# Stylish-TTS/stylish-tts

Measured on AMD Instinct MI355X. Metric: audio frames/sec/GPU (24 kHz) forward+backward; DDP scaling 1/2/4/8 MI355X, higher is better.
Workload: dtype bf16 GEMM operands, f32 accumulation/storage; 1 GPU; c3: B=32/GPU T=520 frames (6.5 s) L=100

## Files before the change

### stylish_tts_amd/csrc/api.hip

```cpp
#include <math.h>
#include <stdarg.h>
#include <string.h>
#include <stdlib.h>
#include <cxxabi.h>

#include <map>
#include <string>

#include "model.h"

namespace sty {

static thread_local char g_err[1024] = "";
void set_error(const char* fmt, ...) {
  va_list ap;
  va_start(ap, fmt);
  vsnprintf(g_err, sizeof(g_err), fmt, ap);
  va_end(ap);
}
int hip_fail(hipError_t e, const char* what) {
  set_error("HIP error %d (%s) at %s", (int)e, hipGetErrorString(e), what);
  return STY_EHIP;
}

// ... 44 lines not shown
  auto it = cache.find(fn);
  if (it != cache.end()) return it->second;
  std::string out;
  const char* mangled = hipKernelNameRefByPtr(fn, st);
  if (mangled) {
    int status = 0;
    char* dem = abi::__cxa_demangle(mangled, nullptr, nullptr, &status);
    std::string d = (status == 0 && dem) ? dem : mangled;
    free(dem);
    int depth = 0;
    size_t cut = d.size();
    for (size_t i = 0; i < d.size(); ++i) {
      if (d[i] == '<') ++depth;
      if (d[i] == '>') --depth;
      if (d[i] == '(' && depth == 0 && d.compare(i, 21, "(anonymous namespace)") != 0) {
        cut = i;
        break;
      }
    }
    d = d.substr(0, cut);
    if (d.compare(0, 5, "void ") == 0) d = d.substr(5);
    for (const char* ns : {"sty::(anonymous namespace)::", "sty::"})
      if (d.compare(0, strlen(ns), ns) == 0) d = d.substr(strlen(ns));
    out = d;
  }
  cache[fn] = out;
  return out;
}

struct Builder {
  sty_model* m;
  bool dry;
  bool ok = true;

  const Param* get(const std::string& key, std::initializer_list<int64_t> shape = {}) {
    if (dry) m->requested.push_back(key);
    auto it = m->params.find(key);
    if (it == m->params.end()) {
      if (ok) m->missing = key;
      ok = false;
      return nullptr;
    }
    if (shape.size()) {
      std::vector<int64_t> want(shape);
      if (want != it->second.shape) {
        if (ok) m->missing = key + " (shape mismatch)";
        ok = false;
        return nullptr;
      }
    }
    return &it->second;
  }
  const float* ptr(const std::string& key, std::initializer_list<int64_t> shape = {}) {
    const Param* p = get(key, shape);
    return p ? p->p : nullptr;
  }
  bool has(const std::string& key) const { return m->params.count(key) != 0; }

  PackedConv conv(const std::string& name, bool wn = false, bool bias = true, bool glu = false,
                  const float* bias_override_src = nullptr) {
    PackedConv pc;
    const Param* w = wn ? get(name + ".parametrizations.weight.original1") : get(name + ".weight");
    const Param* g = wn ? get(name + ".parametrizations.weight.original0") : nullptr;
    const float* b = bias ? ptr(name + ".bias") : nullptr;
    if (!w || (wn && !g)) return pc;
    const auto& s = w->shape;
    pc.Cout = (int)s[0];
    pc.Cin = (int)s[1];
    pc.K = s.size() > 2 ? (int)s[2] : 1;
    pc.CinP = (int)align_up(pc.Cin, CI_CHUNK);
    pc.CoutP = glu ? (int)align_up(pc.Cout, 64) : (int)align_up(pc.Cout, 32);
    float* wp = m->ab.take<float>((size_t)pc.K * pc.CinP * pc.CoutP);
    float* bp = m->ab.take<float>(pc.CoutP);
    pc.wp = wp;
    pc.bias = (bias || bias_override_src) ? bp : nullptr;
    if (!dry) {
      PackJob j;
      j.kind = glu ? PK_CONV_GLU : (wn ? PK_CONV_WN : PK_CONV);
      j.w = wn ? nullptr : w->p;
      j.g = g ? g->p : nullptr;
      j.v = wn ? w->p : nullptr;
      j.bias = b;
      j.Cout = pc.Cout;
      j.Cin = pc.Cin;
      j.K = pc.K;
      j.CinP = pc.CinP;
      j.CoutP = pc.CoutP;
      j.wp = wp;
      j.bp = bp;
      m->jobs.push_back(j);
    }
    if (m->train_enabled) {
      if (glu) {
        PackedConv pl = pc;
        pl.CoutP = (int)align_up(pc.Cout, 32);
        float* wp2 = m->ab.take<float>((size_t)pc.K * pc.CinP * pl.CoutP);
        float* bp2 = m->ab.take<float>(pl.CoutP);
        pl.wp = wp2;
        pl.bias = bias ? bp2 : nullptr;
        if (!dry) {
          PackJob j;
          j.kind = PK_CONV;
          j.w = w->p;
          j.bias = b;
          j.Cout = pc.Cout;
          j.Cin = pc.Cin;
          j.K = pc.K;
          j.CinP = pc.CinP;
          j.CoutP = pl.CoutP;
          j.wp = wp2;
          j.bp = bp2;
          m->jobs.push_back(j);
          m->plain_of[wp] = pl;
        }
        add_dgrad(pl);
      } else {
        add_dgrad(pc);
      }
    }
    return pc;
  }

  void add_dgrad(const PackedConv& pc) {
    PackedConv d;
    d.Cin = pc.Cout;
    d.CinP = pc.CoutP;
    d.Cout = pc.Cin;
    d.CoutP = pc.CinP;
    d.K = pc.K;
    float* wd = m->ab.take<float>((size_t)pc.K * pc.CinP * pc.CoutP);
    d.wp = wd;
    d.bias = nullptr;
    if (!dry) {
      PackJob j;
      j.kind = PK_DGRAD;
      j.w = pc.wp;
      j.K = pc.K;
      j.CinP = pc.CinP;
      j.CoutP = pc.CoutP;
      j.wp = wd;
      m->jobs.push_back(j);
      m->dgrad[pc.wp] = d;
    }
  }

  AdaFc fc(const std::string& name, int C) {
    AdaFc a;
    a.C = C;
    const float* W = ptr(name + ".fc.weight", {2 * C, m->style_dim});
    const float* b = ptr(name + ".fc.bias", {2 * C});
    a.off = m->gb_floats_per_batch;
    m->gb_floats_per_batch += 2 * C;
    if (!dry) {
      a.idx = (int)m->fcs.size();
      StyleFcDesc d;
      d.W = W;
      d.b = b;
      d.off = a.off;
      d.n = 2 * C;
      d.pad = 0;
      m->fcs.push_back(d);
    }
    return a;
  }

  ConvNeXt convnext(const std::string& p, int C, bool snake = true) {
    ConvNeXt c;
    c.C = C;
    c.dw_w = ptr(p + ".dwconv.weight", {C, 1, 7});
    c.dw_b = ptr(p + ".dwconv.bias", {C});
    c.norm = fc(p + ".norm", C);
    c.alpha = snake ? ptr(p + ".snake", {1, 1, 4 * C}) : nullptr;
    c.grn_gamma = ptr(p + ".grn.gamma", {1, 1, 4 * C});
    const float* grn_beta = ptr(p + ".grn.beta", {1, 1, 4 * C});
    c.b1 = ptr(p + ".pwconv1.bias", {4 * C});
    const float* w2 = ptr(p + ".pwconv2.weight", {C, 4 * C});
// ... 115 lines not shown
    v.phase_norm_w = ptr(b + "phase_norm.weight", {32});
    v.phase_norm_b = ptr(b + "phase_norm.bias", {32});
    v.amp_fln_w = ptr(b + "amp_final_layer_norm.weight", {32});
    v.amp_fln_b = ptr(b + "amp_final_layer_norm.bias", {32});
    v.phase_fln_w = ptr(b + "phase_final_layer_norm.weight", {32});
    v.phase_fln_b = ptr(b + "phase_final_layer_norm.bias", {32});
    v.phase_convnext.clear();
    for (int i = 0; has(b + "phase_convnext." + std::to_string(i) + ".dwconv.weight"); ++i)
      v.phase_convnext.push_back(convnext(b + "phase_convnext." + std::to_string(i), 32));
    if (ok && (v.amp_convnext.empty() || v.phase_convnext.empty())) {
      m->missing = b + "amp_convnext.0 / phase_convnext.0";
      ok = false;
    }
  }

  void text_encoder(const std::string& p) {
    TextEncPlan& t = m->te;
    const Param* e = get(p + "emb.weight");
    if (!e) return;
    t.emb = e->p;
    t.tokens = (int)e->shape[0];
    t.H = (int)e->shape[1];
    for (int i = 0; i < 3; ++i) {
      const std::string si = std::to_string(i);
      t.pre[i] = conv(p + "prenet.conv_layers." + si);
      t.pre_g[i] = ptr(p + "prenet.norm_layers." + si + ".gamma", {t.H});
      t.pre_b[i] = ptr(p + "prenet.norm_layers." + si + ".beta", {t.H});
    }
    t.proj = conv(p + "prenet.proj");
    t.layers.clear();
    for (int i = 0; has(p + "encoder.attn_layers." + std::to_string(i) + ".conv_q.weight"); ++i) {
      const std::string si = std::to_string(i);
      TextEncLayer l;
      l.q = conv(p + "encoder.attn_layers." + si + ".conv_q");
      l.k = conv(p + "encoder.attn_layers." + si + ".conv_k");
      l.v = conv(p + "encoder.attn_layers." + si + ".conv_v");
      l.o = conv(p + "encoder.attn_layers." + si + ".conv_o");
      l.n1g = ptr(p + "encoder.norm_layers_1." + si + ".gamma", {t.H});
      l.n1b = ptr(p + "encoder.norm_layers_1." + si + ".beta", {t.H});
      l.f1 = conv(p + "encoder.ffn_layers." + si + ".conv_1");
      l.f2 = conv(p + "encoder.ffn_layers." + si + ".conv_2");
      l.n2g = ptr(p + "encoder.norm_layers_2." + si + ".gamma", {t.H});
      l.n2b = ptr(p + "encoder.norm_layers_2." + si + ".beta", {t.H});
      t.layers.push_back(l);
    }
    t.proj_m = conv(p + "proj_m");
    for (int i = 0; i < 4; ++i) t.theta[i] = 1.0f / powf(10000.0f, (float)(2 * i) / 8.0f);
  }

  DecBlock dec_block(const std::string& p) {
    DecBlock d;
    d.c1 = conv(p + ".conv1", true);
    d.c2 = conv(p + ".conv2", true);
    d.Cin = d.c1.Cin;
    d.Cout = d.c1.Cout;
    d.n1 = fc(p + ".norm1", d.Cin);
    d.n2 = fc(p + ".norm2", d.Cout);
    d.has_sc = has(p + ".conv1x1.parametrizations.weight.original0");
    if (d.has_sc) d.sc = conv(p + ".conv1x1", true, false);
    return d;
  }

  void decoder(const std::string& p) {
    DecoderPlan& d = m->dec;
    d.encode = dec_block(p + "encode");
    for (int i = 0; i < 4; ++i) d.decode[i] = dec_block(p + "decode." + std::to_string(i));
    d.asr_res = conv(p + "asr_res.0", true);
    d.f0_g = ptr(p + "F0_conv.parametrizations.weight.original0", {1, 1, 1});
    d.f0_v = ptr(p + "F0_conv.parametrizations.weight.original1", {1, 1, 3});
// ... 1349 lines not shown
  std::vector<MultiJob> jobs[5];
  std::vector<int> blk[5];
  std::vector<int> blk1;
  auto PG = [&](const float* p) -> float* {
    auto it = p ? m->pgrad.find(p) : m->pgrad.end();
    return it == m->pgrad.end() ? nullptr : it->second;
  };
  auto GA = [&](const float* packed) -> float* {
    return (packed && m->garena) ? reinterpret_cast<float*>(m->garena + (reinterpret_cast<const char*>(packed) - m->arena))
                                 : nullptr;
  };
  auto add = [&](int which, MultiJob j, int nblocks) {
    j.blk0 = (int)blk[which].size();
    for (int i = 0; i < nblocks; ++i) blk[which].push_back((int)jobs[which].size());
    jobs[which].push_back(j);
  };
  size_t job_index = 0;
  m->seg_blk_split = 0;
  for (const PackJob& j : m->jobs) {
    if (job_index++ == m->seg_job_split) m->seg_blk_split = (int)blk[2].size();
    if (j.kind == PK_CONV || j.kind == PK_CONV_WN || j.kind == PK_CONV_GLU) {
      MultiJob a;
      a.p0 = j.w;
      a.p1 = j.g;
      a.p2 = j.v;
      a.p3 = j.bias;
      a.q0 = j.wp;
      a.q1 = j.bp;
      a.Cout = j.Cout;
      a.Cin = j.Cin;
      a.K = j.K;
      a.CinP = j.CinP;
      a.CoutP = j.CoutP;
      a.glu = j.kind == PK_CONV_GLU;
      add(0, a, j.Cout);
      if (m->garena && j.kind != PK_CONV_GLU) {
        MultiJob u;
        u.p0 = GA(j.wp);
        u.p1 = j.g;
        u.p2 = j.kind == PK_CONV_WN ? j.v : nullptr;
        u.p3 = (j.bias && j.bp) ? GA(j.bp) : nullptr;
        u.q0 = j.kind == PK_CONV ? PG(j.w) : nullptr;
        u.q1 = j.kind == PK_CONV_WN ? PG(j.g) : nullptr;
        u.q2 = j.kind == PK_CONV_WN ? PG(j.v) : nullptr;
        u.q3 = (j.bias && j.bp) ? PG(j.bias) : nullptr;
        u.Cout = j.Cout;
        u.Cin = j.Cin;
        u.K = j.K;
        u.CinP = j.CinP;
        u.CoutP = j.CoutP;
        if (u.q0 || (u.q1 && u.q2) || u.q3) add(2, u, j.Cout);
      }
    } else if (j.kind == PK_DGRAD) {
      MultiJob a;
      a.p0 = j.w;
      a.q0 = j.wp;
      a.K = j.K;
      a.CinP = j.CinP;
      a.CoutP = j.CoutP;
      add(1, a, (int)(((size_t)j.K * j.CinP * j.CoutP + 255) / 256));
    } else if (j.kind == PK_DGRAD2D) {
      MultiJob a;
      a.p0 = j.w;
      a.q0 = j.wp;
      a.K = j.K;
      a.KH = j.KH;
      a.Cin = j.Cin;
      a.Cout = j.Cout;
      a.CinP = j.CinP;
      a.CoutP = j.CoutP;
      a.glu = 2;
      a.blk1 = (int)align_up(j.KH * j.Cout, CI_CHUNK);
      a.pad = (int)align_up(j.Cin, 32);
      add(1, a, (int)(((size_t)j.K * j.KH * j.Cout * j.Cin + 255) / 256));
    }
    if (j.kind == PK_CONV2D_SN || j.kind == PK_DW2D_SN) {
      MultiJob a;
      a.p0 = j.w;
      a.p1 = j.bias;
      a.p2 = j.kind == PK_CONV2D_SN ? j.bp : nullptr;
      a.q0 = const_cast<float*>(j.g);
      a.q1 = const_cast<float*>(j.v);
      a.q2 = j.scratch;
// ... 1159 lines not shown
```

### stylish_tts_amd/csrc/attn.hip

```cpp
#include "sty_common.h"

namespace sty {


template <int DH, bool DROP>
__global__ __launch_bounds__(256) void attn_kernel(AttnArgs a) {
  constexpr int DP = DH < 32 ? 32 : DH;
  constexpr int LS = 33;
  __shared__ float ks[DH * LS];
  __shared__ float vs[DP * LS];
  const int tid = threadIdx.x, lane = tid & 63, wave = tid >> 6, l31 = lane & 31, hi = lane >> 5;
  const int b = blockIdx.z, h = blockIdx.y, T = a.T;
  const int i0 = blockIdx.x * 128 + wave * 32;
  const int qi = i0 + l31;
  const float* qb = a.q + (size_t)b * a.qbs + (size_t)h * DH * T;
  const float* kb = a.k + (size_t)b * a.kbs + (size_t)h * DH * T;
  const float* vb = a.v + (size_t)b * a.vbs + (size_t)h * DH * T;
  int len = T;
  if (a.lengths) len = (int)a.lengths[b];

  float qreg[DH / 2];
#pragma unroll
  for (int c2 = 0; c2 < DH / 2; ++c2) qreg[c2] = qi < T ? qb[(size_t)(2 * c2 + hi) * T + qi] * a.scale : 0.f;

  f32x16 oacc[DP / 32];
#pragma unroll
  for (int d = 0; d < DP / 32; ++d)
#pragma unroll
    for (int r = 0; r < 16; ++r) oacc[d][r] = 0.f;
  float m_run = -3.0e38f, l_run = 0.f;
  const bool q_pad = a.lengths && qi >= len;

  for (int j0 = 0; j0 < T; j0 += 32) {
    __syncthreads();
    for (int e = tid; e < DH * 32; e += 256) {
      const int d = e >> 5, jj = e & 31;
      const int j = j0 + jj;
      ks[d * LS + jj] = j < T ? kb[(size_t)d * T + j] : 0.f;
      vs[d * LS + jj] = j < T ? vb[(size_t)d * T + j] : 0.f;
    }
    if (DP > DH)
      for (int e = tid; e < (DP - DH) * 32; e += 256) vs[(DH + (e >> 5)) * LS + (e & 31)] = 0.f;
    __syncthreads();

    f32x16 s;
#pragma unroll
    for (int r = 0; r < 16; ++r) s[r] = 0.f;
#pragma unroll
    for (int c2 = 0; c2 < DH / 2; ++c2)
      s = __builtin_amdgcn_mfma_f32_32x32x2f32(ks[(2 * c2 + hi) * LS + l31], qreg[c2], s, 0, 0, 0);

    float mx = -3.0e38f;
#pragma unroll
    for (int r = 0; r < 16; ++r) {
      const int j = j0 + (r & 3) + 8 * (r >> 2) + 4 * hi;
      float x = s[r];
      if (a.lengths && (q_pad || j >= len)) x += -1e4f;
      if (j >= T) x = -INFINITY;
      s[r] = x;
      mx = fmaxf(mx, x);
    }
    mx = fmaxf(mx, __shfl_xor(mx, 32));
    const float m_new = fmaxf(m_run, mx);
    const float alpha = expf(m_run - m_new);
    float rs = 0.f;
#pragma unroll
    for (int r = 0; r < 16; ++r) {
      const float p = expf(s[r] - m_new);
      s[r] = p;
      rs += p;
    }
// ... 5 lines not shown
      const unsigned rowi = ((unsigned)(b * a.H + h) * (unsigned)T + (unsigned)qi) * (unsigned)T;
#pragma unroll
      for (int r = 0; r < 16; ++r) {
        const int j = j0 + (r & 3) + 8 * (r >> 2) + 4 * hi;
        s[r] = sty_hash_u(a.drop_seed, a.drop_site, rowi + (unsigned)j) >= a.drop_p ? s[r] * ks_ : 0.f;
      }
    }
#pragma unroll
    for (int d = 0; d < DP / 32; ++d) {
#pragma unroll
      for (int r = 0; r < 16; ++r) oacc[d][r] *= alpha;
#pragma unroll
      for (int q = 0; q < 16; ++q) {
        const float av = vs[(d * 32 + l31) * LS + (q & 3) + 8 * (q >> 2) + 4 * hi];
        oacc[d] = __builtin_amdgcn_mfma_f32_32x32x2f32(av, s[q], oacc[d], 0, 0, 0);
      }
    }
  }
  if (qi < T) {
    if (a.lse && hi == 0) a.lse[((size_t)b * a.H + h) * T + qi] = m_run + logf(l_run);
    const float inv = 1.0f / l_run;
    float* ob = a.o + (size_t)b * a.obs + (size_t)h * DH * T;
#pragma unroll
    for (int d = 0; d < DP / 32; ++d)
#pragma unroll
      for (int r = 0; r < 16; ++r) {
        const int dd = d * 32 + (r & 3) + 8 * (r >> 2) + 4 * hi;
        if (dd < DH) ob[(size_t)dd * T + qi] = oacc[d][r] * inv;
      }
  }
}

int launch_attention(const AttnArgs& a, int B, int DH, hipStream_t st) {
  if (attention16_eligible(a, DH)) return launch_attention16(a, B, st);
  dim3 grid(cdiv(a.T, 128), a.H, B);
  const bool drop = a.drop_p > 0.f;
  if (DH == 64 && !drop)
    hipLaunchKernelGGL((attn_kernel<64, false>), grid, dim3(256), 0, st, a);
  else if (DH == 16 && !drop)
    hipLaunchKernelGGL((attn_kernel<16, false>), grid, dim3(256), 0, st, a);
  else if (DH == 160 && !drop)
    hipLaunchKernelGGL((attn_kernel<160, false>), grid, dim3(256), 0, st, a);
  else if (DH == 96 && !drop)
    hipLaunchKernelGGL((attn_kernel<96, false>), grid, dim3(256), 0, st, a);
  else if (DH == 16)
    hipLaunchKernelGGL((attn_kernel<16, true>), grid, dim3(256), 0, st, a);
  else if (DH == 160)
    hipLaunchKernelGGL((attn_kernel<160, true>), grid, dim3(256), 0, st, a);
  else {
    set_error("attention: head dim %d%s not built (16, 64, 96, 160; dropout: 16, 160)", DH, drop ? " with dropout" : "");
    return STY_EINVAL;
  }
  STY_LAUNCH_CHECK();
  return STY_OK;
}

__global__ void rope_kernel(const float* qs, const float* ks, float* q, float* k, int H, int DH, int L, int d, float t0, float t1, float t2, float t3,
                            float sgn) {
  const int pos = blockIdx.x * blockDim.x + threadIdx.x;
  const int h = blockIdx.y, b = blockIdx.z;
  if (pos >= L) return;
  const float theta[4] = {t0, t1, t2, t3};
  const int half = d / 2;
  const float* src[2] = {qs, ks};
  float* ptr[2] = {q, k};
  for (int w = 0; w < 2; ++w) {
    const size_t o = ((size_t)b * H + h) * DH * L + pos;
    const float* sb_ = src[w] + o;
    float* base = ptr[w] + o;
    float x[8];
    for (int i = 0; i < d; ++i) x[i] = sb_[(size_t)i * L];
    for (int i = 0; i < d; ++i) {
      const float ang = (float)pos * theta[i % half];
      const float rot = i < half ? -x[i + half] : x[i - half];
      base[(size_t)i * L] = x[i] * cosf(ang) + rot * (sgn * sinf(ang));
    }
    if (sb_ != base)
      for (int i = d; i < DH; ++i) base[(size_t)i * L] = sb_[(size_t)i * L];
  }
}

int launch_rope_signed(float* q, float* k, int B, int H, int DH, int L, int d, const float* theta4, float sgn,
                       hipStream_t st) {
  if (d != 8) {
    set_error("rope: only d == 8 built");
    return STY_EINVAL;
  }
  hipLaunchKernelGGL(rope_kernel, dim3(cdiv(L, 64), H, B), dim3(64), 0, st, q, k, q, k, H, DH, L, d, theta4[0], theta4[1],
                     theta4[2], theta4[3], sgn);
  STY_LAUNCH_CHECK();
  return STY_OK;
}
int launch_rope_copy(const float* qs, const float* ks, float* q, float* k, int B, int H, int DH, int L, int d,
                     const float* theta4, hipStream_t st) {
  if (d != 8) {
    set_error("rope: only d == 8 built");
    return STY_EINVAL;
  }
  hipLaunchKernelGGL(rope_kernel, dim3(cdiv(L, 64), H, B), dim3(64), 0, st, qs, ks, q, k, H, DH, L, d, theta4[0], theta4[1],
                     theta4[2], theta4[3], 1.0f);
  STY_LAUNCH_CHECK();
  return STY_OK;
}
int launch_rope(float* q, float* k, int B, int H, int DH, int L, int d, const float* theta4, hipStream_t st) {
  return launch_rope_signed(q, k, B, H, DH, L, d, theta4, 1.0f, st);
}
}
```

### stylish_tts_amd/csrc/attn_bwd.hip

```cpp
#include <stdlib.h>

#include "sty_common.h"

namespace sty {

template <int DH>
__global__ __launch_bounds__(64) void attn_bwd_a_kernel(AttnArgs a, const float* __restrict__ dO, size_t dobs,
                                                        float* __restrict__ lse, float* __restrict__ delta) {
  const int T = a.T, b = blockIdx.z, h = blockIdx.y, i = blockIdx.x * 64 + threadIdx.x;
  if (i >= T) return;
  const float* qb = a.q + (size_t)b * a.qbs + (size_t)h * DH * T;
  const float* kb = a.k + (size_t)b * a.kbs + (size_t)h * DH * T;
  const float* ob = a.o + (size_t)b * a.obs + (size_t)h * DH * T;
  const float* gb = dO + (size_t)b * dobs + (size_t)h * DH * T;
  const int len = a.lengths ? (int)a.lengths[b] : T;
  float q[DH];
  float dl = 0.f;
#pragma unroll
  for (int d = 0; d < DH; ++d) {
    q[d] = qb[(size_t)d * T + i] * a.scale;
    dl = fmaf(gb[(size_t)d * T + i], ob[(size_t)d * T + i], dl);
  }
  float m = -3.0e38f, l = 0.f;
  const bool qpad = a.lengths && i >= len;
// ... 295 lines not shown
    }
#pragma unroll
    for (int n = 0; n < NB; ++n)
#pragma unroll
      for (int q = 0; q < 16; ++q)
        dq[n] = __builtin_amdgcn_mfma_f32_32x32x2f32(ks[(n * 32 + l31) * LS + frag_row(q, hi)], dp[q], dq[n], 0, 0, 0);
  }
  if (i < T) {
    float* dqb = dQ + (size_t)b * dqbs + (size_t)h * DH * T;
#pragma unroll
    for (int n = 0; n < NB; ++n)
#pragma unroll
      for (int r = 0; r < 16; ++r) dqb[(size_t)(n * 32 + frag_row(r, hi)) * T + i] += dq[n][r] * a.scale;
  }
}


template <int DH, bool DROP>
__global__ __launch_bounds__(256) void attn_bwd_small_kernel(AttnArgs a, const float* __restrict__ dO, size_t dobs,
                                                            float* __restrict__ dQ, size_t dqbs, float* __restrict__ dK,
                                                            size_t dkbs, float* __restrict__ dV, size_t dvbs, int overwrite) {
  constexpr int TP = 129;
  __shared__ float qs[DH * TP], ks[DH * TP], vs[DH * TP], gs[DH * TP];
  __shared__ float lse_s[128], del_s[128], pm_s[128], pl_s[128];
  const int T = a.T, h = blockIdx.x, b = blockIdx.y, tid = threadIdx.x;
  const int r = tid & 127, half = tid >> 7;
  const size_t ho = (size_t)h * DH * T;
  const float* qb = a.q + (size_t)b * a.qbs + ho;
  const float* kb = a.k + (size_t)b * a.kbs + ho;
  const float* vb = a.v + (size_t)b * a.vbs + ho;
  const float* gb = dO + (size_t)b * dobs + ho;
  const float* ob = a.o + (size_t)b * a.obs + ho;
  const int len = a.lengths ? (int)a.lengths[b] : T;
  for (int e = tid; e < DH * T; e += 256) {
    const int d = e / T, t = e - d * T;
    qs[d * TP + t] = qb[e] * a.scale;
    ks[d * TP + t] = kb[e];
    vs[d * TP + t] = vb[e];
    gs[d * TP + t] = gb[e];
  }
  __syncthreads();
  const int per = (T + 1) / 2, lo = half * per, hi = min(T, lo + per);
  const bool live = r < T;
  const bool rpad = a.lengths && r >= len;
  float q[DH], g[DH];
#pragma unroll
  for (int d = 0; d < DH; ++d) {
    q[d] = live ? qs[d * TP + r] : 0.f;
    g[d] = live ? gs[d * TP + r] : 0.f;
  }
  {
    float m = -3.0e38f, l = 0.f;
    if (live)
      for (int j = lo; j < hi; ++j) {
        float sv = 0.f;
#pragma unroll
        for (int d = 0; d < DH; ++d) sv = fmaf(q[d], ks[d * TP + j], sv);
        if (a.lengths && (rpad || j >= len)) sv += -1e4f;
        const float mn = fmaxf(m, sv);
        l = l * expf(m - mn) + expf(sv - mn);
        m = mn;
      }
    if (half == 1) {
      pm_s[r] = m;
      pl_s[r] = l;
    } else if (live) {
      float dl = 0.f;
#pragma unroll
      for (int d = 0; d < DH; ++d) dl = fmaf(g[d], ob[(size_t)d * T + r], dl);
      del_s[r] = dl;
// ... 6 lines not shown
    }
    __syncthreads();
  }
  const float inv_keep = DROP ? 1.0f / (1.0f - a.drop_p) : 1.f;
  const unsigned rowbase = (unsigned)(b * a.H + h) * (unsigned)T;
  {
    float acc[DH];
#pragma unroll
    for (int d = 0; d < DH; ++d) acc[d] = 0.f;
    if (live) {
      const float L = lse_s[r], dl = del_s[r];
      for (int j = lo; j < hi; ++j) {
        float sv = 0.f, dp = 0.f;
#pragma unroll
        for (int d = 0; d < DH; ++d) {
          sv = fmaf(q[d], ks[d * TP + j], sv);
          dp = fmaf(g[d], vs[d * TP + j], dp);
        }
        if (a.lengths && (rpad || j >= len)) sv += -1e4f;
        if constexpr (DROP) {
          const unsigned idx = (rowbase + (unsigned)r) * (unsigned)T + (unsigned)j;
          dp = sty_hash_u(a.drop_seed, a.drop_site, idx) >= a.drop_p ? dp * inv_keep : 0.f;
        }
        const float ds = expf(sv - L) * (dp - dl);
#pragma unroll
        for (int d = 0; d < DH; ++d) acc[d] = fmaf(ds, ks[d * TP + j], acc[d]);
      }
    }
#pragma unroll
    for (int d = 0; d < DH; ++d) {
      __syncthreads();
      if (half == 1) pm_s[r] = acc[d];
      __syncthreads();
      if (half == 0 && live) {
        float* dq = dQ + (size_t)b * dqbs + ho;
        const float val = (acc[d] + pm_s[r]) * a.scale;
        dq[(size_t)d * T + r] = (overwrite & 1) ? val : dq[(size_t)d * T + r] + val;
      }
    }
  }
  {
    float kk[DH], vv[DH], ak[DH], av[DH];
#pragma unroll
    for (int d = 0; d < DH; ++d) {
      kk[d] = live ? ks[d * TP + r] : 0.f;
      vv[d] = live ? vs[d * TP + r] : 0.f;
      ak[d] = av[d] = 0.f;
    }
    if (live)
      for (int i = lo; i < hi; ++i) {
        float sv = 0.f, dp = 0.f;
#pragma unroll
        for (int d = 0; d < DH; ++d) {
          sv = fmaf(qs[d * TP + i], kk[d], sv);
          dp = fmaf(gs[d * TP + i], vv[d], dp);
        }
        if (a.lengths && (i >= len || rpad)) sv += -1e4f;
        const float p = expf(sv - lse_s[i]);
        float pm = p;
        if constexpr (DROP) {
          const unsigned idx = (rowbase + (unsigned)i) * (unsigned)T + (unsigned)r;
          const float mf = sty_hash_u(a.drop_seed, a.drop_site, idx) >= a.drop_p ? inv_keep : 0.f;
          pm = p * mf;
          dp *= mf;
        }
        const float ds = p * (dp - del_s[i]);
#pragma unroll
        for (int d = 0; d < DH; ++d) {
          av[d] = fmaf(pm, gs[d * TP + i], av[d]);
          ak[d] = fmaf(ds, qs[d * TP + i], ak[d]);
        }
      }
    float* dk = dK + (size_t)b * dkbs + ho;
    float* dv = dV + (size_t)b * dvbs + ho;
#pragma unroll
    for (int d = 0; d < DH; ++d) {
      __syncthreads();
      if (half == 1) {
        pm_s[r] = ak[d];
        pl_s[r] = av[d];
      }
      __syncthreads();
      if (half == 0 && live) {
        const float vk = ak[d] + pm_s[r], vv_ = av[d] + pl_s[r];
        dk[(size_t)d * T + r] = (overwrite & 2) ? vk : dk[(size_t)d * T + r] + vk;
        dv[(size_t)d * T + r] = (overwrite & 4) ? vv_ : dv[(size_t)d * T + r] + vv_;
      }
    }
  }
}

size_t attention_bwd_ws_floats(int B, int H, int T) { return (size_t)2 * B * H * T; }

bool attention_bwd_mfma_dh(int DH) { return DH == 64 || DH == 96 || DH == 160; }
static bool attn_bwd_mfma_path(const AttnArgs& a, int DH) { return a.lse && attention_bwd_mfma_dh(DH); }
static bool attn_bwd_small_path(const AttnArgs& a, int DH) {
  if (attention16_eligible(a, DH) && a.lse) return false;
  if (attn_bwd_mfma_path(a, DH)) return false;
  return DH == 16 && a.T <= 128;
}
bool attention_bwd_can_overwrite(const AttnArgs& a, int DH) { return attn_bwd_small_path(a, DH); }

int launch_attention_bwd(const AttnArgs& a, const float* dO, float* dQ, float* dK, float* dV, size_t dqbs, size_t dkbs,
                         size_t dvbs, size_t dobs, int B, int DH, float* ws, hipStream_t st, int overwrite) {
  if (overwrite && !attn_bwd_small_path(a, DH)) {
    set_error("attention_bwd: overwrite requested on a path that accumulates");
    return STY_EINVAL;
  }
  if (attention16_eligible(a, DH) && a.lse)
    return launch_attention16_bwd(a, dO, dQ, dK, dV, dqbs, dkbs, dvbs, dobs, B, ws, st);
  float* lse = ws;
  float* delta = ws + (size_t)B * a.H * a.T;
  if (attn_bwd_mfma_path(a, DH)) {
    hipLaunchKernelGGL(attn_delta_kernel, dim3(cdiv(a.T, 256), a.H, B), dim3(256), 0, st, a.o, a.obs, dO, dobs, a.H, DH,
                       a.T, delta);
    dim3 g2(cdiv(a.T, 128), a.H, B);
#define STY_ABWD_MFMA(DHV, DR)                                                                                                      \
  hipLaunchKernelGGL((attn_bwd_kv_mfma_kernel<DHV, DR>), g2, dim3(256), 0, st, a, dO, dobs, a.lse, delta, dK, dkbs, dV, dvbs);       \
  hipLaunchKernelGGL((attn_bwd_q_mfma_kernel<DHV, DR>), g2, dim3(256), 0, st, a, dO, dobs, a.lse, delta, dQ, dqbs)
    const bool dr = a.drop_p > 0.f;
    if (DH == 64 && !dr) {
      STY_ABWD_MFMA(64, false);
    } else if (DH == 64) {
      STY_ABWD_MFMA(64, true);
    } else if (DH == 96 && !dr) {
      STY_ABWD_MFMA(96, false);
    } else if (DH == 96) {
      STY_ABWD_MFMA(96, true);
    } else if (!dr) {
      STY_ABWD_MFMA(160, false);
    } else {
      STY_ABWD_MFMA(160, true);
    }
#undef STY_ABWD_MFMA
    STY_LAUNCH_CHECK();
    return STY_OK;
  }
  const bool drop = a.drop_p > 0.f;
  if (attn_bwd_small_path(a, DH)) {
    if (drop)
      hipLaunchKernelGGL((attn_bwd_small_kernel<16, true>), dim3(a.H, B), dim3(256), 0, st, a, dO, dobs, dQ, dqbs, dK, dkbs, dV,
                         dvbs, overwrite);
    else
      hipLaunchKernelGGL((attn_bwd_small_kernel<16, false>), dim3(a.H, B), dim3(256), 0, st, a, dO, dobs, dQ, dqbs, dK, dkbs,
                         dV, dvbs, overwrite);
    STY_LAUNCH_CHECK();
    return STY_OK;
  }
  if (DH != 16) {
    set_error("attention_bwd: head dim %d%s not built", DH, drop ? " with dropout" : "");
    return STY_EINVAL;
  }
  dim3 grid(cdiv(a.T, 64), a.H, B);
#define STY_ABWD(DR)                                                                                                         \
  hipLaunchKernelGGL(attn_bwd_a_kernel<16>, grid, dim3(64), 0, st, a, dO, dobs, lse, delta);                                 \
  hipLaunchKernelGGL((attn_bwd_b_kernel<16, DR>), grid, dim3(256), 2 * 16 * 65 * sizeof(float), st, a, dO, dobs, lse, delta, \
                     dK, dkbs, dV, dvbs);                                                                                    \
  hipLaunchKernelGGL((attn_bwd_c_kernel<16, DR>), grid, dim3(64), 0, st, a, dO, dobs, lse, delta, dQ, dqbs)
  if (drop) {
    STY_ABWD(true);
  } else {
    STY_ABWD(false);
  }
#undef STY_ABWD
  STY_LAUNCH_CHECK();
  return STY_OK;
}

}
```

### stylish_tts_amd/csrc/bwd.hip

```cpp
#include "sty_common.h"

namespace sty {

__device__ __forceinline__ double wave_sum(double v) {
  for (int o = 32; o > 0; o >>= 1) v += __shfl_xor(v, o);
  return v;
}

template <int N>
__device__ __forceinline__ void block_sum(double (&v)[N], double (*red)[4]) {
  const int lane = threadIdx.x & 63, wave = threadIdx.x >> 6;
#pragma unroll
  for (int i = 0; i < N; ++i) {
    v[i] = wave_sum(v[i]);
    if (lane == 0) red[i][wave] = v[i];
  }
  __syncthreads();
  if (threadIdx.x == 0) {
#pragma unroll
    for (int i = 0; i < N; ++i) v[i] = red[i][0] + red[i][1] + red[i][2] + red[i][3];
  }
}

__global__ __launch_bounds__(256) void pro_bwd_kernel(int mode_, const float* __restrict__ u, int Cu, int cu0,
// ... 305 lines not shown
                                                          float eps, float* __restrict__ mean, float* __restrict__ rstd) {
  const int i = blockIdx.x * 4 + (threadIdx.x >> 6), lane = threadIdx.x & 63;
  if (i >= rows) return;
  double sum = 0.0, sq = 0.0;
  for (int k = lane; k < nseg; k += 64) {
    sum += part[((size_t)i * nseg + k) * 2];
    sq += part[((size_t)i * nseg + k) * 2 + 1];
  }
  for (int o = 32; o > 0; o >>= 1) {
    sum += __shfl_xor(sum, o);
    sq += __shfl_xor(sq, o);
  }
  if (lane) return;
  const double m = sum / T;
  double var = sq / T - m * m;
  if (var < 0.0) var = 0.0;
  mean[i] = (float)m;
  rstd[i] = (float)(1.0 / sqrt(var + (double)eps));
}
int launch_adain_stats(const double* part, int nseg, int rows, int T, float eps, float* mean, float* rstd,
                       hipStream_t st) {
  hipLaunchKernelGGL(adain_stats_kernel, dim3(cdiv(rows, 4)), dim3(256), 0, st, part, nseg, rows, T, eps, mean, rstd);
  STY_LAUNCH_CHECK();
  return STY_OK;
}

template <int TC, int NR>
__global__ __launch_bounds__(256) void chan_ln_bwd_dx_reg_kernel(const float* __restrict__ x, const float* __restrict__ dy,
                                                                 const float* __restrict__ y, int C, int T, float eps,
                                                                 int ada, const float* __restrict__ w,
                                                                 const float* __restrict__ gb, int relu,
                                                                 const float* __restrict__ out_mask,
                                                                 float* __restrict__ dx, int accumulate,
                                                                 float* __restrict__ mu_out, float* __restrict__ r_out) {
  constexpr int CG = 256 / TC;
  __shared__ float red[2][CG][TC];
  const int col = threadIdx.x % TC, cg = threadIdx.x / TC;
  const int t = blockIdx.x * TC + col, b = blockIdx.y;
  const bool in = t < T;
  const size_t base = (size_t)b * C * T + (in ? t : 0);
  auto combine = [&](float a, float bb, float& ra, float& rb) {
    red[0][cg][col] = a;
    red[1][cg][col] = bb;
    __syncthreads();
    float s0 = 0.f, s1 = 0.f;
#pragma unroll
    for (int k = 0; k < CG; ++k) {
      s0 += red[0][k][col];
      s1 += red[1][k][col];
    }
    __syncthreads();
    ra = s0;
    rb = s1;
  };
  const float om = (in && out_mask) ? out_mask[(size_t)b * T + t] : 1.f;
  float xr[NR], gr[NR];
#pragma unroll
  for (int i = 0; i < NR; ++i) {
    const int c = cg + i * CG;
    xr[i] = gr[i] = 0.f;
    if (in && c < C) {
      const size_t o = base + (size_t)c * T;
      xr[i] = x[o];
      float g = dy[o] * om;
      if (relu && !(y[o] > 0.f)) g = 0.f;
      const float A = ada ? 1.f + gb[(size_t)b * 2 * C + c] : w[c];
      gr[i] = g * A;
// ... 5 lines not shown
    if (in && cg + i * CG < C) p0 += xr[i];
  combine(p0, 0.f, mean, dummy);
  mean /= (float)C;
  p0 = 0.f;
#pragma unroll
  for (int i = 0; i < NR; ++i)
    if (in && cg + i * CG < C) {
      const float d = xr[i] - mean;
      p0 += d * d;
    }
  float var;
  combine(p0, 0.f, var, dummy);
  const float r = 1.0f / sqrtf(var / (float)C + eps);
  p0 = p1 = 0.f;
#pragma unroll
  for (int i = 0; i < NR; ++i)
    if (in && cg + i * CG < C) {
      const float dxh = gr[i], xh = (xr[i] - mean) * r;
      p0 += dxh;
      p1 += dxh * xh;
    }
  float s1, s2;
  combine(p0, p1, s1, s2);
  s1 /= (float)C;
  s2 /= (float)C;
  if (!in) return;
#pragma unroll
  for (int i = 0; i < NR; ++i) {
    const int c = cg + i * CG;
    if (c < C) {
      const size_t o = base + (size_t)c * T;
      const float xh = (xr[i] - mean) * r;
      const float d = r * (gr[i] - s1 - xh * s2);
      dx[o] = accumulate ? dx[o] + d : d;
    }
  }
  if (cg == 0) {
    mu_out[(size_t)b * T + t] = mean;
    r_out[(size_t)b * T + t] = r;
  }
}
template <int TC>
__global__ __launch_bounds__(256) void chan_ln_bwd_dx_kernel(const float* __restrict__ x, const float* __restrict__ dy,
                                                             const float* __restrict__ y, int C, int T, float eps,
                                                             int ada, const float* __restrict__ w,
                                                             const float* __restrict__ gb, int relu,
                                                             const float* __restrict__ out_mask,
                                                             float* __restrict__ dx, int accumulate,
                                                             float* __restrict__ mu_out, float* __restrict__ r_out) {
  constexpr int CG = 256 / TC;
  __shared__ float red[2][CG][TC];
  const int col = threadIdx.x % TC, cg = threadIdx.x / TC;
  const int t = blockIdx.x * TC + col, b = blockIdx.y;
  const bool in = t < T;
  const size_t base = (size_t)b * C * T + (in ? t : 0);
  auto combine = [&](float a, float bb, float& ra, float& rb) {
    red[0][cg][col] = a;
    red[1][cg][col] = bb;
    __syncthreads();
    float s0 = 0.f, s1 = 0.f;
#pragma unroll
    for (int k = 0; k < CG; ++k) {
      s0 += red[0][k][col];
      s1 += red[1][k][col];
    }
    __syncthreads();
    ra = s0;
    rb = s1;
  };
  float p0 = 0.f, p1 = 0.f, mean, dummy;
  if (in)
    for (int c = cg; c < C; c += CG) p0 += x[base + (size_t)c * T];
  combine(p0, 0.f, mean, dummy);
  mean /= (float)C;
  p0 = 0.f;
  if (in)
    for (int c = cg; c < C; c += CG) {
      const float d = x[base + (size_t)c * T] - mean;
      p0 += d * d;
    }
  float var;
  combine(p0, 0.f, var, dummy);
  const float r = 1.0f / sqrtf(var / (float)C + eps);
  const float om = (in && out_mask) ? out_mask[(size_t)b * T + t] : 1.f;
  p0 = p1 = 0.f;
  if (in)
    for (int c = cg; c < C; c += CG) {
      const size_t o = base + (size_t)c * T;
      float g = dy[o] * om;
      if (relu && !(y[o] > 0.f)) g = 0.f;
      const float A = ada ? 1.f + gb[(size_t)b * 2 * C + c] : w[c];
      const float dxh = g * A, xh = (x[o] - mean) * r;
      p0 += dxh;
      p1 += dxh * xh;
    }
  float s1, s2;
  combine(p0, p1, s1, s2);
  s1 /= (float)C;
  s2 /= (float)C;
  if (!in) return;
  for (int c = cg; c < C; c += CG) {
    const size_t o = base + (size_t)c * T;
    float g = dy[o] * om;
    if (relu && !(y[o] > 0.f)) g = 0.f;
    const float A = ada ? 1.f + gb[(size_t)b * 2 * C + c] : w[c];
    const float xh = (x[o] - mean) * r;
    const float d = r * (g * A - s1 - xh * s2);
    dx[o] = accumulate ? dx[o] + d : d;
  }
  if (cg == 0) {
    mu_out[(size_t)b * T + t] = mean;
    r_out[(size_t)b * T + t] = r;
  }
}
__global__ __launch_bounds__(256) void chan_ln_bwd_param_kernel(const float* __restrict__ x,
                                                                const float* __restrict__ dy,
                                                                const float* __restrict__ y,
                                                                const float* __restrict__ mu,
                                                                const float* __restrict__ r, int C, int T, int ada,
                                                                int relu, const float* __restrict__ out_mask,
                                                                float* __restrict__ dgb, float* __restrict__ dw,
                                                                float* __restrict__ db) {
  __shared__ double red[2][4];
  const int c = blockIdx.x, b = blockIdx.y;
  const size_t row = ((size_t)b * C + c) * T;
  double acc[2] = {0.0, 0.0};
  for (int t = threadIdx.x; t < T; t += 256) {
    float g = dy[row + t];
    if (out_mask) g *= out_mask[(size_t)b * T + t];
    if (relu && !(y[row + t] > 0.f)) g = 0.f;
    const float xh = (x[row + t] - mu[(size_t)b * T + t]) * r[(size_t)b * T + t];
    acc[0] += (double)g * xh;
    acc[1] += (double)g;
  }
  block_sum<2>(acc, red);
  if (threadIdx.x == 0) {
    if (ada) {
      dgb[(size_t)b * 2 * C + c] += (float)acc[0];
      dgb[(size_t)b * 2 * C + C + c] += (float)acc[1];
    } else {
      atomicAdd(&dw[c], (float)acc[0]);
// ... 76 lines not shown
  double s = 0.0;
  for (int b = b0; b < b0 + nb; ++b)
    for (int k = lane; k < nblk; k += 64) s += (double)part[((size_t)b * nblk + k) * 64 + slot];
  s = wave_sum(s);
  if (lane == 0) {
    if (ada)
      dgb[(size_t)b0 * 64 + slot] += (float)s;
    else if (slot < 32)
      dw[slot] += (float)s;
    else
      db[slot - 32] += (float)s;
  }
}

__global__ void cast_any_kernel(const void* __restrict__ x, size_t n, void* __restrict__ y, int to16) {
  const size_t i = (size_t)blockIdx.x * 256 + threadIdx.x;
  if (i < n) sty_st_any(y, i, sty_ld_any(x, i, !to16), to16);
}
int launch_cast_f32_to_16(const float* x, size_t n, void* y16, hipStream_t st) {
  hipLaunchKernelGGL(cast_any_kernel, dim3((unsigned)((n + 255) / 256)), dim3(256), 0, st, x, n, y16, 1);
  STY_LAUNCH_CHECK();
  return STY_OK;
}
int launch_cast_16_to_f32(const void* x16, size_t n, float* y, hipStream_t st) {
  hipLaunchKernelGGL(cast_any_kernel, dim3((unsigned)((n + 255) / 256)), dim3(256), 0, st, x16, n, y, 0);
  STY_LAUNCH_CHECK();
  return STY_OK;
}
bool chan_ln32_eligible(int B, int C, int T, int relu) {
  return C == 32 && !relu && (size_t)B * T >= 65536 && getenv("STY_NO_LN32_BWD") == nullptr;
}
int launch_chan_ln_bwd(const float* x, const float* dy, const float* y, int B, int C, int T, float eps, int ada,
                       const float* w, const float* gb, int relu, const float* out_mask, float* dx, int accumulate,
                       float* mu_tmp, float* r_tmp, float* dgb, float* dw, float* db, hipStream_t st, int h16) {
  const bool no32 = getenv("STY_NO_LN32_BWD") != nullptr;
  if (C == 32 && !relu && (size_t)B * T >= 65536 && !no32) {
    const int nblk = cdiv(T, 256);
    if ((h16 & 4) && accumulate) {
      set_error("chan_ln_bwd: a two-byte dx cannot be accumulated into");
      return STY_EINVAL;
    }
    hipLaunchKernelGGL(chan_ln32_bwd_kernel, dim3(nblk, B), dim3(256), 0, st, x, dy, T, eps, ada, w, gb, out_mask, dx, accumulate,
                       mu_tmp, h16);
    hipLaunchKernelGGL(chan_ln32_param_sum_kernel, dim3(ada ? B * 64 : 64), dim3(64), 0, st, mu_tmp, B, nblk, ada, dgb, dw, db);
    STY_LAUNCH_CHECK();
    return STY_OK;
  }
  if (h16) {
    set_error("chan_ln_bwd: two-byte tensors only on the C = 32 long-row kernel (chan_ln32_eligible)");
    return STY_EINVAL;
  }
  if ((size_t)B * T < 65536 && C <= 256)
    hipLaunchKernelGGL((chan_ln_bwd_dx_reg_kernel<16, 16>), dim3(cdiv(T, 16), B), dim3(256), 0, st, x, dy, y, C, T, eps, ada, w,
                       gb, relu, out_mask, dx, accumulate, mu_tmp, r_tmp);
  else if ((size_t)B * T >= 65536)
    hipLaunchKernelGGL(chan_ln_bwd_dx_kernel<64>, dim3(cdiv(T, 64), B), dim3(256), 0, st, x, dy, y, C, T, eps, ada, w, gb,
                       relu, out_mask, dx, accumulate, mu_tmp, r_tmp);
  else
    hipLaunchKernelGGL(chan_ln_bwd_dx_kernel<16>, dim3(cdiv(T, 16), B), dim3(256), 0, st, x, dy, y, C, T, eps, ada, w, gb,
                       relu, out_mask, dx, accumulate, mu_tmp, r_tmp);
  hipLaunchKernelGGL(chan_ln_bwd_param_kernel, dim3(C, B), dim3(256), 0, st, x, dy, y, mu_tmp, r_tmp, C, T, ada, relu,
                     out_mask, dgb, dw, db);
  STY_LAUNCH_CHECK();
  return STY_OK;
}

__global__ __launch_bounds__(256) void grn_bwd_kernel(const double* __restrict__ part, int nseg,
                                                      const float* __restrict__ gamma,
                                                      const float* __restrict__ ds, int C4,
                                                      float* __restrict__ coef, float* __restrict__ dgamma) {
  __shared__ float gxs[1024];
  __shared__ double red[2][4];
  const int b = blockIdx.x;
  if (nseg < 32) {
    for (int c = threadIdx.x; c < C4; c += 256) {
      double sq = 0.0;
      for (int k = 0; k < nseg; ++k) sq += part[(((size_t)b * C4 + c) * nseg + k) * 2 + 1];
      gxs[c] = (float)sqrt(sq);
    }
  } else {
    const int lane = threadIdx.x & 63, wave = threadIdx.x >> 6;
    for (int c = wave; c < C4; c += 4) {
      const double* pp = part + ((size_t)b * C4 + c) * nseg * 2 + 1;
      double sq = 0.0;
      for (int k = lane; k < nseg; k += 64) sq += pp[(size_t)k * 2];
      for (int o = 32; o > 0; o >>= 1) sq += __shfl_xor(sq, o);
      if (lane == 0) gxs[c] = (float)sqrt(sq);
    }
  }
  __syncthreads();
  double acc[1] = {0.0};
  for (int c = threadIdx.x; c < C4; c += 256) acc[0] += gxs[c];
  __shared__ float mean_s, dot_s;
// ... 44 lines not shown
  else if (kind == ACT_SWISH) r = v / (1.f + expf(-v));
  else if (kind == ACT_SNAKE) r = sty_snake(v, alpha[c], 1.f / alpha[c]);
  else if (kind == 100) r = tanhf(v);
  else if (kind == ACT_GELU) r = 0.5f * v * (1.0f + erff(v * 0.70710678118654752f));
  y[o] = r;
}
__device__ __forceinline__ float act_apply1(int kind, float v, float al, float ral) {
  float r = v;
  if (kind == ACT_RELU) r = fmaxf(v, 0.f);
  else if (kind == ACT_SWISH) r = v / (1.f + expf(-v));
  else if (kind == ACT_SNAKE) r = sty_snake(v, al, ral);
  else if (kind == 100) r = tanhf(v);
  else if (kind == ACT_GELU) r = 0.5f * v * (1.0f + erff(v * 0.70710678118654752f));
  return r;
}
__global__ __launch_bounds__(256) void act_fwd4_kernel(int kind, const float* __restrict__ x, const float* __restrict__ alpha,
                                                       unsigned C, unsigned T4, unsigned n4, float* __restrict__ y) {
  const unsigned idx = blockIdx.x * 256u + threadIdx.x;
  if (idx >= n4) return;
  float al = 1.f, ral = 1.f;
  if (kind == ACT_SNAKE) {
    al = alpha[(idx / T4) % C];
    ral = 1.f / al;
  }
  const float4 v = reinterpret_cast<const float4*>(x)[idx];
  float4 r;
  r.x = act_apply1(kind, v.x, al, ral);
  r.y = act_apply1(kind, v.y, al, ral);
  r.z = act_apply1(kind, v.z, al, ral);
  r.w = act_apply1(kind, v.w, al, ral);
  reinterpret_cast<float4*>(y)[idx] = r;
}
int launch_act_fwd(int kind, const float* x, const float* alpha, int B, int C, int T, float* y, hipStream_t st) {
  const size_t n4 = (size_t)B * C * (T / 4);
  if (kind != ACT_GLU && T % 4 == 0 && n4 < ((size_t)1 << 31) && ((((size_t)x | (size_t)y) & 15) == 0)) {
    hipLaunchKernelGGL(act_fwd4_kernel, dim3((unsigned)((n4 + 255) / 256)), dim3(256), 0, st, kind, x, alpha, (unsigned)C,
                       (unsigned)(T / 4), (unsigned)n4, y);
    STY_LAUNCH_CHECK();
    return STY_OK;
  }
  hipLaunchKernelGGL(act_fwd_kernel, dim3(cdiv(T, 256), C, B), dim3(256), 0, st, kind, x, alpha, C, T, y);
  STY_LAUNCH_CHECK();
  return STY_OK;
}
__global__ __launch_bounds__(256) void act_bwd_kernel(int kind, const float* __restrict__ x,
                                                      const float* __restrict__ dy, const float* __restrict__ alpha,
                                                      int C, int T, float* __restrict__ dx, int accumulate,
                                                      float* __restrict__ dalpha) {
  __shared__ double red[1][4];
  const int c = blockIdx.x, b = blockIdx.y;
  double acc[1] = {0.0};
  if (kind == ACT_GLU) {
    const size_t ra = ((size_t)b * 2 * C + c) * T, rg = ((size_t)b * 2 * C + C + c) * T, ro = ((size_t)b * C + c) * T;
    for (int t = threadIdx.x; t < T; t += 256) {
      const float a = x[ra + t], g = x[rg + t], d = dy[ro + t];
      const float sg = 1.f / (1.f + expf(-g));
      const float da = d * sg, dg = d * a * sg * (1.f - sg);
      dx[ra + t] = accumulate ? dx[ra + t] + da : da;
      dx[rg + t] = accumulate ? dx[rg + t] + dg : dg;
    }
    return;
  }
  const size_t row = ((size_t)b * C + c) * T;
  const float al = kind == ACT_SNAKE ? alpha[c] : 1.f;
  auto one = [&](float v, float d) -> float {
    float g = d;
// ... 31 lines not shown
        g = make_float4(o.x + g.x, o.y + g.y, o.z + g.z, o.w + g.w);
      }
      o4[t] = g;
    }
  } else
  for (int t = threadIdx.x; t < T; t += 256) {
    const float v = x[row + t], d = dy[row + t];
    float g = d;
    if (kind == ACT_RELU) g = v > 0.f ? d : 0.f;
    else if (kind == ACT_SWISH) {
      const float sg = 1.f / (1.f + expf(-v));
      g = d * (sg + v * sg * (1.f - sg));
    } else if (kind == ACT_SNAKE) {
      float sn, cs;
      sty_sincos(al * v, sn, cs);
      const float s2 = sn * sn, s2a = 2.f * sn * cs;
      g = d * (1.f + s2a);
      acc[0] += (double)(d * (v * s2a - s2 / al) / al);
    } else if (kind == 100) {
      const float th = tanhf(v);
      g = d * (1.f - th * th);
    } else if (kind == ACT_GELU) {
      g = d * (0.5f * (1.0f + erff(v * 0.70710678118654752f)) + v * 0.3989422804014327f * expf(-0.5f * v * v));
    }
    dx[row + t] = accumulate ? dx[row + t] + g : g;
  }
  if (kind == ACT_SNAKE && dalpha) {
    block_sum<1>(acc, red);
    if (threadIdx.x == 0) atomicAdd(&dalpha[c], (float)acc[0]);
  }
}
int launch_act_bwd(int kind, const float* x, const float* dy, const float* alpha, int B, int C, int T, float* dx,
                   int accumulate, float* dalpha, hipStream_t st) {
  hipLaunchKernelGGL(act_bwd_kernel, dim3(C, B), dim3(256), 0, st, kind, x, dy, alpha, C, T, dx, accumulate, dalpha);
  STY_LAUNCH_CHECK();
  return STY_OK;
}

__global__ void row_scale_add_kernel(const float* __restrict__ src, const float* __restrict__ coef, float k, int T,
                                     float* __restrict__ dst) {
  const int t = blockIdx.x * 256 + threadIdx.x, row = blockIdx.y;
  if (t >= T) return;
  const size_t o = (size_t)row * T + t;
  dst[o] += src[o] * (coef ? coef[row] : k);
}
__global__ __launch_bounds__(256) void row_scale_add4_kernel(const float* __restrict__ src, const float* __restrict__ coef,
                                                             float k, unsigned T4, unsigned n4, float* __restrict__ dst) {
  const unsigned idx = blockIdx.x * 256u + threadIdx.x;
  if (idx >= n4) return;
  const float f = coef ? coef[idx / T4] : k;
  const float4 sv = reinterpret_cast<const float4*>(src)[idx];
  float4 d = reinterpret_cast<float4*>(dst)[idx];
  d.x += sv.x * f;
  d.y += sv.y * f;
  d.z += sv.z * f;
  d.w += sv.w * f;
  reinterpret_cast<float4*>(dst)[idx] = d;
}
int launch_row_scale_add(const float* src, const float* coef, float k, int rows, int T, float* dst, hipStream_t st) {
  const size_t n4 = (size_t)rows * (T / 4);
  if (vec4_ok(n4, T, src, dst)) {
    hipLaunchKernelGGL(row_scale_add4_kernel, dim3((unsigned)((n4 + 255) / 256)), dim3(256), 0, st, src, coef, k,
                       (unsigned)(T / 4), (unsigned)n4, dst);
    STY_LAUNCH_CHECK();
    return STY_OK;
  }
  hipLaunchKernelGGL(row_scale_add_kernel, dim3(cdiv(T, 256), rows), dim3(256), 0, st, src, coef, k, T, dst);
  STY_LAUNCH_CHECK();
  return STY_OK;
}

__global__ void dwconv_fwd_kernel(const float* __restrict__ x, const float* __restrict__ w,
                                  const float* __restrict__ bias, int C, int T, int K, int pad,
                                  float* __restrict__ y) {
  const int t = blockIdx.x * 256 + threadIdx.x, c = blockIdx.y, b = blockIdx.z;
  if (t >= T) return;
  const float* p = x + ((size_t)b * C + c) * T;
  float acc = bias ? bias[c] : 0.f;
  for (int k = 0; k < K; ++k) {
    const int tt = t - pad + k;
    if (tt >= 0 && tt < T) acc = fmaf(w[c * K + k], p[tt], acc);
  }
  y[((size_t)b * C + c) * T + t] = acc;
}
template <int MAXK>
__global__ __launch_bounds__(256) void dwconv_fwd4_kernel(const float* __restrict__ x, const float* __restrict__ w,
                                                          const float* __restrict__ bias, int C, int T, int K, int pad,
                                                          float* __restrict__ y) {
  const int t0 = (blockIdx.x * 256 + threadIdx.x) * 4, c = blockIdx.y, b = blockIdx.z;
  if (t0 >= T) return;
  const float* p = x + ((size_t)b * C + c) * T;
  float wk[MAXK];
// ... 274 lines not shown
  double acc[2] = {0.0, 0.0};
  for (int b = 0; b < B; ++b) {
    const size_t row = ((size_t)b * C + c) * T;
    for (int t = threadIdx.x; t < T; t += 256) {
      const float g = dy[row + t];
      dx[row + t] = g * w[c] * inv;
      acc[0] += (double)g * ((x[row + t] - rm[c]) * inv);
      acc[1] += g;
    }
  }
  block_sum<2>(acc, red);
  if (threadIdx.x == 0) {
    dw[c] += (float)acc[0];
    db[c] += (float)acc[1];
  }
}
int launch_bn_eval_bwd(const float* x, const float* dy, const float* w, const float* rm, const float* rv, float eps,
                       int B, int C, int T, float* dx, float* dw, float* db, hipStream_t st) {
  hipLaunchKernelGGL(bn_eval_bwd_kernel, dim3(C), dim3(256), 0, st, x, dy, w, rm, rv, eps, B, C, T, dx, dw, db);
  STY_LAUNCH_CHECK();
  return STY_OK;
}

__global__ void dropout_kernel(const float* __restrict__ x, const float* __restrict__ res, size_t n, float p,
                               unsigned seed, unsigned site, float* __restrict__ y, int accumulate, size_t group) {
  const size_t i = (size_t)blockIdx.x * 256 + threadIdx.x;
  if (i >= n) return;
  float v = sty_hash_u(seed, site, (unsigned)(i / group)) >= p ? x[i] / (1.0f - p) : 0.f;
  if (res) v += res[i];
  y[i] = accumulate ? y[i] + v : v;
}
int launch_dropout(const float* x, const float* res, size_t n, float p, unsigned seed, unsigned site, float* y,
                   int accumulate, hipStream_t st, size_t group) {
  hipLaunchKernelGGL(dropout_kernel, dim3((unsigned)((n + 255) / 256)), dim3(256), 0, st, x, res, n, p, seed, site, y,
                     accumulate, group ? group : 1);
  STY_LAUNCH_CHECK();
  return STY_OK;
}

__global__ void bn_train_finalize_kernel(const double* __restrict__ part, int nseg, int B, int C, int T, float eps,
                                         float momentum, float* __restrict__ rm, float* __restrict__ rv,
                                         float* __restrict__ mean, float* __restrict__ rstd) {
  const int c = blockIdx.x * blockDim.x + threadIdx.x;
  if (c >= C) return;
  double s = 0.0, q = 0.0;
  for (int b = 0; b < B; ++b)
    for (int k = 0; k < nseg; ++k) {
      s += part[(((size_t)b * C + c) * nseg + k) * 2];
      q += part[(((size_t)b * C + c) * nseg + k) * 2 + 1];
    }
  const double n = (double)B * T;
  const double mu = s / n;
  double var = q / n - mu * mu;
  if (var < 0.0) var = 0.0;
  mean[c] = (float)mu;
  rstd[c] = (float)(1.0 / sqrt(var + (double)eps));
  rm[c] = (1.f - momentum) * rm[c] + momentum * (float)mu;
  rv[c] = (1.f - momentum) * rv[c] + momentum * (float)(var * n / (n - 1.0));
}
__global__ void bn_apply_kernel(const float* __restrict__ x, const float* __restrict__ w, const float* __restrict__ bvec,
                                const float* __restrict__ mean, const float* __restrict__ rstd, int C, int T,
                                float* __restrict__ y) {
  const int t = blockIdx.x * 256 + threadIdx.x, c = blockIdx.y, b = blockIdx.z;
  if (t >= T) return;
  const size_t o = ((size_t)b * C + c) * T + t;
  y[o] = (x[o] - mean[c]) * rstd[c] * w[c] + bvec[c];
// ... 266 lines not shown
```

### stylish_tts_amd/csrc/conv1d.hip

```cpp
#include <stdlib.h>

#include "sty_common.h"

namespace sty {

__device__ __forceinline__ float sigmoidf_(float v) { return 1.0f / (1.0f + expf(-v)); }

}

#include "conv_stage.h"

namespace sty {

template <int ACT>
__device__ __forceinline__ float act_apply(float x, float alpha) {
  if constexpr (ACT == ACT_RELU) return fmaxf(x, 0.f);
  if constexpr (ACT == ACT_SWISH) return x * sigmoidf_(x);
  if constexpr (ACT == ACT_SNAKE) return sty_snake(x, alpha, 1.0f / alpha);
  if constexpr (ACT == ACT_GELU) return 0.5f * x * (1.0f + erff(x * 0.70710678118654752f));
  return x;
}

constexpr int STY_MINW = 2;
template <int WM, int WN, int MT, int NT, int KS = 1, bool BF = false>
// ... 332 lines not shown
  hipLaunchKernelGGL((conv1d_mfma_kernel<WM, WN, MT, NT, KS, BF>), grid, dim3(64 * WM * WN * KS), lds, st, a);
  STY_LAUNCH_CHECK();
  return STY_OK;
}

static int launch_conv1d_dispatch(const ConvArgs& a, hipStream_t st);
int launch_conv1d(const ConvArgs& a, hipStream_t st) {
  if (a.up_g && !conv1d_has_up_stage(a)) {
    set_error("conv1d: up-sample + gate output stage asked of a conv that does not run on convq_kernel");
    return STY_EINVAL;
  }
  const bool native16 = a.y16 && (stem2d_eligible(a) || (!conv32p_eligible(a) && !convk1_eligible(a) && convp16_eligible(a)));
  int rc = launch_conv1d_dispatch(a, st);
  if (rc == STY_OK && a.y16 && !native16) {
    if (a.shuffle > 1) {
      set_error("conv1d: no output twin for a pixel-shuffled store");
      return STY_EINVAL;
    }
    rc = launch_twin_cast(a.y, nullptr, a.y16_act, a.B, a.w.Cout, a.T, a.y16, st);
  }
  return rc;
}
bool conv1d_reads_twin_only(const ConvArgs& a) {
  if (!a.x16 || a.nsrc != 1 || a.act == ACT_LRELU01) return false;
  if (stem2d_eligible(a) || conv32p_eligible(a) || a.xh || a.yh || a.rh || a.stat_part || convk1_eligible(a)) return false;
  return convp16_eligible(a);
}
bool conv1d_has_up_stage(const ConvArgs& a) {
  if (!conv1d_reads_twin_only(a) || !convq_eligible(a)) return false;
  if (!a.flatW || a.act != ACT_NONE || a.out_mask || a.residual) return false;
  if (a.up_g && (!a.up_gate16 || !a.up_mask || a.up_H <= 0 || a.up_H * a.flatW != a.T)) return false;
  return (long)a.w.Cout * a.T < (1l << 26);
}
static int launch_conv1d_dispatch(const ConvArgs& a, hipStream_t st) {
  int cin = 0;
  for (int i = 0; i < a.nsrc; ++i) cin += a.xc[i];
  if (a.flatW) cin = a.w.Cin;
  if (cin != a.w.Cin) {
    set_error("conv1d: input channels %d != weight Cin %d", cin, a.w.Cin);
    return STY_ESHAPE;
  }
  if (a.pro == PRO_LN_AFFINE && a.w.CinP != CI_CHUNK) {
    set_error("conv1d: LN prologue needs Cin <= %d", CI_CHUNK);
    return STY_EINVAL;
  }
  if (a.ln_out && a.w.Cout != 32) {
    set_error("conv1d: LN epilogue needs Cout == 32");
    return STY_EINVAL;
  }
  if (stem2d_eligible(a)) return launch_stem2d(a, st);
  if (conv32p_eligible(a)) return launch_conv32p(a, st);
  if (a.xh || a.yh || a.rh) {
    set_error("conv1d: bf16-stored operand (xh %d yh %d rh %d) on a conv the persistent 32-channel kernel does not take", a.xh,
              a.yh, a.rh);
    return STY_EINVAL;
  }
  if (a.stat_part) {
    set_error("conv1d: output statistics requested for a conv the persistent 32-channel kernel does not take");
    return STY_EINVAL;
  }
  if (convk1_eligible(a)) return launch_convk1(a, st);
  if (convp16_eligible(a)) return launch_convp16(a, st);
  const long tiles128 = (long)cdiv(a.T, 128) * (a.w.CoutP / 128) * a.B;
  const long t128_min = a.bf16 ? 256 : 512;
  const long t64_min = a.bf16 ? 256 : 512;
  constexpr long t32_min = 512;
  if (a.act == ACT_GLU) {
    if (a.w.CoutP % 128 == 0 && tiles128 >= t128_min) return launch_cfg<2, 2, 2, 2>(a, st);
    return launch_cfg<1, 4, 2, 1>(a, st);
  }
  if (a.w.CoutP % 128 == 0 && tiles128 >= t128_min) return launch_cfg<2, 2, 2, 2>(a, st);
  if (a.w.CoutP % 64 == 0) {
    const long tiles64 = (long)cdiv(a.T, 256) * (a.w.CoutP / 64) * a.B;
    if (tiles64 >= t64_min) return launch_cfg<1, 4, 2, 2>(a, st);
    const long wgs = (long)cdiv(a.T, 64) * (a.w.CoutP / 64) * a.B;
    constexpr int ks4_wgs = 64;
    if (wgs <= ks4_wgs && a.ksplit_max >= 4 && a.w.CinP >= 8 * CI_CHUNK && a.pro != PRO_LN_AFFINE)
      return launch_cfg<2, 2, 1, 1, 4>(a, st);
    constexpr int ks2_wgs = 256;
    if (wgs <= ks2_wgs && a.w.CinP >= 4 * CI_CHUNK && a.pro != PRO_LN_AFFINE) return launch_cfg<2, 2, 1, 1, 2>(a, st);
// ... 60 lines not shown
```

### stylish_tts_amd/csrc/convk1.hip

```cpp
#include <stdlib.h>

#include "sty_common.h"
#include "conv_stage.h"

namespace sty {

constexpr int G_KC = 64;
constexpr int G_PITCH = 160;

typedef short g_s4 __attribute__((ext_vector_type(4)));

__device__ __forceinline__ unsigned g_pk(float a, float b) {
  typedef __bf16 b2 __attribute__((ext_vector_type(2)));
  b2 r;
  r[0] = (__bf16)a;
  r[1] = (__bf16)b;
  return __builtin_bit_cast(unsigned, r);
}

template <int PRO, int RELU>
__global__ __launch_bounds__(256, 2) void convk1_kernel(ConvArgs a, int tiles_per_row, int ncot, int ntiles, int per_xcd) {
  extern __shared__ __attribute__((aligned(16))) __bf16 g_lds[];
  const int tid = threadIdx.x, lane = tid & 63, wave = __builtin_amdgcn_readfirstlane(tid >> 6), l31 = lane & 31, hi = lane >> 5;
  const int wm = wave >> 1, wn = wave & 1;
// ... 89 lines not shown
    for (int ks = 0; ks < 4; ++ks) {
      bf16x8 bfrag[2];
#pragma unroll
      for (int n = 0; n < 2; ++n) {
        const __bf16* p = xb + (ks * 16 + trow) * G_PITCH + tcol + n * 32;
        const g_s4 lo = __builtin_amdgcn_ds_read_tr16_b64_v4i16((__attribute__((address_space(3))) g_s4*)(p));
        const g_s4 hi4 = __builtin_amdgcn_ds_read_tr16_b64_v4i16((__attribute__((address_space(3))) g_s4*)(p + 4 * G_PITCH));
        typedef short s8 __attribute__((ext_vector_type(8)));
        s8 q;
        q[0] = lo[0];
        q[1] = lo[1];
        q[2] = lo[2];
        q[3] = lo[3];
        q[4] = hi4[0];
        q[5] = hi4[1];
        q[6] = hi4[2];
        q[7] = hi4[3];
        bfrag[n] = __builtin_bit_cast(bf16x8, q);
      }
#pragma unroll
      for (int m = 0; m < 2; ++m)
#pragma unroll
        for (int n = 0; n < 2; ++n)
          acc[m][n] = __builtin_amdgcn_mfma_f32_32x32x16_bf16(ac[ks >> 1][ks & 1][m], bfrag[n], acc[m][n], 0, 0, 0);
    }
  }

  __syncthreads();
  float* stg = reinterpret_cast<float*>(g_lds) + wave * 32 * 68;
  const unsigned ybytes = (unsigned)((size_t)a.B * Cout * T * 4);
  const __amdgpu_buffer_rsrc_t ry = __builtin_amdgcn_make_buffer_rsrc(a.y, 0, ybytes, 0x00020000);
  const __amdgpu_buffer_rsrc_t rres = __builtin_amdgcn_make_buffer_rsrc(
      const_cast<float*>(a.residual ? a.residual : a.y), 0, a.residual ? ybytes : 0, 0x00020000);
  const bool post = a.out_mask && a.out_mask_post;
  const int c4 = lane & 15, rq = lane >> 4;
  const int nq = n0 + wn * 64 + 4 * c4;
  const bool qin = nq < NT;
  const int bq = qin ? nq / T : 0, tq = nq - bq * T;
  float om[4] = {1.f, 1.f, 1.f, 1.f};
  if (a.out_mask && qin) {
#pragma unroll
    for (int e = 0; e < 4; ++e) om[e] = a.out_mask[(size_t)nq + e];
  }
#pragma unroll
  for (int m = 0; m < 2; ++m) {
#pragma unroll
    for (int n = 0; n < 2; ++n)
#pragma unroll
      for (int r = 0; r < 16; ++r) stg[((r & 3) + 8 * (r >> 2) + 4 * hi) * 68 + n * 32 + l31] = acc[m][n][r];
    __syncthreads();
    const int cobase = cot * 128 + (wm * 2 + m) * 32;
#pragma unroll
    for (int i = 0; i < 8; ++i) {
      const int row = rq + 4 * i, co = cobase + row;
      if (co < Cout && qin) {
        const int yo = ((bq * Cout + co) * T + tq) * 4;
        const float4 sv = *reinterpret_cast<const float4*>(stg + row * 68 + 4 * c4);
        const float bi = a.w.bias ? a.w.bias[co] : 0.f;
        float v[4] = {sv.x + bi, sv.y + bi, sv.z + bi, sv.w + bi};
        float al = 1.f, ral = 1.f;
        if (RELU == 2) {
          al = a.act_alpha[co];
          ral = 1.0f / al;
        }
        float4 res = make_float4(0.f, 0.f, 0.f, 0.f);
        if (a.residual) res = __builtin_bit_cast(float4, __builtin_amdgcn_raw_buffer_load_b128(rres, yo, 0, 0));
        const float rr[4] = {res.x, res.y, res.z, res.w};
#pragma unroll
        for (int e = 0; e < 4; ++e) {
          if (RELU == 1) v[e] = fmaxf(v[e], 0.f);
          if (RELU == 2) v[e] = sty_snake(v[e], al, ral);
          if (RELU == 3) v[e] = 0.5f * v[e] * (1.0f + erff(v[e] * 0.70710678118654752f));
          v[e] *= a.out_scale;
          if (a.out_mask && !post) v[e] *= om[e];
          v[e] += rr[e];
          if (post) v[e] *= om[e];
        }
        const float4 o4 = make_float4(v[0], v[1], v[2], v[3]);
        __builtin_amdgcn_raw_buffer_store_b128(
            __builtin_bit_cast(__attribute__((__vector_size__(4 * sizeof(unsigned)))) unsigned, o4), ry, yo, 0, 0);
      }
    }
    __syncthreads();
  }
}

int convp16_frags(const ConvArgs& a, hipStream_t st, const void** out);

bool convk1_eligible(const ConvArgs& a) {
  if (!a.bf16 || getenv("STY_NO_CONVK1")) return false;
  if (a.w.K != 1 || a.flatW || a.nsrc != 1 || a.in_shuffle > 1 || a.shuffle != 1 || a.ln_out || a.Tin || a.y_split) return false;
  if (!(a.act == ACT_NONE || a.act == ACT_RELU || (a.act == ACT_SNAKE && a.act_alpha) || a.act == ACT_GELU)) return false;
  if (!(a.pro == PRO_NONE || a.pro == PRO_MASK || a.pro == PRO_SCALE)) return false;
  if (a.T % 4 || a.w.CinP % G_KC || a.w.CinP < 64 || a.w.CoutP < 64) return false;
  if ((size_t)a.B * a.w.CinP * a.T * 4 >= (size_t)1 << 31 || (size_t)a.B * a.w.CoutP * a.T * 4 >= (size_t)1 << 31) return false;
  const char* mt = getenv("STY_CONVK1_MIN_TILES");
  return (long)cdiv(a.B * a.T, 128) * cdiv(a.w.CoutP, 128) >= (mt ? atoi(mt) : 24);
}

template <int PRO>
static void g_launch(const ConvArgs& a, dim3 grid, size_t lds, int tpr, int ncot, int ntiles, int per, hipStream_t st) {
  if (a.act == ACT_RELU)
    hipLaunchKernelGGL((convk1_kernel<PRO, 1>), grid, dim3(256), lds, st, a, tpr, ncot, ntiles, per);
  else if (a.act == ACT_SNAKE)
    hipLaunchKernelGGL((convk1_kernel<PRO, 2>), grid, dim3(256), lds, st, a, tpr, ncot, ntiles, per);
  else if (a.act == ACT_GELU)
    hipLaunchKernelGGL((convk1_kernel<PRO, 3>), grid, dim3(256), lds, st, a, tpr, ncot, ntiles, per);
// ... 28 lines not shown
```

### stylish_tts_amd/csrc/convp16.hip

```cpp
#include <stdlib.h>

#include <mutex>
#include <unordered_map>

#include <algorithm>
#include <vector>

#include "sty_common.h"
#include "conv_stage.h"

namespace sty {

constexpr int Q_TT = 128;
constexpr int Q_PITCH = 40;
constexpr int Q_MAXQ = 3;
constexpr int Q_MAXK = 5;
constexpr int Q_NP = 12;
constexpr int Q_THREADS = 64 * (4 + Q_NP);

struct QTile {
  int b, t0, cot;
};
__device__ __forceinline__ QTile q_tile(int tile, int tiles_per_row, int ncot) {
  QTile t;
// ... 162 lines not shown
  if (t >= T) return;
  const bool wide = t + 3 < T;
  const __amdgpu_buffer_rsrc_t yrs =
      __builtin_amdgcn_make_buffer_rsrc(a.y + (size_t)tl.b * Cout * T, 0, Cout * T * 4, 0x00020000);
  const __amdgpu_buffer_rsrc_t rrs = __builtin_amdgcn_make_buffer_rsrc(
      const_cast<float*>(a.residual ? a.residual + (size_t)tl.b * Cout * T : a.y), 0, a.residual ? Cout * T * 4 : 0, 0x00020000);
  float om[4] = {1.f, 1.f, 1.f, 1.f};
  if (a.out_mask) {
#pragma unroll
    for (int e = 0; e < 4; ++e) om[e] = t + e < T ? a.out_mask[(size_t)tl.b * T + t + e] : 0.f;
  }
  const bool post = a.out_mask && a.out_mask_post;
  const float pre_scale = a.out_scale;
  const int rl0 = 2 * pw + half + 2 * Q_NP * part;
#pragma unroll 1
  for (int rl = rl0; rl < ROWS; rl += 2 * Q_NP * nparts) {
    const int co = tl.cot * ROWS + rl;
    if (co >= Cout) continue;
    float4 res = make_float4(0.f, 0.f, 0.f, 0.f);
    if (a.residual) res = __builtin_bit_cast(float4, __builtin_amdgcn_raw_buffer_load_b128(rrs, t * 4, co * T * 4, 0));
    const float4 sv = *reinterpret_cast<const float4*>(ost + rl * Q_TT + 4 * l);
    const float bi = bias_lds[co];
    float v[4] = {sv.x + bi, sv.y + bi, sv.z + bi, sv.w + bi};
    float rr[4] = {res.x, res.y, res.z, res.w};
    if (!wide && a.residual) {
#pragma unroll 1
      for (int e = 1; e < 4; ++e) {
        const float x = t + e < T ? __builtin_bit_cast(float, __builtin_amdgcn_raw_buffer_load_b32(rrs, (t + e) * 4, co * T * 4, 0)) : 0.f;
        rr[1] = e == 1 ? x : rr[1];
        rr[2] = e == 2 ? x : rr[2];
        rr[3] = e == 3 ? x : rr[3];
      }
    }
#pragma unroll
    for (int e = 0; e < 4; ++e) {
      if (RELU == 1) v[e] = fmaxf(v[e], 0.f);
      if (RELU == 2) v[e] = v[e] > 0.f ? v[e] : 0.1f * v[e];
      v[e] *= pre_scale;
      if (a.out_mask && !post) v[e] *= om[e];
      v[e] += rr[e];
      if (post) v[e] *= om[e];
    }
    if (RELU == 2 && a.y_split) {
      float* sp = a.y_split + (size_t)tl.b * 2 * Cout * (T >> 1) + (size_t)co * (T >> 1) + (t >> 1);
      *reinterpret_cast<float2*>(sp) = make_float2(v[0], v[2]);
      *reinterpret_cast<float2*>(sp + (size_t)Cout * (T >> 1)) = make_float2(v[1], v[3]);
    }
    if (a.y16) {
      float u[4];
#pragma unroll
      for (int e = 0; e < 4; ++e) u[e] = (a.y16_act == PRO_LRELU && v[e] < 0.f) ? 0.2f * v[e] : v[e];
      const __amdgpu_buffer_rsrc_t trs =
          __builtin_amdgcn_make_buffer_rsrc(a.y16 + (size_t)tl.b * Cout * T, 0, Cout * T * 2, 0x00020000);
      typedef __bf16 bf16x2 __attribute__((ext_vector_type(2)));
      bf16x2 p0, p1;
      p0[0] = (__bf16)u[0];
      p0[1] = (__bf16)u[1];
      p1[0] = (__bf16)u[2];
      p1[1] = (__bf16)u[3];
      const unsigned d0 = __builtin_bit_cast(unsigned, p0), d1 = __builtin_bit_cast(unsigned, p1);
      if (wide) {
        typedef unsigned u32x2 __attribute__((ext_vector_type(2)));
        u32x2 dd;
        dd[0] = d0;
        dd[1] = d1;
        __builtin_amdgcn_raw_buffer_store_b64(dd, trs, t * 2, co * T * 2, 0);
      } else {
#pragma unroll 1
        for (int e = 0; e < 4; ++e) {
          const unsigned h = e == 0 ? d0 : e == 1 ? d0 >> 16 : e == 2 ? d1 : d1 >> 16;
          if (t + e < T) __builtin_amdgcn_raw_buffer_store_b16((unsigned short)h, trs, (t + e) * 2, co * T * 2, 0);
        }
// ... 509 lines not shown
```

### stylish_tts_amd/csrc/misc.hip

```cpp
#include <stdlib.h>

#include "sty_common.h"

namespace sty {

__global__ void embedding_kernel(const int64_t* __restrict__ tok, const float* __restrict__ emb, int L, int H, int ntok,
                                 float scale, float* __restrict__ y) {
  const int l = blockIdx.x * blockDim.x + threadIdx.x;
  const int c = blockIdx.y, b = blockIdx.z;
  if (l >= L) return;
  int64_t t = tok[(size_t)b * L + l];
  if (t < 0 || t >= ntok) t = 0;
  y[((size_t)b * H + c) * L + l] = emb[(size_t)t * H + c] * scale;
}
int launch_embedding(const int64_t* tokens, const float* emb, int B, int L, int H, int ntok, float scale, float* y,
                     hipStream_t st) {
  hipLaunchKernelGGL(embedding_kernel, dim3(cdiv(L, 64), H, B), dim3(64), 0, st, tokens, emb, L, H, ntok, scale, y);
  STY_LAUNCH_CHECK();
  return STY_OK;
}

__global__ void length_mask_kernel(const int64_t* __restrict__ len, int L, float* __restrict__ mask) {
  const int l = blockIdx.x * blockDim.x + threadIdx.x;
  const int b = blockIdx.y;
  if (l < L) mask[(size_t)b * L + l] = (int64_t)l < len[b] ? 1.f : 0.f;
}
int launch_length_mask(const int64_t* lengths, int B, int L, float* mask, hipStream_t st) {
  hipLaunchKernelGGL(length_mask_kernel, dim3(cdiv(L, 64), B), dim3(64), 0, st, lengths, L, mask);
  STY_LAUNCH_CHECK();
  return STY_OK;
}

__global__ __launch_bounds__(256) void bmm_ct_kernel(const float* __restrict__ enc, const float* __restrict__ ali,
                                                     int C, int L, int T, float* __restrict__ y) {
  extern __shared__ float es[];
  const int b = blockIdx.z, c0 = blockIdx.y * 4;
  const int t = blockIdx.x * 64 + (threadIdx.x & 63), cw = threadIdx.x >> 6;
  for (int i = threadIdx.x; i < 4 * L; i += 256) {
    const int cc = i / L, l = i % L;
    es[i] = (c0 + cc < C) ? enc[((size_t)b * C + c0 + cc) * L + l] : 0.f;
  }
  __syncthreads();
  if (t >= T || c0 + cw >= C) return;
  const float* a = ali + (size_t)b * L * T + t;
  float acc = 0.f;
  for (int l = 0; l < L; ++l) acc = fmaf(es[cw * L + l], a[(size_t)l * T], acc);
  y[((size_t)b * C + c0 + cw) * T + t] = acc;
}
__global__ __launch_bounds__(256) void bmm_ct_mfma_kernel(const float* __restrict__ enc, const float* __restrict__ ali, int C, int L,
// ... 164 lines not shown
  __syncthreads();
  float s = 0.f;
  for (int l = threadIdx.x; l < L; l += 256) {
    const float e = expf(sm[l] - mx);
    sm[l] = e;
    s += e;
  }
  red[threadIdx.x] = s;
  __syncthreads();
  for (int o = 128; o > 0; o >>= 1) {
    if (threadIdx.x < o) red[threadIdx.x] += red[threadIdx.x + o];
    __syncthreads();
  }
  const float inv = 1.f / red[0];
  for (int l = threadIdx.x; l < L; l += 256) ali[((size_t)b * L + l) * T + t] = sm[l] * inv;
}
int launch_alignment(const float* dur, int B, int L, int T, float* ali, hipStream_t st) {
  hipLaunchKernelGGL(alignment_kernel, dim3(T, B), dim3(256), L * sizeof(float), st, dur, L, T, ali);
  STY_LAUNCH_CHECK();
  return STY_OK;
}

__global__ void embedding_bwd_kernel(const int64_t* __restrict__ tok, const float* __restrict__ g, int L, int H,
                                     int ntok, float scale, float* __restrict__ demb) {
  const int l = blockIdx.x * blockDim.x + threadIdx.x;
  const int c = blockIdx.y, b = blockIdx.z;
  if (l >= L) return;
  int64_t t = tok[(size_t)b * L + l];
  if (t < 0 || t >= ntok) t = 0;
  atomicAdd(&demb[(size_t)t * H + c], g[((size_t)b * H + c) * L + l] * scale);
}
int launch_embedding_bwd(const int64_t* tokens, const float* g, int B, int L, int H, int ntok, float scale, float* demb,
                         hipStream_t st) {
  hipLaunchKernelGGL(embedding_bwd_kernel, dim3(cdiv(L, 64), H, B), dim3(64), 0, st, tokens, g, L, H, ntok, scale, demb);
  STY_LAUNCH_CHECK();
  return STY_OK;
}
__global__ __launch_bounds__(64) void bmm_ct_bwd_kernel(const float* __restrict__ g, const float* __restrict__ ali, int C,
                                                        int L, int T, float* __restrict__ denc) {
  const int l = blockIdx.x, c = blockIdx.y, b = blockIdx.z, lane = threadIdx.x;
  const float* gr = g + ((size_t)b * C + c) * T;
  const float* ar = ali + ((size_t)b * L + l) * T;
  float acc = 0.f;
  for (int t = lane; t < T; t += 64) acc = fmaf(gr[t], ar[t], acc);
  for (int o = 32; o > 0; o >>= 1) acc += __shfl_xor(acc, o);
  if (lane == 0) denc[((size_t)b * C + c) * L + l] += acc;
}
constexpr int BMM_TT = 64, BMM_P = BMM_TT + 1;
__global__ __launch_bounds__(256) void bmm_ct_bwd_mfma_kernel(const float* __restrict__ g, const float* __restrict__ ali, int C,
                                                             int L, int T, float* __restrict__ denc) {
  __shared__ float gs[32 * BMM_P], as[128 * BMM_P];
  const int tid = threadIdx.x, lane = tid & 63, wave = tid >> 6, l31 = lane & 31, hi = lane >> 5;
  const int c0 = blockIdx.x * 32, b = blockIdx.y;
  const float* gb = g + ((size_t)b * C + c0) * T;
  const float* ab = ali + (size_t)b * L * T;
  f32x16 acc;
#pragma unroll
  for (int r = 0; r < 16; ++r) acc[r] = 0.f;
  const bool v4 = (T & 3) == 0;
  float4 nx[10];
  auto fetch = [&](int t0) {
#pragma unroll
    for (int i = 0; i < 10; ++i) {
      const int e = tid + 256 * i, r = e >> 4, tt = (e & 15) * 4, t = t0 + tt;
      const bool isg = r < 32;
      const int row = isg ? r : r - 32;
// ... 190 lines not shown
```

### stylish_tts_amd/csrc/model.h

```cpp
#pragma once
#include <string>
#include <unordered_map>
#include <vector>

#include "sty_common.h"

namespace sty {

struct Param {
  const float* p = nullptr;
  std::vector<int64_t> shape;
};

int convnext32_ntiles(int T);
int launch_convnext32(const Cnx32Args& a, int B, int pass, hipStream_t st);
int launch_pack_w2a(const float* w2, const float* b2, const float* grn_beta, int C, float* w2a, float* b2eff,
                    hipStream_t st);
int launch_attention(const AttnArgs& a, int B, int DH, hipStream_t st);
int launch_rope_n(float* q, float* k, int B, int H, int DH, int L, int d, hipStream_t st, float sgn = 1.0f);
int launch_style_expand(const float* style, int B, int S, int L, float* y, hipStream_t st);
int launch_row_sum_add(const float* src, int rows, int L, float* dst, hipStream_t st);
int launch_wn_dw_bwd(const float* dw, const float* g, const float* v, int C, int K, float* dg, float* dv, hipStream_t st);
int launch_dur_post_bwd(const float* d, const float* mask, const float* go, int B, int NC, int L, float* gd, hipStream_t st);
int trainer_duration_forward(struct Trainer* t, int B, int L, const int64_t* texts, const int64_t* lengths, const float* style,
                             float* out, void* ws, size_t ws_bytes, hipStream_t st, size_t* need);
int trainer_duration_backward(struct Trainer* t, const float* d_out, float* d_style, hipStream_t st);
int launch_scale_copy(const float* x, float a, size_t n, float* y, hipStream_t st);
int launch_mask_mul(float* x, const float* mask, int B, int C, int T, hipStream_t st);
int launch_wn_dw(const float* g, const float* v, int C, int K, float* w, hipStream_t st);
int launch_pad_time(const float* x, int rows, int T, int pad, float* y, hipStream_t st);
int launch_dur_post(const float* d, const float* mask, int B, int NC, int L, float* out, hipStream_t st);
int launch_rope(float* q, float* k, int B, int H, int DH, int L, int d, const float* theta4, hipStream_t st);
int launch_rope_copy(const float* qs, const float* ks, float* q, float* k, int B, int H, int DH, int L, int d,
                     const float* theta4, hipStream_t st);
int source_workspace_floats(int B, int T);
int launch_source(int B, int T, const float* pitch, const float* voiced, const float* noise, uint64_t seed,
                  const float* lin_w, const float* lin_b, float* prior, float* ws, hipStream_t st);
int launch_stft64(int B, int N, const float* wave, const float* br, const float* bi, float* spec, float* phase,
                  hipStream_t st);
int launch_istft64(int B, int F, const float* logamp, const float* real, const float* imag, const float* bbr,
                   const float* bbi, float* audio, hipStream_t st);
void build_stft64_bases(float* out);
size_t mel_workspace_floats(int B, int N, int n_fft, int hop, int n_mels);
int launch_mel(int B, int N, const float* audio, int n_fft, int win, int hop, int n_mels, int sample_rate, float mean,
               float std_, float* mel, float* energy, float* ws, hipStream_t st);
size_t multispec_workspace_floats(int B, int N, int n_fft, int hop);
size_t acoustic_loss_workspace_floats(int B, int N);
int launch_acoustic_loss(int B, int N, const float* audio_gt, const float* audio_pred, float w_mel, float w_phase,
                         float* losses_out, float* d_pred, float* ws, hipStream_t st);
int specdisc_run(const sty_specdisc_params* p, int B, int H, int W, size_t sb, size_t sh, const float* target,
                 const float* pred, float* scores_t, float* scores_p, float gen_scale, float* gen_loss, float* d_pred,
                 float disc_scale, float* disc_loss, const sty_specdisc_grads* grads, int compute_bf16, void* workspace,
                 size_t ws_bytes, hipStream_t st, size_t* need);
struct AcousticGan {
  const sty_specdisc_params* p[3] = {nullptr, nullptr, nullptr};
  const sty_specdisc_grads* g[3] = {nullptr, nullptr, nullptr};
  float w_gen = 1.f, disc_scale = 1.f;
  float* out = nullptr;
  int bf16 = 0;
  void* ws = nullptr;
  size_t ws_bytes = 0;
};
size_t acoustic_gan_workspace_bytes(int B, int N, int with_grads);
int launch_acoustic_loss_gan(int B, int N, const float* audio_gt, const float* audio_pred, float w_mel, float w_phase,
                             float* losses_out, float* d_pred, float* ws, const AcousticGan* gan, hipStream_t st);
int launch_multispec_single(int B, int N, const float* audio, int n_fft, int hop, int sample_rate, float* mag,
                            float* phase, float* fft_mag, float* ws, hipStream_t st);

struct Bump {
  char* base = nullptr;
  size_t off = 0, cap = 0;
  bool overflow = false;
  template <typename T>
  T* take(size_t n) {
    off = align_up(off, 256);
    T* p = base ? reinterpret_cast<T*>(base + off) : nullptr;
    off += n * sizeof(T);
    if (base && off > cap) overflow = true;
    return p;
  }
};

enum PackKind { PK_CONV, PK_CONV_WN, PK_CONV_GLU, PK_W2A, PK_CONV2D_SN, PK_DW2D_SN, PK_DGRAD, PK_DGRAD2D };
int launch_dwconv2d_s2(const float* x, const float* w9, const float* bias, int B, int C, int H, int W, float* y,
                       hipStream_t st, __bf16* y16_lrelu = nullptr);
int launch_avgpool2(const float* x, int BC, int H, int W, float scale, float* y, hipStream_t st, __bf16* y16 = nullptr);
int launch_pool_fc(const float* x, int B, int C, int n, int count, const float* W, const float* bvec, int S,
                   float* out, hipStream_t st);
struct PackJob {
  PackKind kind;
  const float *w = nullptr, *g = nullptr, *v = nullptr, *bias = nullptr, *extra = nullptr;
  int Cout = 0, Cin = 0, K = 1, CinP = 0, CoutP = 0, KH = 1;
  float* wp = nullptr;
  float* bp = nullptr;
  float* scratch = nullptr;
  float* scratch2 = nullptr;
};

struct AdaFc {
  int idx = -1;
  int C = 0;
  size_t off = 0;
};

struct ConvNeXt {
  int C = 0;
  const float *dw_w = nullptr, *dw_b = nullptr, *b1 = nullptr, *alpha = nullptr, *grn_gamma = nullptr;
  AdaFc norm;
  PackedConv pw1, pw2;
  const float* w2a = nullptr;
  const float* w1p = nullptr;
  const float *w1_raw = nullptr, *w2_raw = nullptr;
};

struct ResBlock32 {
  PackedConv c1[3], c2[3];
  AdaFc n1[3], n2[3];
  const float *a1[3], *a2[3];
};

struct Conformer {
  AdaFc ff1n, ff2n, attn_n, conv_n, post_n;
  PackedConv ff1a, ff1b, ff2a, ff2b, to_q, to_kv, to_out, pw1, pw2;
  const float *dw_w, *dw_b, *bn_w, *bn_b, *bn_rm, *bn_rv;
};

struct VocoderPlan {
  PackedConv amp_input_conv;
  const float *amp_norm_w, *amp_norm_b;
  Conformer conf;
  std::vector<ConvNeXt> amp_convnext;
  PackedConv upconv[3];
  ConvNeXt upblock[3];
  const float *lin_w, *lin_b;
  const float *stft_fr, *stft_fi, *stft_br, *stft_bi;
  PackedConv amp_prior_conv, phase_prior_conv, phase_input_conv, amp_output_conv, real_conv, imag_conv;
  ResBlock32 amp_prior_block, phase_prior_block;
  const float *phase_norm_w, *phase_norm_b, *amp_fln_w, *amp_fln_b, *phase_fln_w, *phase_fln_b;
  std::vector<ConvNeXt> phase_convnext;
  int hidden = 256;
};

struct TextEncLayer {
  PackedConv q, k, v, o, f1, f2;
  const float *n1g, *n1b, *n2g, *n2b;
};
struct TextEncPlan {
  const float* emb = nullptr;
  int tokens = 0, H = 0;
  PackedConv pre[3], proj, proj_m;
  const float *pre_g[3], *pre_b[3];
  std::vector<TextEncLayer> layers;
  float theta[4];
};

struct DecBlock {
  int Cin = 0, Cout = 0;
  PackedConv c1, c2, sc;
  bool has_sc = false;
  AdaFc n1, n2;
};
struct DecoderPlan {
  DecBlock encode, decode[4];
  PackedConv asr_res;
  float* fnv_w = nullptr;
  const float *f0_g, *f0_v, *f0_b, *n_g, *n_v, *n_b, *v_g, *v_v, *v_b;
};

struct ProsodyLayer {
  PackedConv q, k, v, o, f1, f2, proj;
  AdaFc n1, n2;
};
struct DurationPlan {
  AdaFc qn, kn;
  PackedConv cq, ck, cv, co, post, proj;
  const float *dw_g = nullptr, *dw_v = nullptr, *dw_b = nullptr;
  std::vector<ConvNeXt> cnx;
// ... 58 lines not shown
  sty::MultiJob* mj_dev[5] = {nullptr, nullptr, nullptr, nullptr, nullptr};
  int* mj_blk_dev[5] = {nullptr, nullptr, nullptr, nullptr, nullptr};
  int mj_nblk[5] = {0, 0, 0, 0, 0};
  int* mj_blk1_dev = nullptr;
  int mj_nblk1 = 0, mj_nsn = 0;
  bool mj_ready = false;
  size_t seg_job_split = 0;
  int seg_blk_split = 0;
  sty_grad_hook grad_hook = nullptr;
  void* grad_hook_user = nullptr;
  sty_train_opts topts = {0, 0, 0, 0, 0.1f, 0u, 0.2f, 0, 0};
  struct sty::Trainer* trainer = nullptr;
};

#include <functional>
#include <unordered_set>
namespace sty {
int launch_pro_bwd(int mode, const float* u, int Cu, int cu0, const float* x, int B, int C, int T, const float* pa,
                   const float* ps, int pC, int pc0, const float* alpha, const float* mask, float* dx, int accumulate,
                   float* dpa, float* dps, float* dalpha, hipStream_t st);
int launch_adain_fold_bwd(const float* da, const float* ds, const float* mean, const float* rstd, const float* gb, int B,
                          int C, int T, float* dgb, float* c0, float* c1, hipStream_t st);
int launch_row_axpb(const float* x, const float* c0, const float* c1, int rows, int T, float* dx, hipStream_t st);
int launch_pro_bwd_adain(const void* u, int uh, const void* x, int xh, int B, int C, int T, const float* pa, const float* ps,
                         const float* alpha, const float* mean, const float* rstd, const float* gb, void* dx, int dh,
                         int accumulate, float* dgb, float* dalpha, int hw, hipStream_t st, const void* dsrc = nullptr);
int launch_adain_stats(const double* part, int nseg, int rows, int T, float eps, float* mean, float* rstd,
                       hipStream_t st);
int launch_cast_f32_to_16(const float* x, size_t n, void* y16, hipStream_t st);
int launch_cast_16_to_f32(const void* x16, size_t n, float* y, hipStream_t st);
bool chan_ln32_eligible(int B, int C, int T, int relu);
int launch_chan_ln_bwd(const float* x, const float* dy, const float* y, int B, int C, int T, float eps, int ada,
                       const float* w, const float* gb, int relu, const float* out_mask, float* dx, int accumulate,
                       float* mu_tmp, float* r_tmp, float* dgb, float* dw, float* db, hipStream_t st, int h16 = 0);
int launch_grn_bwd(const double* part, int nseg, const float* gamma, const float* ds, int B, int C4, float* coef,
                   float* dgamma, hipStream_t st);
int launch_act_fwd(int kind, const float* x, const float* alpha, int B, int C, int T, float* y, hipStream_t st);
int launch_act_bwd(int kind, const float* x, const float* dy, const float* alpha, int B, int C, int T, float* dx,
                   int accumulate, float* dalpha, hipStream_t st);
int launch_row_scale_add(const float* src, const float* coef, float k, int rows, int T, float* dst, hipStream_t st);
int launch_dwconv_fwd(const float* x, const float* w, const float* bias, int B, int C, int T, int K, int pad, float* y,
                      hipStream_t st);
size_t dwconv_bwd_scratch_floats(int B, int C, int T, int K);
int launch_dwconv_bwd(const float* x, const float* dy, const float* w, int B, int C, int T, int K, int pad, float* dx,
                      int accumulate, float* dw, float* db, float* scratch, hipStream_t st, const float* dx_src = nullptr,
                      int x16 = 0, int dy16 = 0);
int launch_bn_eval_fwd(const float* x, const float* w, const float* b, const float* rm, const float* rv, float eps,
                       int B, int C, int T, float* y, hipStream_t st);
int launch_bn_eval_bwd(const float* x, const float* dy, const float* w, const float* rm, const float* rv, float eps,
                       int B, int C, int T, float* dx, float* dw, float* db, hipStream_t st);
size_t bias_grad_scratch_floats(int B, int C, int T);
int launch_bias_grad(const float* g, const float* mask, int B, int C, int T, int shuffle, float scale, float* db,
                     float* scratch, hipStream_t st);
int launch_style_fc_bwd(const void* descs_dev, int nlayers, int B, int style_dim, const float* style,
                        const float* dgb_base, float* dstyle, hipStream_t st);
int launch_istft64_bwd(int B, int F, const float* audio, const float* daudio, const float* logamp, const float* real,
                       const float* imag, const float* bbr, const float* bbi, float* dlogamp, float* dreal,
                       float* dimag, hipStream_t st);
size_t wgrad_partial_floats(const PackedConv& w, int B, int T);
struct WgReduceDefer;
WgReduceDefer* wgrad_defer_create();
void wgrad_defer_destroy(WgReduceDefer* d);
WgReduceDefer* wgrad_defer_set(WgReduceDefer* d);
size_t wgrad_defer_pending(const WgReduceDefer* d);
int wgrad_defer_flush(WgReduceDefer* d, int site, hipStream_t st);
inline bool wgrad_fuses_bias(const PackedConv& w) { return w.K <= 12; }
int launch_conv1d_wgrad(const ConvArgs& fwd, const float* g, const float* gmask, float scale, float* gwp,
// ... 71 lines not shown
```

### stylish_tts_amd/csrc/norms.hip

```cpp
#include "sty_common.h"

namespace sty {

__global__ __launch_bounds__(256) void style_fc_kernel(const StyleFcDesc* __restrict__ descs, int style_dim,
                                                       const float* __restrict__ style, float* __restrict__ gb_base,
                                                       int B) {
  __shared__ float s[256];
  const StyleFcDesc d = descs[blockIdx.x];
  const int b = blockIdx.y;
  for (int i = threadIdx.x; i < style_dim; i += 256) s[i] = style[(size_t)b * style_dim + i];
  __syncthreads();
  for (int j = threadIdx.x; j < d.n; j += 256) {
    const float* w = d.W + (size_t)j * style_dim;
    float acc = 0.f;
    for (int k = 0; k < style_dim; ++k) acc = fmaf(s[k], w[k], acc);
    gb_base[d.off * B + (size_t)b * d.n + j] = acc + d.b[j];
  }
}

int launch_style_fc(const StyleFcDesc* descs_dev, int nlayers, int B, int style_dim, const float* style,
                    float* gb_base, hipStream_t st) {
  if (style_dim > 256) {
    set_error("style_fc: style_dim %d > 256", style_dim);
    return STY_EINVAL;
// ... 181 lines not shown
  const float mean = (red[0][lane] + red[1][lane] + red[2][lane] + red[3][lane]) * (1.0f / C);
  __syncthreads();
  float q = 0.f;
#pragma unroll
  for (int i = 0; i < CPT; ++i) {
    const float d = v[i] - mean;
    q += d * d;
  }
  red[wave][lane] = q;
  __syncthreads();
  const float rstd = 1.0f / sqrtf((red[0][lane] + red[1][lane] + red[2][lane] + red[3][lane]) * (1.0f / C) + eps);
  if (!in) return;
  const float om = out_mask ? out_mask[(size_t)b * T + t] : 1.f;
  float* o = y + (size_t)b * C * T + t;
#pragma unroll
  for (int i = 0; i < CPT; ++i) {
    const int c = wave + 4 * i;
    float sc, sh;
    if (ada) {
      sc = 1.f + gb[(size_t)b * 2 * C + c];
      sh = gb[(size_t)b * 2 * C + C + c];
    } else {
      sc = w[c];
      sh = bvec[c];
    }
    float r = (v[i] - mean) * rstd * sc + sh;
    if (relu) r = fmaxf(r, 0.f);
    o[(size_t)c * T] = r * om;
  }
}

int launch_chan_layernorm(const float* x, float* y, int B, int C, int T, float eps, int ada, const float* w,
                          const float* bvec, const float* gb, int relu, const float* out_mask, hipStream_t st) {
  const dim3 grid(cdiv(T, 64), B);
#define STY_LN_CASE(CPT)                                                                                          \
  case 4 * CPT:                                                                                                    \
    hipLaunchKernelGGL(chan_layernorm_reg_kernel<CPT>, grid, dim3(256), 0, st, x, y, T, eps, ada, w, bvec, gb, relu, \
                       out_mask);                                                                                  \
    break;
  switch (C) {
    STY_LN_CASE(8)
    STY_LN_CASE(16)
    STY_LN_CASE(32)
    STY_LN_CASE(64)
    STY_LN_CASE(80)
    STY_LN_CASE(96)
    STY_LN_CASE(128)
    default:
      hipLaunchKernelGGL(chan_layernorm_kernel, grid, dim3(64), 0, st, x, y, C, T, eps, ada, w, bvec, gb, relu,
                         out_mask);
  }
#undef STY_LN_CASE
  STY_LAUNCH_CHECK();
  return STY_OK;
}

template <int KT>
__global__ __launch_bounds__(256) void dwconv_adaln_kernel(const float* __restrict__ x, const float* __restrict__ w,
                                                           const float* __restrict__ bias, int C, int T, int K,
                                                           float eps, const float* __restrict__ gb,
                                                           float* __restrict__ y, int TT) {
  extern __shared__ __attribute__((aligned(16))) float u[];
  float* smean = u + (size_t)C * TT;
  float* srstd = smean + TT;
  float* part = srstd + TT;
  const int b = blockIdx.y, t0 = blockIdx.x * TT;
// ... 115 lines not shown
```

### stylish_tts_amd/csrc/sty_common.h

```cpp
#pragma once
#include <hip/hip_runtime.h>
#include <stdint.h>
#include <stdio.h>

#include "../../include/stylish_hip.h"

namespace sty {

void set_error(const char* fmt, ...);
int hip_fail(hipError_t e, const char* what);

#define STY_HIP(expr)                                      \
  do {                                                     \
    hipError_t _e = (expr);                                \
    if (_e != hipSuccess) return sty::hip_fail(_e, #expr); \
  } while (0)

#define STY_LAUNCH_CHECK() STY_HIP(hipGetLastError())

extern thread_local const void* g_last_kernel;
template <class R, class... A>
inline const void* kernel_handle(R (*f)(A...)) {
  return reinterpret_cast<const void*>(f);
}
// ... 127 lines not shown
  int in_shuffle = 0;
  PackedConv w;
  int pro = PRO_NONE;
  const float* pa = nullptr;
  const float* ps = nullptr;
  const float* palpha = nullptr;
  const float* pbeta = nullptr;
  float ln_eps = 1e-6f;
  const float* mask = nullptr;
  int act = ACT_NONE;
  const float* act_alpha = nullptr;
  float out_scale = 1.f;
  const float* residual = nullptr;
  const float* out_mask = nullptr;
  int out_mask_post = 0;
  int shuffle = 1;
  int ln_out = 0;
  const float* ln_w = nullptr;
  const float* ln_b = nullptr;
  float* y = nullptr;
  float* y_split = nullptr;
  double* stat_part = nullptr;
  const __bf16* x16 = nullptr;
  const __bf16* g16 = nullptr;
  __bf16* y16 = nullptr;
  int y16_act = PRO_NONE;
  const float* up_g = nullptr;
  const __bf16* up_gate16 = nullptr;
  const float* up_mask = nullptr;
  float up_scale = 1.f;
  int up_H = 0;
  int xh = 0, yh = 0, rh = 0, gh = 0;
  int w_row = 0, w_tap = 0;
};
int launch_twin_cast(const float* x, const float* mask, int pro, int B, int C, int T, __bf16* y16, hipStream_t st);
bool wgradb16_eligible(const ConvArgs& fwd);
int launch_wgradb16(const ConvArgs& fwd, int nsplit, float* partial, int want_bias, hipStream_t st);

int launch_conv1d(const ConvArgs& a, hipStream_t st);
bool conv1d_reads_twin_only(const ConvArgs& a);
bool conv1d_has_up_stage(const ConvArgs& a);
bool conv32p_eligible(const ConvArgs& a);
int conv32p_stat_nseg(int T);
bool wgradb_eligible(const ConvArgs& fwd, bool gmask);
int launch_wgradb(const ConvArgs& ax, const ConvArgs& ag, int nsplit, float* partial, int want_bias, hipStream_t st);
int wgradb_chunks(const PackedConv& w, int B, int T, int dil);
bool wgradp32_eligible(const ConvArgs& fwd);
int wgradp32_chunks(const ConvArgs& fwd);
int launch_wgradp32(const ConvArgs& ax, const ConvArgs& ag, int nsplit, float* partial, int want_bias, hipStream_t st);
int wgrad_cnx_nsplit(int B, int T);
int launch_conv_wgrad_cnx(int x_wide, const void* wide, const float* narrow, int B, int T, float* gwp, float* partial,
                          float* gbias, hipStream_t st, int narrow16 = 0);
int wgrad_cnx_per_b(int B, int T);
int launch_wgrad_cnx(int x_wide, const void* wide, const float* narrow, int B, int T, float* partial, int want_bias,
                     hipStream_t st, int per_b = 0, int narrow16 = 0);
bool stem2d_eligible(const ConvArgs& a);
int launch_stem2d(const ConvArgs& a, hipStream_t st);
bool convk1_eligible(const ConvArgs& a);
int launch_convk1(const ConvArgs& a, hipStream_t st);
bool convp16_eligible(const ConvArgs& a);
bool convq_eligible(const ConvArgs& a);
int launch_convq(const ConvArgs& a, hipStream_t st);
int convp16_repack_range(const void* lo, const void* hi, hipStream_t st);
void convp16_forget_range(const void* lo, const void* hi);
int launch_convp16(const ConvArgs& a, hipStream_t st);
int launch_conv32p(const ConvArgs& a, hipStream_t st);

struct MultiJob {
  const float *p0 = nullptr, *p1 = nullptr, *p2 = nullptr, *p3 = nullptr, *p4 = nullptr;
  float *q0 = nullptr, *q1 = nullptr, *q2 = nullptr, *q3 = nullptr, *q4 = nullptr;
  int Cout = 0, Cin = 0, K = 1, CinP = 0, CoutP = 0, glu = 0, blk0 = 0, KH = 1;
  int blk1 = 0, pad = 0;
};
int launch_multi(int which, const MultiJob* jobs, const int* job_of_block, int nblocks, hipStream_t st, int blk_base = 0);
int launch_sn_unpack_multi(const MultiJob* jobs, const int* job_of_block, int nblocks, hipStream_t st);
int launch_sn_prep_multi(const MultiJob* jobs, int njobs, const int* job_of_row, int nrows, const int* job_of_blk1, int nblk1,
                         bool power_iter, bool pack, hipStream_t st);

int launch_pack_conv(const float* w, const float* g, const float* v, const float* bias, int Cout, int Cin, int K,
                     float* wp, float* bp, int CinP, int CoutP, hipStream_t st);

}

namespace sty {
int launch_pack_conv_glu(const float* w, const float* bias, int Cout, int Cin, int K, float* wp, float* bp, int CinP,
                         int CoutP, hipStream_t st);

struct StyleFcDesc {
  const float* W;
  const float* b;
  size_t off;
  int n;
  int pad;
};
int launch_style_fc(const StyleFcDesc* descs_dev, int nlayers, int B, int style_dim, const float* style,
                    float* gb_base, hipStream_t st);
struct StyleFcBwdDesc {
  const float* W;
  float* dW;
  float* db;
  size_t off;
  int n;
  int pad;
};
int row_stats_nseg(int T);
// ... 58 lines not shown
  int T, ntiles;
  int bf16 = 0;
  int out_bf16 = 0;
  int lean = 0;
  const void* wfrag = nullptr;
  float* gx = nullptr;
  int xn16 = 0;
  int gy16 = 0, gx16 = 0, gu16 = 0;
  int x16 = 0;
};
constexpr int CNX_BWD_FUSED_STRIDE = 248;
int convnext32_bwd_ntiles(int T, int fused);
constexpr size_t CNX_FRAG_HALFS = 3 * 4 * 2 * 64 * 8;
int launch_cnx_frag_pack(const float* w1p, const float* w2raw, const float* w1raw, void* wfrag, hipStream_t st);
int launch_cnx_m_finish(float* partial, int B, int SB, const float* w2raw, const float* scale, float* ds, float* gw2,
                        float* gb2, hipStream_t st);
int launch_cnx_dalpha(const float* w1raw, const float* b1, const float* alpha, const float* gw1, const float* gb1,
                      const float* scale, const float* ds, const float* coef, const double* part, int nseg, int B,
                      float* dalpha, hipStream_t st);
int launch_convnext32_bwd(const Cnx32BwdArgs& a, int B, int pass, hipStream_t st);
int launch_cnx_partial_sum(const double* part, int B, int C, int ntiles, int mode, float* out, hipStream_t st);

constexpr int W2A_MAXJ = 16;
struct W2aJobs {
  const float* w2[W2A_MAXJ];
  const float* b2[W2A_MAXJ];
  const float* gb[W2A_MAXJ];
  float* w2a[W2A_MAXJ];
  float* b2eff[W2A_MAXJ];
  int C[W2A_MAXJ];
  int n = 0;
};
int launch_pack_w2a_multi(const W2aJobs& jobs, hipStream_t st);
struct AttnArgs {
  const float* q;
  const float* k;
  const float* v;
  float* o;
  size_t qbs, kbs, vbs, obs;
  int T, H;
  float scale;
  const int64_t* lengths;
  float drop_p = 0.f;
  unsigned drop_seed = 0, drop_site = 0;
  float* lse = nullptr;
  int bf16 = 0;
};
bool attention16_eligible(const AttnArgs& a, int DH);
int launch_attention16(const AttnArgs& a, int B, hipStream_t st);
int launch_attention16_bwd(const AttnArgs& a, const float* dO, float* dQ, float* dK, float* dV, size_t dqbs, size_t dkbs,
                           size_t dvbs, size_t dobs, int B, float* ws, hipStream_t st);
}

#ifdef __HIPCC__
namespace sty {
__device__ __forceinline__ float sty_hash_u(unsigned seed, unsigned site, unsigned idx) {
  unsigned x = idx * 0x9E3779B1u + site * 0x85EBCA77u + seed * 0xC2B2AE3Du;
  x ^= x >> 16;
  x *= 0x7FEB352Du;
  x ^= x >> 15;
  x *= 0x846CA68Bu;
  x ^= x >> 16;
  return (float)(x >> 8) * (1.0f / 16777216.0f);
}
__device__ __forceinline__ void sty_unit_vec(float re, float im, float& c, float& s) {
  const float h2 = re * re + im * im;
  if (h2 > 0.f && h2 < 3.0e38f) {
    const float r = 1.0f / sqrtf(h2);
    c = re * r;
    s = im * r;
  } else {
    const float ph = atan2f(im, re);
    c = cosf(ph);
    s = sinf(ph);
  }
}
static __device__ __attribute__((noinline)) float sty_sinf_slow(float x) { return sinf(x); }
__device__ __forceinline__ float sty_sinf(float x) {
  if (__builtin_expect(fabsf(x) > 8192.0f, 0)) return sty_sinf_slow(x);
  const float kf = rintf(x * 0.636619772f);
  const int k = (int)kf;
  float r = fmaf(-kf, 1.57079637050628662109375f, x);
  r = fmaf(-kf, -4.37113900018624283e-8f, r);
  r = fmaf(-kf, -1.71512449e-15f, r);
  const float r2 = r * r;
  const float ps = fmaf(r2, fmaf(r2, -1.9515295891e-4f, 8.3321608736e-3f), -1.6666654611e-1f);
  const float s = fmaf(r * r2, ps, r);
  const float pc = fmaf(r2, fmaf(r2, 2.443315711809948e-5f, -1.388731625493765e-3f), 4.166664568298827e-2f);
  const float c = fmaf(r2 * r2, pc, fmaf(r2, -0.5f, 1.0f));
  const float res = (k & 1) ? c : s;
  return (k & 2) ? -res : res;
}
__device__ __forceinline__ float sty_sin2_fast(float x) {
  const float kf = rintf(x * 0.636619772f);
  float r = fmaf(-kf, 1.57079637050628662109375f, x);
  r = fmaf(-kf, -4.37113900018624283e-8f, r);
// ... 113 lines not shown
```

### stylish_tts_amd/csrc/train.hip

```cpp
#include <stdlib.h>
#include <string.h>

#include <map>
#include <memory>
#include <unordered_map>

#include "model.h"

namespace sty {

struct Trainer {
  sty_model* m = nullptr;
  hipStream_t st = nullptr;
  int B = 0, T = 0;
  Bump ws;
  int rc = STY_OK;
  float* gb = nullptr;
  float* dgb = nullptr;
  const float* style = nullptr;
  float* audio = nullptr;
  std::vector<std::function<void()>> tape;
  std::unordered_map<const float*, float*> gmap;
  std::unordered_set<const float*> nograd;
  float* scratch_param = nullptr;
// ... 77 lines not shown
  std::unordered_map<const float*, LazyMask> lazy_mask;
  bool mask_pending(const float* act) const { return !lazy_mask.empty() && lazy_mask.count(act) != 0; }
  void mask_flush(const float* act) {
    auto it = lazy_mask.find(act);
    if (it == lazy_mask.end()) return;
    const LazyMask z = it->second;
    lazy_mask.erase(it);
    if (live())
      chk(launch_pro_bwd(PRO_MASK, z.src, z.C, 0, z.src, B, z.C, z.n, nullptr, nullptr, z.C, 0, nullptr, z.mask, z.dst, 0,
                         nullptr, nullptr, nullptr, st));
  }
  struct PendUp {
    const float* g;
    const float* mask;
    float scale;
    int BC, C, H, W, n;
  };
  std::unordered_map<const float*, PendUp> pend_up;
  void up_apply(const float* src, const PendUp& u) {
    const bool gated = gate_pending(src);
    if (gated) ungated.erase(src);
    float* gs = G(src, (size_t)u.BC * u.n);
    __bf16* g16 = twins_on() && tw_want.count(src) && u.n % 4 == 0 ? take<__bf16>((size_t)u.BC * u.n) : nullptr;
    if (g16) tw_g[gs] = std::make_pair(g16, u.mask);
    if (live()) chk(launch_avgpool2_bwd(u.g, u.BC, u.H, u.W, u.scale, gs, gated ? src : nullptr, st, g16, u.mask, u.C));
  }
  void up_flush(const float* act) {
    auto it = pend_up.find(act);
    if (it == pend_up.end()) return;
    const PendUp u = it->second;
    pend_up.erase(it);
    up_apply(act, u);
  }
  void grad_sets_clear() {
    g_twin_only.clear();
    g_no_fp32.clear();
    lazy_mask.clear();
    pend_up.clear();
  }
  ~Trainer() {
    wgrad_defer_destroy(defer);
    for (hipEvent_t e : evs) (void)hipEventDestroy(e);
    if (d_style_done) (void)hipEventDestroy(d_style_done);
    if (st2) (void)hipStreamDestroy(st2);
  }
  hipEvent_t next_event() {
    if (ev_used == evs.size()) {
      hipEvent_t e = nullptr;
      hipError_t r = hipEventCreateWithFlags(&e, hipEventDisableTiming);
      if (r != hipSuccess) rc = hip_fail(r, "event");
      evs.push_back(e);
    }
    return evs[ev_used++];
  }
  void side_begin() {
    ev_used = 0;
    side_reads.clear();
    side_dirty = false;
    const bool on = side_on && !single_stream_mode();
    side_partial = on && side_need ? take<float>(side_need) : nullptr;
    wg_base = defer_on && wg_sum ? take<float>(wg_sum) : nullptr;
    wg_off = 0;
    flush_site = 0;
    after_reduce.clear();
    if (on && !st2 && live()) {
      int least = 0, greatest = 0;
      (void)hipDeviceGetStreamPriorityRange(&least, &greatest);
      hipError_t r = hipStreamCreateWithPriority(&st2, hipStreamNonBlocking, least);
      if (r != hipSuccess) rc = hip_fail(r, "side stream");
    }
  }
// ... 138 lines not shown
    return scratch_param;
  }

  ConvArgs base(const PackedConv& w, const float* x, int Tt, float* y) {
    ConvArgs a;
    a.x[0] = x;
    a.xc[0] = w.Cin;
    a.nsrc = 1;
    a.B = B;
    a.T = Tt;
    a.w = w;
    a.pad = (w.K - 1) / 2;
    a.y = y;
    a.bf16 = m->topts.compute_bf16;
    return a;
  }

  void conv(const ConvArgs& a0) {
    ConvArgs a = a0;
    a.bf16 = m->topts.compute_bf16;
    a.xh = is16(a.x[0]);
    a.yh = is16(a.y);
    a.rh = is16(a.residual);
    if (a.nsrc > 1 && (is16(a.x[1]) || is16(a.x[2]))) {
      set_error("training: a bf16-stored tensor as source 1 / 2 of a channel-concatenated conv");
      rc = STY_ESTATE;
      return;
    }
    const size_t pn = wgrad_partial_floats(a.w, B, a.T);
    side_need = pn > side_need ? pn : side_need;
    wg_need(pn);
    if (live()) chk(launch_conv1d(a, st));
    ConvArgs f = a;
    tape.push_back([this, f]() { conv_bwd(f); });
  }
  void conv_bwd(const ConvArgs& f) {
    const PackedConv& w = f.w;
    const int Tt = f.T;
    const size_t ny = (size_t)B * w.Cout * Tt;
    float* gY = G(f.y, ny);
    float* gR = nullptr;
    if (f.residual && wants(f.residual)) {
      if (!gmap.count(f.residual) && !(f.out_mask && f.out_mask_post) && f.shuffle <= 1)
        gmap[f.residual] = gY;
      else
        gR = G(f.residual, ny);
    }
    float* gX[3] = {nullptr, nullptr, nullptr};
    int accX[3] = {1, 1, 1};
    bool any = false;
    const float* gX_src = nullptr;
    if (f.nsrc == 1 && f.pro == PRO_AFFINE_SNAKE && Tt % 8 == 0 && wants(f.x[0]) && !side_reads.empty()) {
      auto ia = adain_of.find(f.pa);
      auto ig = gmap.find(f.x[0]);
      if (ia != adain_of.end() && ia->second.x == f.x[0] && ia->second.s == f.ps && !*ia->second.done && ig != gmap.end() &&
          side_reads.count(ig->second) && !is16(ig->second) && (ungated.empty() || !ungated.count(f.x[0]))) {
        gX_src = ig->second;
        gX[0] = take<float>((size_t)B * f.xc[0] * Tt);
        gmap[f.x[0]] = gX[0];
        accX[0] = 1;
        any = true;
      }
    }
    for (int i = 0; i < f.nsrc; ++i)
      if (wants(f.x[i]) && !(i == 0 && gX_src)) {
        gX[i] = Gw(f.x[i], (size_t)B * f.xc[i] * Tt, accX[i]);
        any = true;
      }
    for (int i = 1; i < f.nsrc; ++i)
      for (int j = 0; j < i; ++j)
        if (gX[i] && gX[i] == gX[j]) accX[i] = 1;
    if (side_ready())
      for (int i = 0; i < f.nsrc; ++i)
// ... 6 lines not shown
      auto it = adain_of.find(f.pa);
      if (it != adain_of.end() && it->second.x == f.x[0] && it->second.s == f.ps && !*it->second.done) fuse = &it->second;
    }
    if (any && fuse) {
      dal = PG(f.palpha, w.Cin);
    } else if (any) {
      if (f.pro == PRO_AFFINE_SNAKE || f.pro == PRO_AFFINE_LRELU || f.pro == PRO_AFFINE) {
        int dummy;
        dpa = Gw(f.pa, (size_t)B * w.Cin, dummy);
        dps = Gw(f.ps, (size_t)B * w.Cin, dummy);
      } else if (f.pro == PRO_SCALE) {
        int dummy;
        dpa = Gw(f.pa, (size_t)B * w.Cin, dummy);
      }
      if (f.pro == PRO_AFFINE_SNAKE) dal = PG(f.palpha, w.Cin);
    }
    const size_t mark = ws.off;
    const float* gmask = f.out_mask;
    if (gR && live()) {
      if (f.out_mask && f.out_mask_post)
        chk(launch_pro_bwd(PRO_MASK, gY, w.Cout, 0, gY, B, w.Cout, Tt, nullptr, nullptr, w.Cout, 0, nullptr, f.out_mask,
                           gR, 1, nullptr, nullptr, nullptr, st));
      else
        chk(launch_row_scale_add(gY, nullptr, 1.0f, B * w.Cout, Tt, gR, st));
    }
    bool bias_done = false;
    float* gbias = w.bias ? PGpacked(w.bias) : nullptr;
    if (m->topts.frozen) {
      bias_done = true;
    } else if (side_ready()) {
      float* sp = deferring() ? wg_take(wgrad_partial_floats(w, B, Tt)) : side_partial;
      float* gwp = PGpacked(w.wp);
      const float osc = f.out_scale;
      side_push(gY, [=](hipStream_t s) { chk(launch_conv1d_wgrad(f, gY, gmask, osc, gwp, sp, gbias, nullptr, s)); });
      bias_done = wgrad_fuses_bias(w);
    } else {
      const size_t pn = wgrad_partial_floats(w, B, Tt);
      float* partial = deferring() ? wg_take(pn) : take<float>(pn);
      DeferScope ds(this);
      if (live()) chk(launch_conv1d_wgrad(f, gY, gmask, f.out_scale, PGpacked(w.wp), partial, gbias, &bias_done, st));
    }
    if (w.bias && !bias_done) {
      float* bs = take<float>(bias_grad_scratch_floats(B, w.Cout, Tt));
      if (live()) chk(launch_bias_grad(gY, gmask, B, w.Cout, Tt, f.shuffle, f.out_scale, PGpacked(w.bias), bs, st));
    }
    if (any) {
      auto it = m->dgrad.find(w.wp);
      if (it == m->dgrad.end()) {
        set_error("training: no input-gradient weights for a conv (model not finalized for training?)");
        rc = STY_ESTATE;
        return;
      }
      const bool u16 = f.xh && f.nsrc == 1 && act16_on();
      float* U = take_act((size_t)B * w.Cin * Tt, u16);
      struct UGuard {
        Trainer* t;
        float* U;
        size_t mark;
        ~UGuard() {
          t->half_.erase(U);
          t->ws.off = mark;
        }
      } u_guard{this, U, mark};
      ConvArgs d;
      d.x[0] = gY;
      d.xc[0] = w.Cout;
      d.nsrc = 1;
      d.B = B;
      d.T = Tt;
      d.w = it->second;
      d.dil = f.dil;
      d.bf16 = f.bf16;
      d.pad = (w.K - 1) * f.dil - f.pad;
      d.out_scale = f.out_scale;
      d.in_shuffle = f.shuffle > 1 ? f.shuffle : 0;
      if (gmask) {
        d.pro = PRO_MASK;
        d.mask = gmask;
      }
      d.y = U;
      d.yh = u16;
      d.xh = is16(gY);
      if (f.nsrc == 1 && (f.pro == PRO_NONE || f.pro == PRO_MASK) && gX[0] != gY) {
        d.y = gX[0];
        d.yh = is16(gX[0]);
        d.rh = d.yh;
        d.residual = accX[0] ? gX[0] : nullptr;
        if (f.pro == PRO_MASK) {
          d.out_mask = f.mask;
          d.out_mask_post = 0;
        }
        if (live()) chk(launch_conv1d(d, st));
        ws.off = mark;
        return;
      }
      if (live()) chk(launch_conv1d(d, st));
      if (fuse) {
        *fuse->done = true;
        if (live())
          chk(launch_pro_bwd_adain(U, u16, f.x[0], f.xh, B, w.Cin, Tt, f.pa, f.ps, f.palpha, fuse->mean, fuse->rstd, fuse->gbl,
                                   gX[0], is16(gX[0]), accX[0], fuse->dgl, dal, f.bf16 ? 1 : 0, st, gX_src));
        half_.erase(U);
        ws.off = mark;
        return;
      }
      if (gX_src) {
        set_error("training: out-of-place prologue backward planned without the fused kernel");
        rc = STY_ESTATE;
        return;
      }
      if (u16 || f.xh) {
        half_.erase(U);
        set_error("training: bf16-stored conv input without the fused prologue backward");
        rc = STY_ESTATE;
        return;
      }
      int c0 = 0;
      for (int i = 0; i < f.nsrc; ++i) {
        if (gX[i] && live())
          chk(launch_pro_bwd(f.pro | (f.bf16 ? 0x100 : 0), U, w.Cin, c0, f.x[i], B, f.xc[i], Tt, f.pa, f.ps, w.Cin, c0, f.palpha, f.mask, gX[i],
                             accX[i], dpa, dps, dal, st));
        c0 += f.xc[i];
      }
    }
    ws.off = mark;
  }

  float* act(int kind, const float* x, const float* alpha, int C, int Tt) {
    float* y = take<float>((size_t)B * C * Tt);
    if (live()) chk(launch_act_fwd(kind, x, alpha, B, C, Tt, y, st));
    tape.push_back([=]() {
      const int Cin = kind == ACT_GLU ? 2 * C : C;
      float* gY = G(y, (size_t)B * C * Tt);
      int acc = 1;
      float* gX = Gw(x, (size_t)B * Cin * Tt, acc);
      float* dal = kind == ACT_SNAKE ? PG(alpha, C) : nullptr;
      if (live()) chk(launch_act_bwd(kind, x, gY, alpha, B, C, Tt, gX, acc, dal, st));
    });
    return y;
  }

  unsigned drop_site = 0;
  bool dropout_on() const { return m->topts.dropout_seed != 0; }
  float* dropout(const float* x, float p, int C, int Tt, const float* residual, size_t group = 1) {
    const size_t n = (size_t)B * C * Tt;
    float* y = take<float>(n);
    const unsigned seed = m->topts.dropout_seed, site = drop_site++;
    if (live()) chk(launch_dropout(x, residual, n, p, seed, site, y, 0, st, group));
    tape.push_back([=]() {
      float* gY = G(y, n);
      if (residual && wants(residual)) {
        if (!gmap.count(residual)) {
          gmap[residual] = gY;
        } else {
          float* gR = G(residual, n);
          if (live()) chk(launch_row_scale_add(gY, nullptr, 1.0f, 1, (int)n, gR, st));
        }
      }
      int acc = 1;
      float* gX = Gw(x, n, acc);
      if (gX == gY) {
        set_error("dropout backward: aliased gradient buffers");
        rc = STY_ESTATE;
        return;
      }
      if (live()) chk(launch_dropout(gY, nullptr, n, p, seed, site, gX, acc, st, group));
    });
    return y;
  }

  float* layernorm(const float* x, int C, int Tt, float eps, const AdaFc* fc, const float* w, const float* bvec,
                   int relu = 0, const float* omask = nullptr) {
    float* y = take<float>((size_t)B * C * Tt);
    const float* gbl = fc ? gbp(*fc) : nullptr;
    float* dgl = fc ? dgbp(*fc) : nullptr;
    if (live()) chk(launch_chan_layernorm(x, y, B, C, Tt, eps, fc ? 1 : 0, w, bvec, gbl, relu, omask, st));
    const bool ln32 = grad16_on() && chan_ln32_eligible(B, C, Tt, relu);
    if (ln32 && grad16_stream_on()) g16_ok.insert(y);
    tape.push_back([=]() {
      const size_t nel = (size_t)B * C * Tt;
      float* gY = ln32 ? G16(y, nel) : G(y, nel);
      int acc = 1, h16 = is16(gY) ? 2 : 0;
      float* gX;
      if (ln32 && g16_ok.count(x) && !gmap.count(x)) {
        gX = take_act(nel, true);
        gmap[x] = gX;
        acc = 0;
        h16 |= 4;
      } else {
        gX = Gw(x, nel, acc);
      }
      const size_t mark = ws.off;
      float* mu = take<float>((size_t)B * Tt);
      float* r = take<float>((size_t)B * Tt);
      float* dw = fc ? nullptr : PG(w, C);
      float* db = fc ? nullptr : PG(bvec, C);
      if (live())
        chk(launch_chan_ln_bwd(x, gY, y, B, C, Tt, eps, fc ? 1 : 0, w, gbl, relu, omask, gX, acc, mu, r, dgl, dw, db, st, h16));
      ws.off = mark;
    });
    return y;
  }

  struct AdainInfo {
    const float *x, *s, *mean, *rstd, *gbl;
    float* dgl;
    std::shared_ptr<bool> done;
  };
  std::unordered_map<const float*, AdainInfo> adain_of;
  void adain(const float* x, int C, int Tt, const AdaFc& fc, float*& a, float*& s, const double* have_part = nullptr,
             int have_nseg = 0) {
    a = take<float>((size_t)B * C);
    s = take<float>((size_t)B * C);
    float* mean = take<float>((size_t)B * C);
    float* rstd = take<float>((size_t)B * C);
    const int nseg = have_part ? have_nseg : row_stats_nseg(Tt);
    const double* part = have_part;
    if (!have_part) {
      double* p2 = take<double>((size_t)B * C * nseg * 2);
      if (live()) chk(launch_row_stats(x, B * C, Tt, p2, st));
      part = p2;
    }
    if (live()) {
      chk(launch_adain_finalize(part, nseg, gbp(fc), B, C, Tt, 1e-5f, a, s, st));
      chk(launch_adain_stats(part, nseg, B * C, Tt, 1e-5f, mean, rstd, st));
    }
    const float* gbl = gbp(fc);
    float* dgl = dgbp(fc);
    float* aa = a;
    float* ss = s;
    auto done = std::make_shared<bool>(false);
// ... 481 lines not shown
    at.k = k;
    at.v = v;
    at.o = o;
    at.qbs = at.kbs = at.vbs = at.obs = (size_t)Hd * L;
    at.T = L;
    at.H = heads;
    at.scale = 1.0f / sqrtf((float)(Hd / heads));
    at.lengths = lengths;
    const float pa = p_attn >= 0.f ? p_attn : m->topts.text_dropout;
    if (dropout_on() && pa > 0.f) {
      at.drop_p = pa;
      at.drop_seed = m->topts.dropout_seed;
      at.drop_site = drop_site++;
    }
    if (attention_bwd_mfma_dh(Hd / heads)) at.lse = take<float>((size_t)B * heads * L);
    if (live()) chk(launch_attention(at, B, Hd / heads, st));
    tape.push_back([=]() {
      float* gO = G(o, n);
      int aq = 1, ak = 1, av = 1;
      const bool ow = attention_bwd_can_overwrite(at, Hd / heads);
      float* gQ = ow ? Gw(q, n, aq) : G(q, n);
      float* gK = ow ? Gw(k, n, ak) : G(k, n);
      float* gV = ow ? Gw(v, n, av) : G(v, n);
      const size_t mark = ws.off;
      float* w2 = take<float>(attention_bwd_ws_floats(B, heads, L));
      if (live())
        chk(launch_attention_bwd(at, gO, gQ, gK, gV, at.qbs, at.kbs, at.vbs, at.obs, B, Hd / heads, w2, st,
                                 (aq ? 0 : 1) | (ak ? 0 : 2) | (av ? 0 : 4)));
      ws.off = mark;
    });
    return o;
  }

  float* text_encoder(const int64_t* tokens, const int64_t* lengths, int L) {
    const TextEncPlan& t = m->te;
    const int H = t.H;
    const size_t n = (size_t)B * H * L;
    float* mask = take<float>((size_t)B * L);
    float* x0 = take<float>(n);
    const float esc = sqrtf((float)H);
    if (live()) {
      chk(launch_length_mask(lengths, B, L, mask, st));
      chk(launch_embedding(tokens, t.emb, B, L, H, t.tokens, esc, x0, st));
    }
    nograd.insert(mask);
    {
      const float* emb = t.emb;
      const int ntok = t.tokens;
      tape.push_back([=]() {
        float* g = G(x0, n);
        if (live()) chk(launch_embedding_bwd(tokens, g, B, L, H, ntok, esc, PG(emb, (size_t)ntok * H), st));
      });
    }
    const float* h = x0;
    for (int i = 0; i < 3; ++i) {
      float* h1 = take<float>(n);
      ConvArgs a = base(t.pre[i], h, L, h1);
      a.pro = PRO_MASK;
      a.mask = mask;
      conv(a);
      h = layernorm(h1, H, L, 1e-4f, nullptr, t.pre_g[i], t.pre_b[i], 1, nullptr);
      if (dropout_on()) h = dropout(h, 0.5f, H, L, nullptr);
    }
    float* x = take<float>(n);
    ConvArgs pj = base(t.proj, h, L, x);
    pj.residual = x0;
    pj.out_mask = mask;
    pj.out_mask_post = 1;
    conv(pj);
    for (const TextEncLayer& l : t.layers) {
      float* q = take<float>(n);
      float* k = take<float>(n);
      float* v = take<float>(n);
      ConvArgs aq = base(l.q, x, L, q);
      aq.pro = PRO_MASK;
      aq.mask = mask;
      conv(aq);
      aq.w = l.k;
      aq.y = k;
      conv(aq);
      aq.w = l.v;
      aq.y = v;
      conv(aq);
      float* qr = take<float>(n);
      float* kr = take<float>(n);
      if (live()) chk(launch_rope_copy(q, k, qr, kr, B, 8, H / 8, L, 8, t.theta, st));
      {
        const float* th = t.theta;
        tape.push_back([=]() {
          float* gqr = G(qr, n);
          float* gkr = G(kr, n);
          if (live()) chk(launch_rope_signed(gqr, gkr, B, 8, H / 8, L, 8, th, -1.0f, st));
          if (!alias_grad(q, gqr)) {
            float* gq = G(q, n);
            if (live()) chk(launch_row_scale_add(gqr, nullptr, 1.0f, B * H, L, gq, st));
          }
          if (!alias_grad(k, gkr)) {
            float* gk = G(k, n);
            if (live()) chk(launch_row_scale_add(gkr, nullptr, 1.0f, B * H, L, gk, st));
          }
        });
      }
      float* o = attention3(qr, kr, v, H, L, lengths);
      const float pd = m->topts.text_dropout;
      const bool dr = dropout_on() && pd > 0.f;
      float* h1 = take<float>(n);
      ConvArgs ao = base(l.o, o, L, h1);
      if (dr) {
        conv(ao);
        h1 = dropout(h1, pd, H, L, x);
      } else {
        ao.residual = x;
        conv(ao);
      }
      float* x1 = layernorm(h1, H, L, 1e-4f, nullptr, l.n1g, l.n1b);
      const int Fc = l.f1.Cout;
      float* f0 = take<float>((size_t)B * Fc * L);
      ConvArgs f1 = base(l.f1, x1, L, f0);
      f1.pro = PRO_MASK;
      f1.mask = mask;
      conv(f1);
      float* fr = act(ACT_RELU, f0, nullptr, Fc, L);
      if (dr) fr = dropout(fr, pd, Fc, L, nullptr);
      float* h2 = take<float>(n);
      ConvArgs f2 = base(l.f2, fr, L, h2);
      f2.pro = PRO_MASK;
      f2.mask = mask;
      f2.out_mask = mask;
      if (dr) {
        conv(f2);
        h2 = dropout(h2, pd, H, L, x1);
      } else {
        f2.residual = x1;
        conv(f2);
      }
      x = layernorm(h2, H, L, 1e-4f, nullptr, l.n2g, l.n2b, 0, mask);
    }
    float* mu = take<float>((size_t)B * t.proj_m.Cout * L);
    ConvArgs pm = base(t.proj_m, x, L, mu);
    pm.out_mask = mask;
    pm.out_mask_post = 1;
    conv(pm);
    return mu;
  }

  float* concat(const float* const* src, const int* ch, int nsrc, int Tt) {
    int Ctot = 0;
    for (int i = 0; i < nsrc; ++i) Ctot += ch[i];
    float* y = take<float>((size_t)B * Ctot * Tt);
    if (live()) chk(launch_concat(src, ch, nsrc, B, Tt, y, st));
    std::vector<const float*> sv(src, src + nsrc);
    std::vector<int> cv(ch, ch + nsrc);
    tape.push_back([=]() {
      float* gY = G(y, (size_t)B * Ctot * Tt);
      int c0 = 0;
      for (int i = 0; i < nsrc; ++i) {
        if (wants(sv[i])) {
          float* gs = G(sv[i], (size_t)B * cv[i] * Tt);
          if (live()) chk(launch_slice_add(gY, Ctot, c0, B, cv[i], Tt, gs, st));
        }
        c0 += cv[i];
      }
    });
    return y;
// ... 1095 lines not shown
      if (e != hipSuccess) rc = hip_fail(e, "seed copy");
    }
    if (!d_mel) nograd.insert(mel_in);
    if (d_mel == reinterpret_cast<float*>(2)) d_mel = nullptr;
    for (auto it = tape.rbegin(); it != tape.rend(); ++it) {
      (*it)();
      if (rc != STY_OK) break;
    }
    side_join();
    if (rc != STY_OK) return;
    style_fc_backward();
    if (live() && d_mel) {
      float* gm = G(mel_in, (size_t)B * m->voc.amp_input_conv.Cin * T);
      hipError_t e = hipMemcpyAsync(d_mel, gm, (size_t)B * m->voc.amp_input_conv.Cin * T * sizeof(float),
                                    hipMemcpyDeviceToDevice, st);
      if (e != hipSuccess) rc = hip_fail(e, "d_mel copy");
    }
  }
};

int trainer_speech_forward(Trainer* t, const sty_speech_io* io, void* ws, size_t ws_bytes, hipStream_t st,
                           size_t* need) {
  t->st = st;
  t->B = io->B;
  t->rc = STY_OK;
  t->ws = Bump();
  t->dry = need != nullptr;
  t->ws.base = need ? reinterpret_cast<char*>(size_t(1) << 30) : (char*)ws;
  t->ws.cap = need ? (size_t(1) << 46) : ws_bytes;
  t->peak = 0;
  t->begin(io->style);
  const int inter = t->m->te.proj_m.Cout ? t->m->te.proj_m.Cout : 128;
  float* mu = t->text_encoder(io->texts, io->text_lengths, io->L);
  t->tape.push_back([t]() {
    t->style_fc_backward();
    if (t->on_segment && t->live()) {
      t->side_join();
      if (t->rc == STY_OK) t->on_segment(0);
    } else if (t->live()) {
      t->side_reduce_nowait();
    }
  });
  t->style_fc(reinterpret_cast<hipStream_t>(io->style_stream));
  float* asr = t->expand(mu, io->alignment, inter, io->L, io->T);
  float* mel = t->decoder(asr, io->pitch, io->energy, io->voiced, io->T);
  if (mel) {
    sty_vocoder_io v = io->voc_taps;
    v.B = io->B;
    v.T = io->T;
    v.mel = mel;
    v.style = io->style;
    v.pitch = io->denormal_pitch;
    v.voiced = io->voiced;
    v.noise = io->noise;
    v.prior_override = io->prior_override;
    v.seed = io->seed;
    v.audio = io->audio;
    t->forward(v, false);
  }
  if (need) {
    t->backward(nullptr, reinterpret_cast<float*>(2), nullptr);
    *need = align_up(t->peak, 256) + (64 << 20);
    t->tape.clear();
    return t->rc;
  }
  if (t->ws.overflow) {
// ... 306 lines not shown
```

### stylish_tts_amd/csrc/wgrad.hip

```cpp
#include <stdlib.h>
#include <string.h>

#include <vector>

#include "conv_stage.h"

namespace sty {

constexpr int WG_MODE = 0;
constexpr int WG_TW = 128;
constexpr int WG_TARGET = 1024;
static inline int wg_target(bool bf16) { return bf16 ? 768 : WG_TARGET; }
constexpr float WG_PARTIAL_FRAC = 0.25f;
constexpr int WG_MIN_WGS = 128;
static inline int wg_cap_partial(int nsplit, const PackedConv& w, int B, int T, bool bf16, int tiles = 0) {
  if (!bf16) return nsplit;
  const double operands = (double)B * T * (w.Cin + w.Cout), plane = (double)w.K * w.CinP * w.CoutP;
  int cap = (int)(WG_PARTIAL_FRAC * operands / plane);
  if (tiles > 0 && cap < cdiv(WG_MIN_WGS, tiles)) cap = cdiv(WG_MIN_WGS, tiles);
  if (cap < 1) cap = 1;
  if (cap >= 8) cap &= ~7;
  return nsplit < cap ? nsplit : cap;
}

// ... 1260 lines not shown
  STY_LAUNCH_CHECK();
  return STY_OK;
}

__global__ __launch_bounds__(256) void pack_conv_multi_kernel(const MultiJob* __restrict__ jobs,
                                                              const int* __restrict__ job_of_block) {
  __shared__ float red[256];
  const MultiJob j = jobs[job_of_block[blockIdx.x]];
  const int co = blockIdx.x - j.blk0;
  const int n = j.Cin * j.K;
  int cp = co;
  if (j.glu) {
    const int Ch = j.Cout / 2;
    const int half = co >= Ch, c = half ? co - Ch : co;
    cp = (c >> 5) * 64 + half * 32 + (c & 31);
  }
  float scale = 1.f;
  const float* src = j.p0;
  if (!src) {
    src = j.p2;
    float s = 0.f;
    for (int i = threadIdx.x; i < n; i += 256) {
      const float x = src[(size_t)co * n + i];
      s += x * x;
    }
    red[threadIdx.x] = s;
    __syncthreads();
    for (int o = 128; o > 0; o >>= 1) {
      if (threadIdx.x < o) red[threadIdx.x] += red[threadIdx.x + o];
      __syncthreads();
    }
    scale = j.p1[co] / sqrtf(red[0]);
  }
  for (int i = threadIdx.x; i < n; i += 256) {
    const int ci = i / j.K, k = i % j.K;
    j.q0[((size_t)k * j.CinP + ci) * j.CoutP + cp] = src[(size_t)co * n + i] * scale;
  }
  if (threadIdx.x == 0 && j.q1) j.q1[cp] = j.p3 ? j.p3[co] : 0.f;
}
__global__ __launch_bounds__(256) void pack_dgrad_multi_kernel(const MultiJob* __restrict__ jobs,
                                                               const int* __restrict__ job_of_block) {
  const MultiJob j = jobs[job_of_block[blockIdx.x]];
  const size_t i = (size_t)(blockIdx.x - j.blk0) * 256 + threadIdx.x;
  if (j.glu == 2) {
    const size_t n2 = (size_t)j.K * j.KH * j.Cout * j.Cin;
    if (i >= n2) return;
    const int ci = (int)(i % j.Cin);
    const int co = (int)((i / j.Cin) % j.Cout);
    const int kh = (int)((i / ((size_t)j.Cin * j.Cout)) % j.KH);
    const int kw = (int)(i / ((size_t)j.Cin * j.Cout * j.KH));
    j.q0[((size_t)kw * j.blk1 + kh * j.Cout + co) * j.pad + ci] =
        j.p0[((size_t)(j.K - 1 - kw) * j.CinP + (j.KH - 1 - kh) * j.Cin + ci) * j.CoutP + co];
    return;
  }
  const size_t n = (size_t)j.K * j.CinP * j.CoutP;
  if (i >= n) return;
  const int ci = (int)(i % j.CinP);
  const int co = (int)((i / j.CinP) % j.CoutP);
  const int kd = (int)(i / ((size_t)j.CinP * j.CoutP));
  j.q0[i] = j.p0[((size_t)(j.K - 1 - kd) * j.CinP + ci) * j.CoutP + co];
}
__global__ __launch_bounds__(256) void unpack_grad_multi_kernel(const MultiJob* __restrict__ jobs,
                                                                const int* __restrict__ job_of_block, int blk_base) {
  __shared__ float r1[256], r2[256];
  const int blk = (int)blockIdx.x + blk_base;
  const MultiJob j = jobs[job_of_block[blk]];
  const int co = blk - j.blk0;
  const int n = j.Cin * j.K;
  const int cp = co;
  if (threadIdx.x == 0 && j.q3 && j.p3) j.q3[co] += j.p3[cp];
  if (!j.p2) {
    if (!j.q0) return;
    for (int i = threadIdx.x; i < n; i += 256) {
      const int ci = i / j.K, k = i % j.K;
      j.q0[(size_t)co * n + i] += j.p0[((size_t)k * j.CinP + ci) * j.CoutP + cp];
    }
    return;
  }
  if (!j.q1 || !j.q2) return;
  float dot = 0.f, nn = 0.f;
  for (int i = threadIdx.x; i < n; i += 256) {
    const int ci = i / j.K, k = i % j.K;
    const float v = j.p2[(size_t)co * n + i];
    dot = fmaf(j.p0[((size_t)k * j.CinP + ci) * j.CoutP + cp], v, dot);
    nn = fmaf(v, v, nn);
  }
  r1[threadIdx.x] = dot;
  r2[threadIdx.x] = nn;
  __syncthreads();
  for (int o = 128; o > 0; o >>= 1) {
    if (threadIdx.x < o) {
      r1[threadIdx.x] += r1[threadIdx.x + o];
      r2[threadIdx.x] += r2[threadIdx.x + o];
    }
    __syncthreads();
  }
  const float norm = sqrtf(r2[0]), d = r1[0], gg = j.p1[co];
  if (threadIdx.x == 0) j.q1[co] += d / norm;
  for (int i = threadIdx.x; i < n; i += 256) {
    const int ci = i / j.K, k = i % j.K;
    const float v = j.p2[(size_t)co * n + i];
    j.q2[(size_t)co * n + i] += gg / norm * (j.p0[((size_t)k * j.CinP + ci) * j.CoutP + cp] - v * d / (norm * norm));
  }
}
int launch_multi(int which, const MultiJob* jobs, const int* job_of_block, int nblocks, hipStream_t st, int blk_base) {
  if (nblocks <= 0) return STY_OK;
  if (which == 0)
    hipLaunchKernelGGL(pack_conv_multi_kernel, dim3(nblocks), dim3(256), 0, st, jobs, job_of_block);
  else if (which == 1)
    hipLaunchKernelGGL(pack_dgrad_multi_kernel, dim3(nblocks), dim3(256), 0, st, jobs, job_of_block);
  else
    hipLaunchKernelGGL(unpack_grad_multi_kernel, dim3(nblocks), dim3(256), 0, st, jobs, job_of_block, blk_base);
  STY_LAUNCH_CHECK();
  return STY_OK;
}

__global__ void pack_dgrad2d_kernel(const float* __restrict__ wp, int KW, int KH, int Cin, int Cout, int CinP,
                                    int CoutP, int CinPd, int CoutPd, float* __restrict__ wd) {
  const size_t i = (size_t)blockIdx.x * 256 + threadIdx.x;
  const size_t n = (size_t)KW * KH * Cout * Cin;
  if (i >= n) return;
  const int ci = (int)(i % Cin);
  const int co = (int)((i / Cin) % Cout);
  const int kh = (int)((i / ((size_t)Cin * Cout)) % KH);
  const int kw = (int)(i / ((size_t)Cin * Cout * KH));
  wd[((size_t)kw * CinPd + kh * Cout + co) * CoutPd + ci] =
      wp[((size_t)(KW - 1 - kw) * CinP + (KH - 1 - kh) * Cin + ci) * CoutP + co];
}
int launch_pack_dgrad2d(const float* wp, int KW, int KH, int Cin, int Cout, int CinP, int CoutP, int CinPd, int CoutPd,
                        float* wd, hipStream_t st) {
  const size_t n = (size_t)KW * KH * Cout * Cin;
  hipLaunchKernelGGL(pack_dgrad2d_kernel, dim3((unsigned)((n + 255) / 256)), dim3(256), 0, st, wp, KW, KH, Cin, Cout,
                     CinP, CoutP, CinPd, CoutPd, wd);
  STY_LAUNCH_CHECK();
  return STY_OK;
// ... 89 lines not shown
```

### stylish_tts_amd/modules.py

```python
import ctypes as C

import torch

from . import lib as L
from .manifest import (DEFAULT_CFG, N3_CFG, duration_predictor_manifest, multi_generator_manifest,
                       pitch_energy_predictor_manifest, pitch_style_encoder_manifest, speech_predictor_manifest,
                       style_encoder_manifest)


class DecoderPrediction:
    def __init__(self, *, audio, magnitude, phase):
        self.audio = audio
        self.magnitude = magnitude
        self.phase = phase


_BUFFER_SUFFIXES = ("running_mean", "running_var", "num_batches_tracked", "weight_u", "weight_v")


class _Node(torch.nn.Module):
    """Anonymous container so that dotted state_dict keys come out identical to the reference's."""


def _register(root, key, tensor, as_buffer):
# ... 399 lines not shown
        B, T = self._train_shape
        d_audio = _f32(d_audio, dev)
        d_mel = torch.zeros(B, self.cfg["gen_input_dim"], T, device=dev) if want_mel else None
        d_style = torch.zeros(B, self.cfg["style_dim"], device=dev) if want_style else None
        st = C.c_void_p(torch.cuda.current_stream(dev).cuda_stream)
        L.check(lib.sty_vocoder_bwd(self._handle, L.ptr(d_audio), L.ptr(d_mel), L.ptr(d_style), st))
        return d_mel, d_style


    def block_forward_backward(self, kind, prefix, x, style, gy, compute_bf16=False):
        dev = style.device
        self._train = True
        self._tape_id += 1
        lib = self._ensure(dev)
        self.set_train_opts(compute_bf16=bool(compute_bf16))
        x, style, gy = _f32(x.detach(), dev), _f32(style.detach(), dev), _f32(gy.detach(), dev)
        B, Cc, T = x.shape
        y, gx = torch.empty_like(x), torch.empty_like(x)
        d_style = torch.zeros(B, self.cfg["style_dim"], device=dev)
        need = C.c_size_t()
        L.check(lib.sty_block_train_workspace_bytes(self._handle, kind.encode(), prefix.encode(), B, Cc, T, C.byref(need)))
        ws = torch.empty(need.value, dtype=torch.uint8, device=dev)
        st = C.c_void_p(torch.cuda.current_stream(dev).cuda_stream)
        L.check(lib.sty_block_fwd_bwd(self._handle, kind.encode(), prefix.encode(), B, Cc, T, L.ptr(x), L.ptr(style),
                                      L.ptr(gy), L.ptr(y), L.ptr(gx), L.ptr(d_style), L.ptr(ws), ws.numel(), st))
        return y, gx, d_style

    def prepare_train(self, device):
        self._train = True
        lib = self._ensure(device)
        L.check(lib.sty_speech_prepare_train(self._handle, C.c_void_p(torch.cuda.current_stream(device).cuda_stream)))

    def forward_train(self, texts, text_lengths, alignment, pitch, energy, voiced, style, denormal_pitch, *, noise=None,
                      seed=0, prior_override=None, style_stream=None):
        _check_speech_shapes(texts, text_lengths, alignment, pitch, energy, voiced, style, denormal_pitch, noise,
                             self.cfg["style_dim"])
        dev = style.device
        self._train = True
        self._tape_id += 1
        lib = self._ensure(dev)
        B, Lt = texts.shape
        T = pitch.shape[1]
        io = L.SpeechIO()
        io.B, io.L, io.T = B, Lt, T
        keep = [texts.to(dev, torch.int64).contiguous(), text_lengths.to(dev, torch.int64).contiguous()]
        io.texts, io.text_lengths = keep[0].data_ptr(), keep[1].data_ptr()
        for name, t in (("alignment", alignment), ("pitch", pitch), ("energy", energy), ("voiced", voiced),
                        ("style", style), ("denormal_pitch", denormal_pitch), ("noise", noise),
                        ("prior_override", prior_override)):
            if t is not None:
                t = _f32(t.detach(), dev)
                keep.append(t)
                setattr(io, name, t.data_ptr())
        io.seed = int(seed)
        io.style_stream = style_stream.cuda_stream if style_stream is not None else None
        audio = torch.empty(B, 1, 300 * T, dtype=torch.float32, device=dev)
        io.audio = audio.data_ptr()
        need = C.c_size_t()
        L.check(lib.sty_speech_train_workspace_bytes(self._handle, B, Lt, T, C.byref(need)))
        if getattr(self, "_train_ws", None) is None or self._train_ws.numel() < need.value:
            self._train_ws = torch.empty(need.value, dtype=torch.uint8, device=dev)
        self._train_keep = keep
        self._train_shape = (B, T)
        st = C.c_void_p(torch.cuda.current_stream(dev).cuda_stream)
        L.check(lib.sty_speech_fwd_train(self._handle, C.byref(io), C.c_void_p(self._train_ws.data_ptr()),
                                         self._train_ws.numel(), st))
        return audio

    def backward(self, d_audio, want_style=True, want_energy=True, want_pitch=False):
        lib = L.load()
        dev = d_audio.device
        B, T = self._train_shape
        d_audio = _f32(d_audio, dev)
        d_style = torch.zeros(B, self.cfg["style_dim"], device=dev) if want_style else None
        d_energy = torch.zeros(B, T, device=dev) if want_energy else None
        d_pitch = torch.zeros(B, T, device=dev) if want_pitch else None
        st = C.c_void_p(torch.cuda.current_stream(dev).cuda_stream)
        L.check(lib.sty_speech_bwd_pe(self._handle, L.ptr(d_audio), L.ptr(d_style), L.ptr(d_pitch), L.ptr(d_energy), st))
        return (d_style, d_energy, d_pitch) if want_pitch else (d_style, d_energy)

    def wait_d_style(self, stream):
        L.check(L.load().sty_speech_d_style_ready(self._handle, C.c_void_p(stream.cuda_stream)))


class _VocoderFn(torch.autograd.Function):

    @staticmethod
    def forward(ctx, anchor, mel, style, module, kw):
# ... 340 lines not shown
```

Before: 381,600 frames/s.

## Fuse text-encoder QKV convs, RoPE into attention, and dropout into conv epilogues

Packs the q/k/v 1x1 convs of each text-encoder attention layer into one concatenated weight so training runs a single conv. RoPE is applied inside the small-T attention forward and backward kernels instead of separate rope copy and grad kernels. ReLU and dropout are fused into conv epilogues where supported, and a dropped second output is added to the LN backward. It also adds profiling scopes and a text-encoding tap. The text encoder is a small share of the total work, so fewer launches and less memory traffic there may barely show in end-to-end throughput, and the new paths carry correctness risk.

```diff
diff --git a/stylish_tts_amd/csrc/api.hip b/stylish_tts_amd/csrc/api.hip
--- a/stylish_tts_amd/csrc/api.hip
+++ b/stylish_tts_amd/csrc/api.hip
@@ -100,6 +100,7 @@
   sty_model* m;
   bool dry;
   bool ok = true;
+  bool fwd_only = false;
 
   const Param* get(const std::string& key, std::initializer_list<int64_t> shape = {}) {
     if (dry) m->requested.push_back(key);
@@ -156,9 +157,10 @@
       j.CoutP = pc.CoutP;
       j.wp = wp;
       j.bp = bp;
+      j.fwd_only = fwd_only;
       m->jobs.push_back(j);
     }
-    if (m->train_enabled) {
+    if (m->train_enabled && !fwd_only) {
       if (glu) {
         PackedConv pl = pc;
         pl.CoutP = (int)align_up(pc.Cout, 32);
@@ -210,6 +212,54 @@
       m->jobs.push_back(j);
       m->dgrad[pc.wp] = d;
     }
+  }
+
+  PackedConv conv_cat3(const std::string* names) {
+    PackedConv pc;
+    const Param* w[3];
+    const float* b[3];
+    for (int i = 0; i < 3; ++i) {
+      auto iw = m->params.find(names[i] + ".weight");
+      auto ib = m->params.find(names[i] + ".bias");
+      if (iw == m->params.end() || ib == m->params.end()) return pc;
+      w[i] = &iw->second;
+      b[i] = ib->second.p;
+    }
+    for (int i = 0; i < 3; ++i)
+      if (w[i]->shape.size() < 2 || w[i]->shape[0] != w[0]->shape[0] || w[i]->shape[1] != w[0]->shape[1] ||
+          (w[i]->shape.size() > 2 && w[i]->shape[2] != 1)) {
+        if (ok) m->missing = names[i] + ".weight (q / k / v convs of differing shapes)";
+        ok = false;
+        return pc;
+      }
+    const int C = (int)w[0]->shape[0];
+    pc.Cout = 3 * C;
+    pc.Cin = (int)w[0]->shape[1];
+    pc.K = 1;
+    pc.CinP = (int)align_up(pc.Cin, CI_CHUNK);
+    pc.CoutP = (int)align_up(pc.Cout, 32);
+    float* wp = m->ab.take<float>((size_t)pc.CinP * pc.CoutP);
+    float* bp = m->ab.take<float>(pc.CoutP);
+    pc.wp = wp;
+    pc.bias = bp;
+    if (!dry)
+      for (int i = 0; i < 3; ++i) {
+        PackJob j;
+        j.kind = PK_CONV;
+        j.w = w[i]->p;
+        j.bias = b[i];
+        j.Cout = C;
+        j.Cin = pc.Cin;
+        j.K = 1;
+        j.CinP = pc.CinP;
+        j.CoutP = pc.CoutP;
+        j.ld = pc.CoutP;
+        j.wp = wp + (size_t)i * C;
+        j.bp = bp + (size_t)i * C;
+        m->jobs.push_back(j);
+      }
+    add_dgrad(pc);
+    return pc;
   }
 
   AdaFc fc(const std::string& name, int C) {
@@ -391,9 +441,14 @@
     for (int i = 0; has(p + "encoder.attn_layers." + std::to_string(i) + ".conv_q.weight"); ++i) {
       const std::string si = std::to_string(i);
       TextEncLayer l;
-      l.q = conv(p + "encoder.attn_layers." + si + ".conv_q");
-      l.k = conv(p + "encoder.attn_layers." + si + ".conv_k");
-      l.v = conv(p + "encoder.attn_layers." + si + ".conv_v");
+      const std::string qkv[3] = {p + "encoder.attn_layers." + si + ".conv_q", p + "encoder.attn_layers." + si + ".conv_k",
+                                  p + "encoder.attn_layers." + si + ".conv_v"};
+      fwd_only = m->train_enabled;
+      l.q = conv(qkv[0]);
+      l.k = conv(qkv[1]);
+      l.v = conv(qkv[2]);
+      fwd_only = false;
+      if (m->train_enabled) l.qkv = conv_cat3(qkv);
       l.o = conv(p + "encoder.attn_layers." + si + ".conv_o");
       l.n1g = ptr(p + "encoder.norm_layers_1." + si + ".gamma", {t.H});
       l.n1b = ptr(p + "encoder.norm_layers_1." + si + ".beta", {t.H});
@@ -1809,9 +1864,10 @@
       a.K = j.K;
       a.CinP = j.CinP;
       a.CoutP = j.CoutP;
+      a.ld = j.ld;
       a.glu = j.kind == PK_CONV_GLU;
       add(0, a, j.Cout);
-      if (m->garena && j.kind != PK_CONV_GLU) {
+      if (m->garena && j.kind != PK_CONV_GLU && !j.fwd_only) {
         MultiJob u;
         u.p0 = GA(j.wp);
         u.p1 = j.g;
@@ -1826,6 +1882,7 @@
         u.K = j.K;
         u.CinP = j.CinP;
         u.CoutP = j.CoutP;
+        u.ld = j.ld;
         if (u.q0 || (u.q1 && u.q2) || u.q3) add(2, u, j.Cout);
       }
     } else if (j.kind == PK_DGRAD) {
diff --git a/stylish_tts_amd/csrc/attn.hip b/stylish_tts_amd/csrc/attn.hip
--- a/stylish_tts_amd/csrc/attn.hip
+++ b/stylish_tts_amd/csrc/attn.hip
@@ -21,7 +21,21 @@
 
   float qreg[DH / 2];
 #pragma unroll
-  for (int c2 = 0; c2 < DH / 2; ++c2) qreg[c2] = qi < T ? qb[(size_t)(2 * c2 + hi) * T + qi] * a.scale : 0.f;
+  for (int c2 = 0; c2 < DH / 2; ++c2) qreg[c2] = qi < T ? qb[(size_t)(2 * c2 + hi) * T + qi] : 0.f;
+  const bool rope = DH == 16 && a.rope_d == 8;
+  if constexpr (DH == 16) {
+    if (rope) {
+      float xr[4];
+#pragma unroll
+      for (int c2 = 0; c2 < 4; ++c2)
+        xr[c2] = sty_rope8(qreg[c2], qreg[c2 ^ 2], 2 * c2 + hi, qi, a.rope_theta[0], a.rope_theta[1], a.rope_theta[2],
+                           a.rope_theta[3], 1.0f);
+#pragma unroll
+      for (int c2 = 0; c2 < 4; ++c2) qreg[c2] = xr[c2];
+    }
+  }
+#pragma unroll
+  for (int c2 = 0; c2 < DH / 2; ++c2) qreg[c2] *= a.scale;
 
   f32x16 oacc[DP / 32];
 #pragma unroll
@@ -36,7 +50,11 @@
     for (int e = tid; e < DH * 32; e += 256) {
       const int d = e >> 5, jj = e & 31;
       const int j = j0 + jj;
-      ks[d * LS + jj] = j < T ? kb[(size_t)d * T + j] : 0.f;
+      float kv = j < T ? kb[(size_t)d * T + j] : 0.f;
+      if (rope && d < 8 && j < T)
+        kv = sty_rope8(kv, kb[(size_t)(d ^ 4) * T + j], d, j, a.rope_theta[0], a.rope_theta[1], a.rope_theta[2], a.rope_theta[3],
+                       1.0f);
+      ks[d * LS + jj] = kv;
       vs[d * LS + jj] = j < T ? vb[(size_t)d * T + j] : 0.f;
     }
     if (DP > DH)
@@ -108,8 +126,13 @@
 }
 
 int launch_attention(const AttnArgs& a, int B, int DH, hipStream_t st) {
+  if (a.rope_d && !attention_rope_fused(a, DH)) {
+    set_error("attention: fused RoPE asked where the kernels have none (attention_rope_fused)");
+    return STY_EINVAL;
+  }
   if (attention16_eligible(a, DH)) return launch_attention16(a, B, st);
   dim3 grid(cdiv(a.T, 128), a.H, B);
+  ProfScope prof("attn_kernel", 4.0 * (double)B * a.H * DH * a.T * a.T, 16.0 * (double)B * a.H * DH * a.T, st);
   const bool drop = a.drop_p > 0.f;
   if (DH == 64 && !drop)
     hipLaunchKernelGGL((attn_kernel<64, false>), grid, dim3(256), 0, st, a);
@@ -132,7 +155,7 @@
 }
 
 __global__ void rope_kernel(const float* qs, const float* ks, float* q, float* k, int H, int DH, int L, int d, float t0, float t1, float t2, float t3,
-                            float sgn) {
+                            float sgn, size_t sbs, size_t dbs) {
   const int pos = blockIdx.x * blockDim.x + threadIdx.x;
   const int h = blockIdx.y, b = blockIdx.z;
   if (pos >= L) return;
@@ -141,9 +164,9 @@
   const float* src[2] = {qs, ks};
   float* ptr[2] = {q, k};
   for (int w = 0; w < 2; ++w) {
-    const size_t o = ((size_t)b * H + h) * DH * L + pos;
-    const float* sb_ = src[w] + o;
-    float* base = ptr[w] + o;
+    const size_t o = (size_t)h * DH * L + pos;
+    const float* sb_ = src[w] + (size_t)b * sbs + o;
+    float* base = ptr[w] + (size_t)b * dbs + o;
     float x[8];
     for (int i = 0; i < d; ++i) x[i] = sb_[(size_t)i * L];
     for (int i = 0; i < d; ++i) {
@@ -158,23 +181,37 @@
 
 int launch_rope_signed(float* q, float* k, int B, int H, int DH, int L, int d, const float* theta4, float sgn,
                        hipStream_t st) {
+  ProfScope prof("rope_kernel", 0.0, 16.0 * (double)B * H * DH * L, st);
   if (d != 8) {
     set_error("rope: only d == 8 built");
     return STY_EINVAL;
   }
   hipLaunchKernelGGL(rope_kernel, dim3(cdiv(L, 64), H, B), dim3(64), 0, st, q, k, q, k, H, DH, L, d, theta4[0], theta4[1],
-                     theta4[2], theta4[3], sgn);
+                     theta4[2], theta4[3], sgn, (size_t)H * DH * L, (size_t)H * DH * L);
   STY_LAUNCH_CHECK();
   return STY_OK;
 }
 int launch_rope_copy(const float* qs, const float* ks, float* q, float* k, int B, int H, int DH, int L, int d,
                      const float* theta4, hipStream_t st) {
+  ProfScope prof("rope_kernel", 0.0, 16.0 * (double)B * H * DH * L, st);
   if (d != 8) {
     set_error("rope: only d == 8 built");
     return STY_EINVAL;
   }
   hipLaunchKernelGGL(rope_kernel, dim3(cdiv(L, 64), H, B), dim3(64), 0, st, qs, ks, q, k, H, DH, L, d, theta4[0], theta4[1],
-                     theta4[2], theta4[3], 1.0f);
+                     theta4[2], theta4[3], 1.0f, (size_t)H * DH * L, (size_t)H * DH * L);
+  STY_LAUNCH_CHECK();
+  return STY_OK;
+}
+int launch_rope_strided(const float* qs, const float* ks, size_t sbs, float* q, float* k, size_t dbs, int B, int H, int DH, int L,
+                        int d, const float* theta4, float sgn, hipStream_t st) {
+  ProfScope prof("rope_kernel", 0.0, 16.0 * (double)B * H * DH * L, st);
+  if (d != 8 || qs == q || ks == k) {
+    set_error("rope: only d == 8, out of place, built");
+    return STY_EINVAL;
+  }
+  hipLaunchKernelGGL(rope_kernel, dim3(cdiv(L, 64), H, B), dim3(64), 0, st, qs, ks, q, k, H, DH, L, d, theta4[0], theta4[1],
+                     theta4[2], theta4[3], sgn, sbs, dbs);
   STY_LAUNCH_CHECK();
   return STY_OK;
 }
diff --git a/stylish_tts_amd/csrc/attn_bwd.hip b/stylish_tts_amd/csrc/attn_bwd.hip
--- a/stylish_tts_amd/csrc/attn_bwd.hip
+++ b/stylish_tts_amd/csrc/attn_bwd.hip
@@ -351,10 +351,18 @@
   const float* gb = dO + (size_t)b * dobs + ho;
   const float* ob = a.o + (size_t)b * a.obs + ho;
   const int len = a.lengths ? (int)a.lengths[b] : T;
+  const bool rope = a.rope_d == 8;
+  const float th0 = a.rope_theta[0], th1 = a.rope_theta[1], th2 = a.rope_theta[2], th3 = a.rope_theta[3];
   for (int e = tid; e < DH * T; e += 256) {
     const int d = e / T, t = e - d * T;
-    qs[d * TP + t] = qb[e] * a.scale;
-    ks[d * TP + t] = kb[e];
+    float qv = qb[e], kv = kb[e];
+    if (rope && d < 8) {
+      const int ep = (d ^ 4) * T + t;
+      qv = sty_rope8(qv, qb[ep], d, t, th0, th1, th2, th3, 1.0f);
+      kv = sty_rope8(kv, kb[ep], d, t, th0, th1, th2, th3, 1.0f);
+    }
+    qs[d * TP + t] = qv * a.scale;
+    ks[d * TP + t] = kv;
     vs[d * TP + t] = vb[e];
     gs[d * TP + t] = gb[e];
   }
@@ -427,9 +435,14 @@
       __syncthreads();
       if (half == 1) pm_s[r] = acc[d];
       __syncthreads();
-      if (half == 0 && live) {
-        float* dq = dQ + (size_t)b * dqbs + ho;
-        const float val = (acc[d] + pm_s[r]) * a.scale;
+      if (half == 0 && live) acc[d] = (acc[d] + pm_s[r]) * a.scale;
+    }
+    if (half == 0 && live) {
+      float* dq = dQ + (size_t)b * dqbs + ho;
+#pragma unroll
+      for (int d = 0; d < DH; ++d) {
+        float val = acc[d];
+        if (DH >= 8 && d < 8 && rope) val = sty_rope8(acc[d], acc[(d ^ 4) & (DH - 1)], d, r, th0, th1, th2, th3, -1.0f);
         dq[(size_t)d * T + r] = (overwrite & 1) ? val : dq[(size_t)d * T + r] + val;
       }
     }
@@ -477,9 +490,17 @@
       }
       __syncthreads();
       if (half == 0 && live) {
-        const float vk = ak[d] + pm_s[r], vv_ = av[d] + pl_s[r];
+        const float vv_ = av[d] + pl_s[r];
+        ak[d] += pm_s[r];
+        dv[(size_t)d * T + r] = (overwrite & 4) ? vv_ : dv[(size_t)d * T + r] + vv_;
+      }
+    }
+    if (half == 0 && live) {
+#pragma unroll
+      for (int d = 0; d < DH; ++d) {
+        float vk = ak[d];
+        if (DH >= 8 && d < 8 && rope) vk = sty_rope8(ak[d], ak[(d ^ 4) & (DH - 1)], d, r, th0, th1, th2, th3, -1.0f);
         dk[(size_t)d * T + r] = (overwrite & 2) ? vk : dk[(size_t)d * T + r] + vk;
-        dv[(size_t)d * T + r] = (overwrite & 4) ? vv_ : dv[(size_t)d * T + r] + vv_;
       }
     }
   }
@@ -495,9 +516,14 @@
   return DH == 16 && a.T <= 128;
 }
 bool attention_bwd_can_overwrite(const AttnArgs& a, int DH) { return attn_bwd_small_path(a, DH); }
+bool attention_rope_fused(const AttnArgs& a, int DH) { return attn_bwd_small_path(a, DH) && (a.rope_d == 0 || a.rope_d == 8); }
 
 int launch_attention_bwd(const AttnArgs& a, const float* dO, float* dQ, float* dK, float* dV, size_t dqbs, size_t dkbs,
                          size_t dvbs, size_t dobs, int B, int DH, float* ws, hipStream_t st, int overwrite) {
+  if (a.rope_d && !attention_rope_fused(a, DH)) {
+    set_error("attention_bwd: fused RoPE asked where the kernels have none (attention_rope_fused)");
+    return STY_EINVAL;
+  }
   if (overwrite && !attn_bwd_small_path(a, DH)) {
     set_error("attention_bwd: overwrite requested on a path that accumulates");
     return STY_EINVAL;
@@ -533,6 +559,7 @@
   }
   const bool drop = a.drop_p > 0.f;
   if (attn_bwd_small_path(a, DH)) {
+    ProfScope prof("attn_bwd_small_kernel", 14.0 * (double)B * a.H * DH * a.T * a.T, 32.0 * (double)B * a.H * DH * a.T, st);
     if (drop)
       hipLaunchKernelGGL((attn_bwd_small_kernel<16, true>), dim3(a.H, B), dim3(256), 0, st, a, dO, dobs, dQ, dqbs, dK, dkbs, dV,
                          dvbs, overwrite);
diff --git a/stylish_tts_amd/csrc/bwd.hip b/stylish_tts_amd/csrc/bwd.hip
--- a/stylish_tts_amd/csrc/bwd.hip
+++ b/stylish_tts_amd/csrc/bwd.hip
@@ -361,7 +361,8 @@
                                                                  const float* __restrict__ gb, int relu,
                                                                  const float* __restrict__ out_mask,
                                                                  float* __restrict__ dx, int accumulate,
-                                                                 float* __restrict__ mu_out, float* __restrict__ r_out) {
+                                                                 float* __restrict__ mu_out, float* __restrict__ r_out,
+                                                                 LnDropOut dd) {
   constexpr int CG = 256 / TC;
   __shared__ float red[2][CG][TC];
   const int col = threadIdx.x % TC, cg = threadIdx.x / TC;
@@ -433,7 +434,9 @@
       const size_t o = base + (size_t)c * T;
       const float xh = (xr[i] - mean) * r;
       const float d = r * (gr[i] - s1 - xh * s2);
-      dx[o] = accumulate ? dx[o] + d : d;
+      const float val = accumulate ? dx[o] + d : d;
+      dx[o] = val;
+      if (dd.dx2) dd.dx2[o] = sty_drop(val, dd.p, dd.seed, dd.site, (unsigned)o);
     }
   }
   if (cg == 0) {
@@ -448,7 +451,8 @@
                                                              const float* __restrict__ gb, int relu,
                                                              const float* __restrict__ out_mask,
                                                              float* __restrict__ dx, int accumulate,
-                                                             float* __restrict__ mu_out, float* __restrict__ r_out) {
+                                                             float* __restrict__ mu_out, float* __restrict__ r_out,
+                                                             LnDropOut dd) {
   constexpr int CG = 256 / TC;
   __shared__ float red[2][CG][TC];
   const int col = threadIdx.x % TC, cg = threadIdx.x / TC;
@@ -507,7 +511,9 @@
     const float A = ada ? 1.f + gb[(size_t)b * 2 * C + c] : w[c];
     const float xh = (x[o] - mean) * r;
     const float d = r * (g * A - s1 - xh * s2);
-    dx[o] = accumulate ? dx[o] + d : d;
+    const float val = accumulate ? dx[o] + d : d;
+    dx[o] = val;
+    if (dd.dx2) dd.dx2[o] = sty_drop(val, dd.p, dd.seed, dd.site, (unsigned)o);
   }
   if (cg == 0) {
     mu_out[(size_t)b * T + t] = mean;
@@ -650,10 +656,16 @@
 }
 int launch_chan_ln_bwd(const float* x, const float* dy, const float* y, int B, int C, int T, float eps, int ada,
                        const float* w, const float* gb, int relu, const float* out_mask, float* dx, int accumulate,
-                       float* mu_tmp, float* r_tmp, float* dgb, float* dw, float* db, hipStream_t st, int h16) {
+                       float* mu_tmp, float* r_tmp, float* dgb, float* dw, float* db, hipStream_t st, int h16,
+                       const LnDropOut* drop_out) {
+  const LnDropOut dd = drop_out ? *drop_out : LnDropOut{};
   const bool no32 = getenv("STY_NO_LN32_BWD") != nullptr;
   if (C == 32 && !relu && (size_t)B * T >= 65536 && !no32) {
     const int nblk = cdiv(T, 256);
+    if (dd.dx2) {
+      set_error("chan_ln_bwd: no dropped second output on the C = 32 long-row kernel");
+      return STY_EINVAL;
+    }
     if ((h16 & 4) && accumulate) {
       set_error("chan_ln_bwd: a two-byte dx cannot be accumulated into");
       return STY_EINVAL;
@@ -668,15 +680,20 @@
     set_error("chan_ln_bwd: two-byte tensors only on the C = 32 long-row kernel (chan_ln32_eligible)");
     return STY_EINVAL;
   }
-  if ((size_t)B * T < 65536 && C <= 256)
-    hipLaunchKernelGGL((chan_ln_bwd_dx_reg_kernel<16, 16>), dim3(cdiv(T, 16), B), dim3(256), 0, st, x, dy, y, C, T, eps, ada, w,
-                       gb, relu, out_mask, dx, accumulate, mu_tmp, r_tmp);
-  else if ((size_t)B * T >= 65536)
-    hipLaunchKernelGGL(chan_ln_bwd_dx_kernel<64>, dim3(cdiv(T, 64), B), dim3(256), 0, st, x, dy, y, C, T, eps, ada, w, gb,
-                       relu, out_mask, dx, accumulate, mu_tmp, r_tmp);
-  else
-    hipLaunchKernelGGL(chan_ln_bwd_dx_kernel<16>, dim3(cdiv(T, 16), B), dim3(256), 0, st, x, dy, y, C, T, eps, ada, w, gb,
-                       relu, out_mask, dx, accumulate, mu_tmp, r_tmp);
+  const double ln_bytes = 4.0 * (double)B * C * T;
+  {
+    ProfScope prof("chan_ln_bwd_dx_kernel", 0.0, ln_bytes * (dd.dx2 ? 4.0 : 3.0), st);
+    if ((size_t)B * T < 65536 && C <= 256)
+      hipLaunchKernelGGL((chan_ln_bwd_dx_reg_kernel<16, 16>), dim3(cdiv(T, 16), B), dim3(256), 0, st, x, dy, y, C, T, eps, ada, w,
+                         gb, relu, out_mask, dx, accumulate, mu_tmp, r_tmp, dd);
+    else if ((size_t)B * T >= 65536)
+      hipLaunchKernelGGL(chan_ln_bwd_dx_kernel<64>, dim3(cdiv(T, 64), B), dim3(256), 0, st, x, dy, y, C, T, eps, ada, w, gb,
+                         relu, out_mask, dx, accumulate, mu_tmp, r_tmp, dd);
+    else
+      hipLaunchKernelGGL(chan_ln_bwd_dx_kernel<16>, dim3(cdiv(T, 16), B), dim3(256), 0, st, x, dy, y, C, T, eps, ada, w, gb,
+                         relu, out_mask, dx, accumulate, mu_tmp, r_tmp, dd);
+  }
+  ProfScope prof("chan_ln_bwd_param_kernel", 0.0, ln_bytes * 2.0, st);
   hipLaunchKernelGGL(chan_ln_bwd_param_kernel, dim3(C, B), dim3(256), 0, st, x, dy, y, mu_tmp, r_tmp, C, T, ada, relu,
                      out_mask, dgb, dw, db);
   STY_LAUNCH_CHECK();
@@ -787,6 +804,7 @@
   reinterpret_cast<float4*>(y)[idx] = r;
 }
 int launch_act_fwd(int kind, const float* x, const float* alpha, int B, int C, int T, float* y, hipStream_t st) {
+  ProfScope prof("act_fwd_kernel", 0.0, 8.0 * (double)B * C * T, st);
   const size_t n4 = (size_t)B * C * (T / 4);
   if (kind != ACT_GLU && T % 4 == 0 && n4 < ((size_t)1 << 31) && ((((size_t)x | (size_t)y) & 15) == 0)) {
     hipLaunchKernelGGL(act_fwd4_kernel, dim3((unsigned)((n4 + 255) / 256)), dim3(256), 0, st, kind, x, alpha, (unsigned)C,
@@ -884,6 +902,7 @@
 }
 int launch_act_bwd(int kind, const float* x, const float* dy, const float* alpha, int B, int C, int T, float* dx,
                    int accumulate, float* dalpha, hipStream_t st) {
+  ProfScope prof("act_bwd_kernel", 0.0, 12.0 * (double)B * C * T, st);
   hipLaunchKernelGGL(act_bwd_kernel, dim3(C, B), dim3(256), 0, st, kind, x, dy, alpha, C, T, dx, accumulate, dalpha);
   STY_LAUNCH_CHECK();
   return STY_OK;
@@ -910,6 +929,7 @@
   reinterpret_cast<float4*>(dst)[idx] = d;
 }
 int launch_row_scale_add(const float* src, const float* coef, float k, int rows, int T, float* dst, hipStream_t st) {
+  ProfScope prof("row_scale_add_kernel", 0.0, 12.0 * (double)rows * T, st);
   const size_t n4 = (size_t)rows * (T / 4);
   if (vec4_ok(n4, T, src, dst)) {
     hipLaunchKernelGGL(row_scale_add4_kernel, dim3((unsigned)((n4 + 255) / 256)), dim3(256), 0, st, src, coef, k,
@@ -1250,6 +1270,7 @@
 }
 int launch_dropout(const float* x, const float* res, size_t n, float p, unsigned seed, unsigned site, float* y,
                    int accumulate, hipStream_t st, size_t group) {
+  ProfScope prof("dropout_kernel", 0.0, 4.0 * (double)n * (2.0 + (res ? 1.0 : 0.0) + (accumulate ? 1.0 : 0.0)), st);
   hipLaunchKernelGGL(dropout_kernel, dim3((unsigned)((n + 255) / 256)), dim3(256), 0, st, x, res, n, p, seed, site, y,
                      accumulate, group ? group : 1);
   STY_LAUNCH_CHECK();
diff --git a/stylish_tts_amd/csrc/conv1d.hip b/stylish_tts_amd/csrc/conv1d.hip
--- a/stylish_tts_amd/csrc/conv1d.hip
+++ b/stylish_tts_amd/csrc/conv1d.hip
@@ -388,6 +388,10 @@
   if (a.up_g && (!a.up_gate16 || !a.up_mask || a.up_H <= 0 || a.up_H * a.flatW != a.T)) return false;
   return (long)a.w.Cout * a.T < (1l << 26);
 }
+bool conv1d_has_drop_stage(const ConvArgs& a) {
+  if (stem2d_eligible(a) || conv32p_eligible(a) || a.xh || a.yh || a.rh || a.stat_part || a.x16 || a.y_split) return false;
+  return convk1_eligible(a) || convp16_eligible(a);
+}
 static int launch_conv1d_dispatch(const ConvArgs& a, hipStream_t st) {
   int cin = 0;
   for (int i = 0; i < a.nsrc; ++i) cin += a.xc[i];
@@ -402,6 +406,10 @@
   }
   if (a.ln_out && a.w.Cout != 32) {
     set_error("conv1d: LN epilogue needs Cout == 32");
+    return STY_EINVAL;
+  }
+  if ((a.drop_p > 0.f || a.gate) && !conv1d_has_drop_stage(a)) {
+    set_error("conv1d: output-stage dropout / gate asked of a conv whose kernel has no such stage (conv1d_has_drop_stage)");
     return STY_EINVAL;
   }
   if (stem2d_eligible(a)) return launch_stem2d(a, st);
diff --git a/stylish_tts_amd/csrc/convk1.hip b/stylish_tts_amd/csrc/convk1.hip
--- a/stylish_tts_amd/csrc/convk1.hip
+++ b/stylish_tts_amd/csrc/convk1.hip
@@ -145,6 +145,8 @@
   const __amdgpu_buffer_rsrc_t ry = __builtin_amdgcn_make_buffer_rsrc(a.y, 0, ybytes, 0x00020000);
   const __amdgpu_buffer_rsrc_t rres = __builtin_amdgcn_make_buffer_rsrc(
       const_cast<float*>(a.residual ? a.residual : a.y), 0, a.residual ? ybytes : 0, 0x00020000);
+  const __amdgpu_buffer_rsrc_t rgate =
+      __builtin_amdgcn_make_buffer_rsrc(const_cast<float*>(a.gate ? a.gate : a.y), 0, a.gate ? ybytes : 0, 0x00020000);
   const bool post = a.out_mask && a.out_mask_post;
   const int c4 = lane & 15, rq = lane >> 4;
   const int nq = n0 + wn * 64 + 4 * c4;
@@ -179,6 +181,9 @@
         float4 res = make_float4(0.f, 0.f, 0.f, 0.f);
         if (a.residual) res = __builtin_bit_cast(float4, __builtin_amdgcn_raw_buffer_load_b128(rres, yo, 0, 0));
         const float rr[4] = {res.x, res.y, res.z, res.w};
+        float4 gt = make_float4(1.f, 1.f, 1.f, 1.f);
+        if (a.gate) gt = __builtin_bit_cast(float4, __builtin_amdgcn_raw_buffer_load_b128(rgate, yo, 0, 0));
+        const float gg[4] = {gt.x, gt.y, gt.z, gt.w};
 #pragma unroll
         for (int e = 0; e < 4; ++e) {
           if (RELU == 1) v[e] = fmaxf(v[e], 0.f);
@@ -186,6 +191,8 @@
           if (RELU == 3) v[e] = 0.5f * v[e] * (1.0f + erff(v[e] * 0.70710678118654752f));
           v[e] *= a.out_scale;
           if (a.out_mask && !post) v[e] *= om[e];
+          if (a.drop_p > 0.f) v[e] = sty_drop(v[e], a.drop_p, a.drop_seed, a.drop_site, (unsigned)(yo >> 2) + e);
+          if (a.gate) v[e] = sty_gate(v[e], gg[e], a.gate_p);
           v[e] += rr[e];
           if (post) v[e] *= om[e];
         }
diff --git a/stylish_tts_amd/csrc/convp16.hip b/stylish_tts_amd/csrc/convp16.hip
--- a/stylish_tts_amd/csrc/convp16.hip
+++ b/stylish_tts_amd/csrc/convp16.hip
@@ -218,12 +218,20 @@
         rr[3] = e == 3 ? x : rr[3];
       }
     }
+    const unsigned flat = (unsigned)(((size_t)tl.b * Cout + co) * T + t);
+    float gg[4] = {1.f, 1.f, 1.f, 1.f};
+    if (a.gate) {
+#pragma unroll
+      for (int e = 0; e < 4; ++e) gg[e] = t + e < T ? a.gate[(size_t)flat + e] : 0.f;
+    }
 #pragma unroll
     for (int e = 0; e < 4; ++e) {
       if (RELU == 1) v[e] = fmaxf(v[e], 0.f);
       if (RELU == 2) v[e] = v[e] > 0.f ? v[e] : 0.1f * v[e];
       v[e] *= pre_scale;
       if (a.out_mask && !post) v[e] *= om[e];
+      if (a.drop_p > 0.f) v[e] = sty_drop(v[e], a.drop_p, a.drop_seed, a.drop_site, flat + e);
+      if (a.gate) v[e] = sty_gate(v[e], gg[e], a.gate_p);
       v[e] += rr[e];
       if (post) v[e] *= om[e];
     }
diff --git a/stylish_tts_amd/csrc/misc.hip b/stylish_tts_amd/csrc/misc.hip
--- a/stylish_tts_amd/csrc/misc.hip
+++ b/stylish_tts_amd/csrc/misc.hip
@@ -15,6 +15,7 @@
 }
 int launch_embedding(const int64_t* tokens, const float* emb, int B, int L, int H, int ntok, float scale, float* y,
                      hipStream_t st) {
+  ProfScope prof("embedding_kernel", 0.0, 8.0 * (double)B * L * H, st);
   hipLaunchKernelGGL(embedding_kernel, dim3(cdiv(L, 64), H, B), dim3(64), 0, st, tokens, emb, L, H, ntok, scale, y);
   STY_LAUNCH_CHECK();
   return STY_OK;
@@ -245,6 +246,7 @@
 }
 int launch_embedding_bwd(const int64_t* tokens, const float* g, int B, int L, int H, int ntok, float scale, float* demb,
                          hipStream_t st) {
+  ProfScope prof("embedding_bwd_kernel", 0.0, 8.0 * (double)B * L * H, st);
   hipLaunchKernelGGL(embedding_bwd_kernel, dim3(cdiv(L, 64), H, B), dim3(64), 0, st, tokens, g, L, H, ntok, scale, demb);
   STY_LAUNCH_CHECK();
   return STY_OK;
diff --git a/stylish_tts_amd/csrc/model.h b/stylish_tts_amd/csrc/model.h
--- a/stylish_tts_amd/csrc/model.h
+++ b/stylish_tts_amd/csrc/model.h
@@ -33,6 +33,8 @@
 int launch_rope(float* q, float* k, int B, int H, int DH, int L, int d, const float* theta4, hipStream_t st);
 int launch_rope_copy(const float* qs, const float* ks, float* q, float* k, int B, int H, int DH, int L, int d,
                      const float* theta4, hipStream_t st);
+int launch_rope_strided(const float* qs, const float* ks, size_t sbs, float* q, float* k, size_t dbs, int B, int H, int DH, int L,
+                        int d, const float* theta4, float sgn, hipStream_t st);
 int source_workspace_floats(int B, int T);
 int launch_source(int B, int T, const float* pitch, const float* voiced, const float* noise, uint64_t seed,
                   const float* lin_w, const float* lin_b, float* prior, float* ws, hipStream_t st);
@@ -95,6 +97,8 @@
   float* bp = nullptr;
   float* scratch = nullptr;
   float* scratch2 = nullptr;
+  int ld = 0;
+  bool fwd_only = false;
 };
 
 struct AdaFc {
@@ -143,6 +147,7 @@
 
 struct TextEncLayer {
   PackedConv q, k, v, o, f1, f2;
+  PackedConv qkv;
   const float *n1g, *n1b, *n2g, *n2b;
 };
 struct TextEncPlan {
@@ -267,7 +272,8 @@
 bool chan_ln32_eligible(int B, int C, int T, int relu);
 int launch_chan_ln_bwd(const float* x, const float* dy, const float* y, int B, int C, int T, float eps, int ada,
                        const float* w, const float* gb, int relu, const float* out_mask, float* dx, int accumulate,
-                       float* mu_tmp, float* r_tmp, float* dgb, float* dw, float* db, hipStream_t st, int h16 = 0);
+                       float* mu_tmp, float* r_tmp, float* dgb, float* dw, float* db, hipStream_t st, int h16 = 0,
+                       const LnDropOut* drop_out = nullptr);
 int launch_grn_bwd(const double* part, int nseg, const float* gamma, const float* ds, int B, int C4, float* coef,
                    float* dgamma, hipStream_t st);
 int launch_act_fwd(int kind, const float* x, const float* alpha, int B, int C, int T, float* y, hipStream_t st);
diff --git a/stylish_tts_amd/csrc/norms.hip b/stylish_tts_amd/csrc/norms.hip
--- a/stylish_tts_amd/csrc/norms.hip
+++ b/stylish_tts_amd/csrc/norms.hip
@@ -237,6 +237,7 @@
 
 int launch_chan_layernorm(const float* x, float* y, int B, int C, int T, float eps, int ada, const float* w,
                           const float* bvec, const float* gb, int relu, const float* out_mask, hipStream_t st) {
+  ProfScope prof("chan_layernorm_kernel", 0.0, 8.0 * (double)B * C * T, st);
   const dim3 grid(cdiv(T, 64), B);
 #define STY_LN_CASE(CPT)                                                                                          \
   case 4 * CPT:                                                                                                    \
diff --git a/stylish_tts_amd/csrc/sty_common.h b/stylish_tts_amd/csrc/sty_common.h
--- a/stylish_tts_amd/csrc/sty_common.h
+++ b/stylish_tts_amd/csrc/sty_common.h
@@ -183,7 +183,12 @@
   int up_H = 0;
   int xh = 0, yh = 0, rh = 0, gh = 0;
   int w_row = 0, w_tap = 0;
-};
+  float drop_p = 0.f;
+  unsigned drop_seed = 0, drop_site = 0;
+  const float* gate = nullptr;
+  float gate_p = 0.f;
+};
+bool conv1d_has_drop_stage(const ConvArgs& a);
 int launch_twin_cast(const float* x, const float* mask, int pro, int B, int C, int T, __bf16* y16, hipStream_t st);
 bool wgradb16_eligible(const ConvArgs& fwd);
 int launch_wgradb16(const ConvArgs& fwd, int nsplit, float* partial, int want_bias, hipStream_t st);
@@ -222,6 +227,7 @@
   float *q0 = nullptr, *q1 = nullptr, *q2 = nullptr, *q3 = nullptr, *q4 = nullptr;
   int Cout = 0, Cin = 0, K = 1, CinP = 0, CoutP = 0, glu = 0, blk0 = 0, KH = 1;
   int blk1 = 0, pad = 0;
+  int ld = 0;
 };
 int launch_multi(int which, const MultiJob* jobs, const int* job_of_block, int nblocks, hipStream_t st, int blk_base = 0);
 int launch_sn_unpack_multi(const MultiJob* jobs, const int* job_of_block, int nblocks, hipStream_t st);
@@ -346,6 +352,11 @@
   int n = 0;
 };
 int launch_pack_w2a_multi(const W2aJobs& jobs, hipStream_t st);
+struct LnDropOut {
+  float* dx2 = nullptr;
+  float p = 0.f;
+  unsigned seed = 0, site = 0;
+};
 struct AttnArgs {
   const float* q;
   const float* k;
@@ -359,7 +370,10 @@
   unsigned drop_seed = 0, drop_site = 0;
   float* lse = nullptr;
   int bf16 = 0;
-};
+  int rope_d = 0;
+  float rope_theta[4] = {0.f, 0.f, 0.f, 0.f};
+};
+bool attention_rope_fused(const AttnArgs& a, int DH);
 bool attention16_eligible(const AttnArgs& a, int DH);
 int launch_attention16(const AttnArgs& a, int B, hipStream_t st);
 int launch_attention16_bwd(const AttnArgs& a, const float* dO, float* dQ, float* dK, float* dV, size_t dqbs, size_t dkbs,
@@ -376,6 +390,18 @@
   x *= 0x846CA68Bu;
   x ^= x >> 16;
   return (float)(x >> 8) * (1.0f / 16777216.0f);
+}
+__device__ __forceinline__ float sty_rope8(float xi, float xpair, int i, int pos, float t0, float t1, float t2, float t3, float sgn) {
+  const int k = i & 3;
+  const float ang = (float)pos * (k == 0 ? t0 : k == 1 ? t1 : k == 2 ? t2 : t3);
+  const float rot = i < 4 ? -xpair : xpair;
+  return __builtin_fmaf(xi, cosf(ang), rot * (sgn * sinf(ang)));
+}
+__device__ __forceinline__ float sty_drop(float v, float p, unsigned seed, unsigned site, unsigned idx) {
+  return sty_hash_u(seed, site, idx) >= p ? v / (1.0f - p) : 0.f;
+}
+__device__ __forceinline__ float sty_gate(float v, float fwd_out, float p) {
+  return fwd_out > 0.f ? (p > 0.f ? v / (1.0f - p) : v) : 0.f;
 }
 __device__ __forceinline__ void sty_unit_vec(float re, float im, float& c, float& s) {
   const float h2 = re * re + im * im;
diff --git a/stylish_tts_amd/csrc/train.hip b/stylish_tts_amd/csrc/train.hip
--- a/stylish_tts_amd/csrc/train.hip
+++ b/stylish_tts_amd/csrc/train.hip
@@ -133,11 +133,21 @@
     pend_up.erase(it);
     up_apply(act, u);
   }
+  struct DropSite {
+    float p;
+    unsigned site;
+  };
+  std::unordered_map<const float*, DropSite> drop_of;
+  std::unordered_map<const float*, float*> drop_grad;
+  std::unordered_map<const float*, float> relu_gate;
   void grad_sets_clear() {
     g_twin_only.clear();
     g_no_fp32.clear();
     lazy_mask.clear();
     pend_up.clear();
+    drop_of.clear();
+    drop_grad.clear();
+    relu_gate.clear();
   }
   ~Trainer() {
     wgrad_defer_destroy(defer);
@@ -342,6 +352,22 @@
     wg_need(pn);
     if (live()) chk(launch_conv1d(a, st));
     ConvArgs f = a;
+    if (a.act == ACT_RELU) {
+      if (a.residual || a.out_mask) {
+        set_error("training: output-stage ReLU with a residual or an output mask");
+        rc = STY_ESTATE;
+        return;
+      }
+      relu_gate[a.y] = a.drop_p;
+      f.act = ACT_NONE;
+      f.drop_p = 0.f;
+    } else if (a.act != ACT_NONE) {
+      set_error("training: a conv with an output-stage activation has no backward here");
+      rc = STY_ESTATE;
+      return;
+    } else if (a.drop_p > 0.f) {
+      drop_of[a.y] = DropSite{a.drop_p, a.drop_site};
+    }
     tape.push_back([this, f]() { conv_bwd(f); });
   }
   void conv_bwd(const ConvArgs& f) {
@@ -349,6 +375,16 @@
     const int Tt = f.T;
     const size_t ny = (size_t)B * w.Cout * Tt;
     float* gY = G(f.y, ny);
+    float* gC = gY;
+    if (f.drop_p > 0.f) {
+      auto it = drop_grad.find(f.y);
+      if (it != drop_grad.end()) {
+        gC = it->second;
+      } else {
+        gC = take<float>(ny);
+        if (live()) chk(launch_dropout(gY, nullptr, ny, f.drop_p, f.drop_seed, f.drop_site, gC, 0, st, 1));
+      }
+    }
     float* gR = nullptr;
     if (f.residual && wants(f.residual)) {
       if (!gmap.count(f.residual) && !(f.out_mask && f.out_mask_post) && f.shuffle <= 1)
@@ -421,17 +457,17 @@
       float* sp = deferring() ? wg_take(wgrad_partial_floats(w, B, Tt)) : side_partial;
       float* gwp = PGpacked(w.wp);
       const float osc = f.out_scale;
-      side_push(gY, [=](hipStream_t s) { chk(launch_conv1d_wgrad(f, gY, gmask, osc, gwp, sp, gbias, nullptr, s)); });
+      side_push(gC, [=](hipStream_t s) { chk(launch_conv1d_wgrad(f, gC, gmask, osc, gwp, sp, gbias, nullptr, s)); });
       bias_done = wgrad_fuses_bias(w);
     } else {
       const size_t pn = wgrad_partial_floats(w, B, Tt);
       float* partial = deferring() ? wg_take(pn) : take<float>(pn);
       DeferScope ds(this);
-      if (live()) chk(launch_conv1d_wgrad(f, gY, gmask, f.out_scale, PGpacked(w.wp), partial, gbias, &bias_done, st));
+      if (live()) chk(launch_conv1d_wgrad(f, gC, gmask, f.out_scale, PGpacked(w.wp), partial, gbias, &bias_done, st));
     }
     if (w.bias && !bias_done) {
       float* bs = take<float>(bias_grad_scratch_floats(B, w.Cout, Tt));
-      if (live()) chk(launch_bias_grad(gY, gmask, B, w.Cout, Tt, f.shuffle, f.out_scale, PGpacked(w.bias), bs, st));
+      if (live()) chk(launch_bias_grad(gC, gmask, B, w.Cout, Tt, f.shuffle, f.out_scale, PGpacked(w.bias), bs, st));
     }
     if (any) {
       auto it = m->dgrad.find(w.wp);
@@ -451,8 +487,9 @@
           t->ws.off = mark;
         }
       } u_guard{this, U, mark};
+      const auto gate = f.nsrc == 1 ? relu_gate.find(f.x[0]) : relu_gate.end();
       ConvArgs d;
-      d.x[0] = gY;
+      d.x[0] = gC;
       d.xc[0] = w.Cout;
       d.nsrc = 1;
       d.B = B;
@@ -469,7 +506,7 @@
       }
       d.y = U;
       d.yh = u16;
-      d.xh = is16(gY);
+      d.xh = is16(gC);
       if (f.nsrc == 1 && (f.pro == PRO_NONE || f.pro == PRO_MASK) && gX[0] != gY) {
         d.y = gX[0];
         d.yh = is16(gX[0]);
@@ -479,8 +516,17 @@
           d.out_mask = f.mask;
           d.out_mask_post = 0;
         }
+        if (gate != relu_gate.end()) {
+          d.gate = f.x[0];
+          d.gate_p = gate->second;
+        }
         if (live()) chk(launch_conv1d(d, st));
         ws.off = mark;
+        return;
+      }
+      if (gate != relu_gate.end()) {
+        set_error("training: the reader of an output-stage ReLU has no direct input-gradient conv to gate");
+        rc = STY_ESTATE;
         return;
       }
       if (live()) chk(launch_conv1d(d, st));
@@ -532,9 +578,12 @@
   unsigned drop_site = 0;
   bool dropout_on() const { return m->topts.dropout_seed != 0; }
   float* dropout(const float* x, float p, int C, int Tt, const float* residual, size_t group = 1) {
+    return dropout_at(drop_site++, x, p, C, Tt, residual, group);
+  }
+  float* dropout_at(unsigned site, const float* x, float p, int C, int Tt, const float* residual, size_t group = 1) {
     const size_t n = (size_t)B * C * Tt;
     float* y = take<float>(n);
-    const unsigned seed = m->topts.dropout_seed, site = drop_site++;
+    const unsigned seed = m->topts.dropout_seed;
     if (live()) chk(launch_dropout(x, residual, n, p, seed, site, y, 0, st, group));
     tape.push_back([=]() {
       float* gY = G(y, n);
@@ -579,13 +628,23 @@
       } else {
         gX = Gw(x, nel, acc);
       }
+      LnDropOut dd;
+      auto ido = drop_of.find(x);
+      if (ido != drop_of.end() && !ln32 && !drop_grad.count(x)) {
+        dd.dx2 = take<float>(nel);
+        dd.p = ido->second.p;
+        dd.seed = m->topts.dropout_seed;
+        dd.site = ido->second.site;
+        drop_grad[x] = dd.dx2;
+      }
       const size_t mark = ws.off;
       float* mu = take<float>((size_t)B * Tt);
       float* r = take<float>((size_t)B * Tt);
       float* dw = fc ? nullptr : PG(w, C);
       float* db = fc ? nullptr : PG(bvec, C);
       if (live())
-        chk(launch_chan_ln_bwd(x, gY, y, B, C, Tt, eps, fc ? 1 : 0, w, gbl, relu, omask, gX, acc, mu, r, dgl, dw, db, st, h16));
+        chk(launch_chan_ln_bwd(x, gY, y, B, C, Tt, eps, fc ? 1 : 0, w, gbl, relu, omask, gX, acc, mu, r, dgl, dw, db, st, h16,
+                               dd.dx2 ? &dd : nullptr));
       ws.off = mark;
     });
     return y;
@@ -1133,6 +1192,100 @@
     return o;
   }
 
+  float* attention_qkv(const float* qkv, int Hd, int L, const int64_t* lengths, const float* theta) {
+    const size_t n = (size_t)B * Hd * L, blk = (size_t)Hd * L;
+    const int heads = 8, DH = Hd / heads;
+    float* o = take<float>(n);
+    AttnArgs at;
+    at.q = qkv;
+    at.k = qkv + blk;
+    at.v = qkv + 2 * blk;
+    at.o = o;
+    at.qbs = at.kbs = at.vbs = 3 * blk;
+    at.obs = blk;
+    at.T = L;
+    at.H = heads;
+    at.scale = 1.0f / sqrtf((float)DH);
+    at.lengths = lengths;
+    const bool fused = attention_rope_fused(at, DH);
+    float *qr = nullptr, *kr = nullptr;
+    if (fused) {
+      at.rope_d = 8;
+      for (int i = 0; i < 4; ++i) at.rope_theta[i] = theta[i];
+    } else {
+      qr = take<float>(n);
+      kr = take<float>(n);
+      if (live()) chk(launch_rope_strided(at.q, at.k, 3 * blk, qr, kr, blk, B, heads, DH, L, 8, theta, 1.0f, st));
+      at.q = qr;
+      at.k = kr;
+      at.qbs = at.kbs = blk;
+    }
+    const float pa = m->topts.text_dropout;
+    if (dropout_on() && pa > 0.f) {
+      at.drop_p = pa;
+      at.drop_seed = m->topts.dropout_seed;
+      at.drop_site = drop_site++;
+    }
+    if (live()) chk(launch_attention(at, B, DH, st));
+    const float t4[4] = {theta[0], theta[1], theta[2], theta[3]};
+    tape.push_back([=]() {
+      float* gO = G(o, n);
+      int acc = 1;
+      float* g = fused ? Gw(qkv, 3 * n, acc) : G(qkv, 3 * n);
+      const size_t mark = ws.off;
+      float* w2 = take<float>(attention_bwd_ws_floats(B, heads, L));
+      if (fused) {
+        if (live())
+          chk(launch_attention_bwd(at, gO, g, g + blk, g + 2 * blk, 3 * blk, 3 * blk, 3 * blk, at.obs, B, DH, w2, st, acc ? 0 : 7));
+      } else {
+        float* gq = take<float>(2 * n);
+        float* gk = gq + n;
+        if (live()) {
+          hipError_t e = hipMemsetAsync(gq, 0, 2 * n * sizeof(float), st);
+          if (e != hipSuccess) rc = hip_fail(e, "attention grad memset");
+          chk(launch_attention_bwd(at, gO, gq, gk, g + 2 * blk, blk, blk, 3 * blk, at.obs, B, DH, w2, st, 0));
+          chk(launch_rope_strided(gq, gk, blk, g, g + blk, 3 * blk, B, heads, DH, L, 8, t4, -1.0f, st));
+        }
+      }
+      ws.off = mark;
+    });
+    return o;
+  }
+  float* conv_drop_res(ConvArgs a, float p, const float* residual) {
+    const unsigned site = drop_site++;
+    ConvArgs probe = a;
+    probe.bf16 = m->topts.compute_bf16;
+    probe.residual = residual;
+    if (conv1d_has_drop_stage(probe)) {
+      a.residual = residual;
+      a.drop_p = p;
+      a.drop_seed = m->topts.dropout_seed;
+      a.drop_site = site;
+      conv(a);
+      return a.y;
+    }
+    conv(a);
+    return dropout_at(site, a.y, p, a.w.Cout, a.T, residual);
+  }
+  bool relu_stage_ok(const ConvArgs& f1, const ConvArgs& f2) const {
+    auto it = m->dgrad.find(f2.w.wp);
+    if (it == m->dgrad.end() || f2.nsrc != 1 || !(f2.pro == PRO_NONE || f2.pro == PRO_MASK)) return false;
+    ConvArgs a = f1;
+    a.bf16 = m->topts.compute_bf16;
+    a.act = ACT_RELU;
+    ConvArgs d;
+    d.xc[0] = f2.w.Cout;
+    d.nsrc = 1;
+    d.B = B;
+    d.T = f2.T;
+    d.w = it->second;
+    d.dil = f2.dil;
+    d.bf16 = a.bf16;
+    d.pad = (f2.w.K - 1) * f2.dil - f2.pad;
+    d.pro = f2.out_mask ? PRO_MASK : PRO_NONE;
+    return conv1d_has_drop_stage(a) && conv1d_has_drop_stage(d);
+  }
+
   float* text_encoder(const int64_t* tokens, const int64_t* lengths, int L) {
     const TextEncPlan& t = m->te;
     const int H = t.H;
@@ -1170,46 +1323,23 @@
     pj.out_mask_post = 1;
     conv(pj);
     for (const TextEncLayer& l : t.layers) {
-      float* q = take<float>(n);
-      float* k = take<float>(n);
-      float* v = take<float>(n);
-      ConvArgs aq = base(l.q, x, L, q);
+      if (!l.qkv.wp) {
+        set_error("training: the text encoder's packed q / k / v conv is missing (model not finalized for training?)");
+        rc = STY_ESTATE;
+        return x0;
+      }
+      float* qkv = take<float>(3 * n);
+      ConvArgs aq = base(l.qkv, x, L, qkv);
       aq.pro = PRO_MASK;
       aq.mask = mask;
       conv(aq);
-      aq.w = l.k;
-      aq.y = k;
-      conv(aq);
-      aq.w = l.v;
-      aq.y = v;
-      conv(aq);
-      float* qr = take<float>(n);
-      float* kr = take<float>(n);
-      if (live()) chk(launch_rope_copy(q, k, qr, kr, B, 8, H / 8, L, 8, t.theta, st));
-      {
-        const float* th = t.theta;
-        tape.push_back([=]() {
-          float* gqr = G(qr, n);
-          float* gkr = G(kr, n);
-          if (live()) chk(launch_rope_signed(gqr, gkr, B, 8, H / 8, L, 8, th, -1.0f, st));
-          if (!alias_grad(q, gqr)) {
-            float* gq = G(q, n);
-            if (live()) chk(launch_row_scale_add(gqr, nullptr, 1.0f, B * H, L, gq, st));
-          }
-          if (!alias_grad(k, gkr)) {
-            float* gk = G(k, n);
-            if (live()) chk(launch_row_scale_add(gkr, nullptr, 1.0f, B * H, L, gk, st));
-          }
-        });
-      }
-      float* o = attention3(qr, kr, v, H, L, lengths);
+      float* o = attention_qkv(qkv, H, L, lengths, t.theta);
       const float pd = m->topts.text_dropout;
       const bool dr = dropout_on() && pd > 0.f;
       float* h1 = take<float>(n);
       ConvArgs ao = base(l.o, o, L, h1);
       if (dr) {
-        conv(ao);
-        h1 = dropout(h1, pd, H, L, x);
+        h1 = conv_drop_res(ao, pd, x);
       } else {
         ao.residual = x;
         conv(ao);
@@ -1220,17 +1350,30 @@
       ConvArgs f1 = base(l.f1, x1, L, f0);
       f1.pro = PRO_MASK;
       f1.mask = mask;
-      conv(f1);
-      float* fr = act(ACT_RELU, f0, nullptr, Fc, L);
-      if (dr) fr = dropout(fr, pd, Fc, L, nullptr);
-      float* h2 = take<float>(n);
-      ConvArgs f2 = base(l.f2, fr, L, h2);
+      ConvArgs f2 = base(l.f2, nullptr, L, nullptr);
       f2.pro = PRO_MASK;
       f2.mask = mask;
       f2.out_mask = mask;
+      float* fr;
+      if (relu_stage_ok(f1, f2)) {
+        f1.act = ACT_RELU;
+        if (dr) {
+          f1.drop_p = pd;
+          f1.drop_seed = m->topts.dropout_seed;
+          f1.drop_site = drop_site++;
+        }
+        conv(f1);
+        fr = f0;
+      } else {
+        conv(f1);
+        fr = act(ACT_RELU, f0, nullptr, Fc, L);
+        if (dr) fr = dropout(fr, pd, Fc, L, nullptr);
+      }
+      float* h2 = take<float>(n);
+      f2.x[0] = fr;
+      f2.y = h2;
       if (dr) {
-        conv(f2);
-        h2 = dropout(h2, pd, H, L, x1);
+        h2 = conv_drop_res(f2, pd, x1);
       } else {
         f2.residual = x1;
         conv(f2);
@@ -2392,6 +2535,10 @@
   t->begin(io->style);
   const int inter = t->m->te.proj_m.Cout ? t->m->te.proj_m.Cout : 128;
   float* mu = t->text_encoder(io->texts, io->text_lengths, io->L);
+  if (io->tap_text_encoding && t->live()) {
+    hipError_t e = hipMemcpyAsync(io->tap_text_encoding, mu, (size_t)io->B * inter * io->L * sizeof(float), hipMemcpyDeviceToDevice, st);
+    if (e != hipSuccess) t->rc = hip_fail(e, "text_encoding tap");
+  }
   t->tape.push_back([t]() {
     t->style_fc_backward();
     if (t->on_segment && t->live()) {
diff --git a/stylish_tts_amd/csrc/wgrad.hip b/stylish_tts_amd/csrc/wgrad.hip
--- a/stylish_tts_amd/csrc/wgrad.hip
+++ b/stylish_tts_amd/csrc/wgrad.hip
@@ -1316,9 +1316,10 @@
     }
     scale = j.p1[co] / sqrtf(red[0]);
   }
+  const int ld = j.ld ? j.ld : j.CoutP;
   for (int i = threadIdx.x; i < n; i += 256) {
     const int ci = i / j.K, k = i % j.K;
-    j.q0[((size_t)k * j.CinP + ci) * j.CoutP + cp] = src[(size_t)co * n + i] * scale;
+    j.q0[((size_t)k * j.CinP + ci) * ld + cp] = src[(size_t)co * n + i] * scale;
   }
   if (threadIdx.x == 0 && j.q1) j.q1[cp] = j.p3 ? j.p3[co] : 0.f;
 }
@@ -1351,13 +1352,13 @@
   const MultiJob j = jobs[job_of_block[blk]];
   const int co = blk - j.blk0;
   const int n = j.Cin * j.K;
-  const int cp = co;
+  const int cp = co, ld = j.ld ? j.ld : j.CoutP;
   if (threadIdx.x == 0 && j.q3 && j.p3) j.q3[co] += j.p3[cp];
   if (!j.p2) {
     if (!j.q0) return;
     for (int i = threadIdx.x; i < n; i += 256) {
       const int ci = i / j.K, k = i % j.K;
-      j.q0[(size_t)co * n + i] += j.p0[((size_t)k * j.CinP + ci) * j.CoutP + cp];
+      j.q0[(size_t)co * n + i] += j.p0[((size_t)k * j.CinP + ci) * ld + cp];
     }
     return;
   }
@@ -1366,7 +1367,7 @@
   for (int i = threadIdx.x; i < n; i += 256) {
     const int ci = i / j.K, k = i % j.K;
     const float v = j.p2[(size_t)co * n + i];
-    dot = fmaf(j.p0[((size_t)k * j.CinP + ci) * j.CoutP + cp], v, dot);
+    dot = fmaf(j.p0[((size_t)k * j.CinP + ci) * ld + cp], v, dot);
     nn = fmaf(v, v, nn);
   }
   r1[threadIdx.x] = dot;
@@ -1384,7 +1385,7 @@
   for (int i = threadIdx.x; i < n; i += 256) {
     const int ci = i / j.K, k = i % j.K;
     const float v = j.p2[(size_t)co * n + i];
-    j.q2[(size_t)co * n + i] += gg / norm * (j.p0[((size_t)k * j.CinP + ci) * j.CoutP + cp] - v * d / (norm * norm));
+    j.q2[(size_t)co * n + i] += gg / norm * (j.p0[((size_t)k * j.CinP + ci) * ld + cp] - v * d / (norm * norm));
   }
 }
 int launch_multi(int which, const MultiJob* jobs, const int* job_of_block, int nblocks, hipStream_t st, int blk_base) {
diff --git a/stylish_tts_amd/modules.py b/stylish_tts_amd/modules.py
--- a/stylish_tts_amd/modules.py
+++ b/stylish_tts_amd/modules.py
@@ -455,7 +455,7 @@
         L.check(lib.sty_speech_prepare_train(self._handle, C.c_void_p(torch.cuda.current_stream(device).cuda_stream)))
 
     def forward_train(self, texts, text_lengths, alignment, pitch, energy, voiced, style, denormal_pitch, *, noise=None,
-                      seed=0, prior_override=None, style_stream=None):
+                      seed=0, prior_override=None, style_stream=None, taps=None):
         _check_speech_shapes(texts, text_lengths, alignment, pitch, energy, voiced, style, denormal_pitch, noise,
                              self.cfg["style_dim"])
         dev = style.device
@@ -477,6 +477,10 @@
                 setattr(io, name, t.data_ptr())
         io.seed = int(seed)
         io.style_stream = style_stream.cuda_stream if style_stream is not None else None
+        for k, t in (taps or {}).items():
+            if k != "tap_text_encoding":
+                raise KeyError(k)
+            setattr(io, k, t.data_ptr())
         audio = torch.empty(B, 1, 300 * T, dtype=torch.float32, device=dev)
         io.audio = audio.data_ptr()
         need = C.c_size_t()
```

Measured after the change: 384,800 frames/s (median of 6 runs). No clear change (+0.8%).
